# apelykh/deep-audio-mixer

Measured on AMD Instinct MI355X. Metric: stem-spectrogram-frames/sec (train), higher is better.
Workload: dtype f32; 1 GPU; C3: model_resnet (ResNet18, 8 stems) train step incl. STFT front-end, 8-stem 3 s @ 44.1 kHz stereo clips, n_fft 2048 hop 1024 -> 8x1025x130 per clip; batch_per_gpu=8, global_batch=8, parallelism=dp1, hip_graph=True, world_size=1, device_index=0, grad_buckets=1, allreduce_overlap=False

## Files before the change

deep-audio-mixer_amd/_lib.py:

```python
import ctypes
import os

import torch
import torch.utils.data

_HERE = os.path.dirname(os.path.abspath(__file__))
LIB_PATH = os.environ.get('DAM_LIB_PATH') or os.path.join(_HERE, 'libdam_hip.so')

EXPECTED_ABI = 22

_STATUS = {0: 'DAM_OK', -1: 'DAM_ERR_BAD_ARG', -2: 'DAM_ERR_UNSUPPORTED', -3: 'DAM_ERR_LAUNCH',
           -4: 'DAM_ERR_WORKSPACE'}

c_i, c_i64, c_f, c_p = ctypes.c_int, ctypes.c_int64, ctypes.c_float, ctypes.c_void_p
c_d = ctypes.c_double

SIGNATURES = {
    'dam_arch': (ctypes.c_char_p, []),
    'dam_abi_version': (c_i, []),
    'dam_host_dontfork_pinned': (c_i, [c_p, c_p]),
    'dam_step_mark_create': (c_i, [c_p]),
    'dam_step_mark_record': (c_i, [c_p, c_p]),
    'dam_step_mark_wait': (c_i, [c_p, c_p]),
    'dam_step_mark_synchronize': (c_i, [c_p]),
    'dam_step_mark_destroy': (c_i, [c_p]),
    'dam_stft_twiddle_count': (c_i64, [c_i]),
    'dam_stft_fill_twiddles_host': (c_i, [c_i, c_p]),
    'dam_stft_logmag_f32': (c_i, [c_p, c_i, c_i64, c_i64, c_i, c_i64, c_p, c_p, c_p, c_i, c_i, c_f, c_i, c_p, c_p]),
    'dam_stft_logmag_strided_f32': (c_i, [c_p, c_i, c_i64, c_i64, c_i64, c_i64, c_i64, c_i, c_i64, c_i64, c_p, c_p, c_p,
                                          c_i, c_i, c_f, c_i, c_p, c_p, c_i, c_p]),
    'dam_stft_complex_f32': (c_i, [c_p, c_i, c_i64, c_i64, c_i, c_i64, c_i64, c_i64, c_p, c_p, c_p, c_i, c_i, c_p, c_p]),
    'dam_stft_complex_strided_f32': (c_i, [c_p, c_i, c_i64, c_i64, c_i64, c_i64, c_i64, c_i64, c_i64, c_i, c_i64, c_i64,
                                           c_p, c_p, c_p, c_i, c_i, c_p, c_p]),
    'dam_istft_workspace_bytes': (c_i64, [c_i64, c_i64, c_i, c_i, c_i64]),
    'dam_istft_f32': (c_i, [c_p, c_p, c_i64, c_i64, c_i, c_i, c_i64, c_p, c_p, c_p, c_p, c_i64, c_p]),
    'dam_augment_gains_f32': (c_i, [ctypes.c_uint64, c_p, c_i64, c_i, c_i, c_f, c_f, c_p, c_p]),
    'dam_conv_packed_weight_count': (c_i64, [c_i, c_i, c_i, c_i]),
    'dam_conv_pack_weights_f32': (c_i, [c_p, c_i, c_i, c_i, c_i, c_i, c_p, c_p]),
    'dam_conv_pack_weights_multi_f32': (c_i, [c_p, c_i, c_i64, c_p]),
    'dam_conv2d_tapgrid_f32': (c_i, [c_p, c_i, c_i, c_i, c_i, c_i, c_p, c_i, c_i, c_p, c_p, c_p, c_i, c_i, c_p] +
                               [c_i] * 17 + [c_p, c_p, c_p, c_p, c_p, c_p, c_i64, c_p, c_p]),
    'dam_conv_batch_bytes': (c_i64, []),
    'dam_conv_batch_init': (c_i, [c_p]),
    'dam_conv_batch_flush': (c_i, [c_p, c_p]),
    'dam_conv2d_wgrad_workspace_floats': (c_i64, [c_i, c_i, c_i, c_i]),
    'dam_conv2d_wgrad_f32': (c_i, [c_p, c_i, c_i, c_i, c_i, c_i, c_p, c_p, c_i, c_p] + [c_i] * 9 +
                             [c_p, c_i, c_p, c_i64, c_p, c_p]),
    'dam_wgrad_queue_bytes': (c_i64, []),
    'dam_wgrad_queue_init': (c_i, [c_p]),
    'dam_wgrad_queue_pending': (c_i, [c_p]),
    'dam_wgrad_queue_flush': (c_i, [c_p, c_p]),
    'dam_wgrad_queue_set_batching': (c_i, [c_p, c_i]),
    'dam_bn_workspace_floats': (c_i64, [c_i]),
    'dam_bn_stats_f32': (c_i, [c_p, c_i64, c_i, c_p, c_p, c_p, c_p, c_p, c_f, c_f, c_p, c_p, c_p, c_p, c_p, c_p]),
    'dam_bn_finalize_f32': (c_i, [c_p, c_i, c_i, c_p, c_p, c_p, c_p, c_p, c_f, c_f, c_p, c_p, c_p, c_p, c_p]),
    'dam_conv1x1_pair_f32': (c_i, [c_p, c_p, c_i, c_p, c_p, c_i, c_i, c_i, c_i, c_i, c_i, c_p, c_i, c_i, c_i, c_i, c_i, c_p]),
    'dam_dgrad_s2_3x3_f32': (c_i, [c_p, c_p, c_p, c_p, c_i, c_i, c_i, c_i, c_i, c_p, c_i, c_i, c_p, c_p, c_p, c_p]),
    'dam_conv_s2_pair_fwd_f32': (c_i, [c_p, c_p, c_p, c_i, c_i, c_i, c_i, c_i, c_p, c_p, c_p, c_p, c_p, c_p]),
    'dam_bn_finalize_pair_f32': (c_i, [c_p, c_p, c_i, c_i, c_p, c_p, c_p]),
    'dam_strip_diag_counters': (c_i, [c_p, c_i]),
    'dam_bn_stats_partial_f32': (c_i, [c_p, c_i64, c_i, c_p, c_p, c_p]),
    'dam_bn_finalize_apply_f32': (c_i, [c_p, c_i, c_i, c_p, c_p, c_i64, c_p, c_p, c_p, c_i, c_p, c_p, c_p]),
    'dam_bn_eval_affine_f32': (c_i, [c_i, c_p, c_p, c_p, c_p, c_f, c_p, c_p, c_p, c_p, c_p]),
    'dam_bn_apply_f32': (c_i, [c_p, c_i64, c_i, c_p, c_p, c_p, c_p, c_p, c_i, c_p, c_p, c_p]),
    'dam_bn_stats_pair_f32': (c_i, [c_p, c_p, c_i64, c_i, c_p, c_p, c_p, c_p]),
    'dam_bn_pair_workspace_floats': (c_i64, [c_i]),
    'dam_bn_backward_pair_f32': (c_i, [c_p, c_p, c_p, c_i64, c_i, c_i] + [c_p] * 16),
    'dam_bn_backward_f32': (c_i, [c_p, c_p, c_p, c_i64, c_i, c_p, c_p, c_p, c_i, c_p, c_p, c_p, c_p, c_p, c_p, c_p, c_i, c_p]),
    'dam_channel_sum_f32': (c_i, [c_p, c_i64, c_i, c_i, c_p, c_p, c_p]),
    'dam_dropout_tick': (c_i, [c_p, c_i64, c_p, c_p]),
    'dam_dropout_apply_f32': (c_i, [c_p, c_i64, c_f, ctypes.c_uint64, c_p, c_p, c_p]),
    'dam_heads_fwd_f32': (c_i, [c_p, c_i, c_i, c_i, c_i, c_p, c_p, c_p, c_p, c_p, c_p, c_p]),
    'dam_heads_bwd_workspace_floats': (c_i64, [c_i, c_i, c_i, c_i]),
    'dam_heads_bwd_f32': (c_i, [c_p, c_p, c_p, c_i, c_i, c_i, c_i, c_p, c_p, c_p, c_p, c_p, c_p, c_p, c_p, c_p]),
    'dam_masksum_fwd_f32': (c_i, [c_p, c_p, c_i, c_i, c_i64, c_p, c_p]),
    'dam_masksum_workspace_floats': (c_i64, [c_i, c_i]),
    'dam_masksum_bwd_f32': (c_i, [c_p, c_p, c_i, c_i, c_i64, c_p, c_p, c_p]),
    'dam_masksum_mse_f32': (c_i, [c_p, c_p, c_p, c_i, c_i, c_i64, c_p, c_p, c_p, c_p, c_p]),
    'dam_adam_l2_step_f32': (c_i, [c_p, c_p, c_p, c_p, c_i64, c_p, c_p, c_f, c_f, c_f, c_f, c_f, c_f, c_p, c_p]),
    'dam_digest64_u32': (c_i, [c_p, c_i64, c_i64, c_i, c_i, c_p, c_p]),
    'dam_gains_smooth': (c_i, [c_p, c_i, c_i, c_i, c_i, c_p, c_p, c_p, c_p]),
    'dam_gain_ramp_apply': (c_i, [c_p, c_i, c_p, c_i64, c_i64, c_i64, c_i, c_p, c_i, c_p]),
    'dam_mixdown_workspace_elems': (c_i64, [c_i64]),
    'dam_mixdown_peak_normalize': (c_i, [c_p, c_i, c_p, c_i, c_i64, c_i64, c_i, c_i, c_p, c_i, c_p, c_p]),
    'dam_nchw_to_nhwc16_f32': (c_i, [c_p, c_i, c_i, c_i64, c_p, c_p]),
    'dam_loudness_kweight_coeffs': (c_i, [c_d, c_p]),
    'dam_loudness_workspace_bytes': (c_i64, [c_i64, c_i]),
    'dam_loudness_block_energy': (c_i, [c_p, c_i, c_i64, c_i, c_i64, c_i64, c_p, c_p, c_p, c_i, c_d, c_p, c_p, c_p]),
    'dam_loudness_batch_workspace_bytes': (c_i64, [c_i, c_i64, c_i, c_i]),
    'dam_loudness_block_energy_batch': (c_i, [c_p, c_i, c_i, c_i64, c_i, c_i64, c_i64, c_i64, c_p, c_i, c_p, c_p, c_p, c_i,
                                              c_d, c_p, c_p, c_p]),
    'dam_loudness_gate': (c_i, [c_p, c_i, c_i, c_i, c_p, c_p]),
    'dam_loudness_target_gains': (c_i, [c_p, c_p, c_i, c_p, c_p]),
    'dam_pcm_tile_frames': (c_i64, [c_i]),
    'dam_pcm_max_blocks': (c_i, []),
    'dam_pcm_encode': (c_i, [c_p, c_i, c_i, c_i64, c_p, c_i, c_i, c_i, ctypes.c_uint64, c_p, c_p, c_p]),
    'dam_true_peak_taps_host': (c_i, [c_p]),
    'dam_true_peak_tile_samples': (c_i64, []),
    'dam_true_peak_max_blocks': (c_i, []),
    'dam_true_peak_workspace_bytes': (c_i64, [c_i, c_i64, c_i]),
    'dam_true_peak_batch': (c_i, [c_p, c_i, c_i, c_i64, c_i, c_i64, c_i64, c_i64, c_p, c_i, c_p, c_p, c_p, c_p]),
    'dam_peak_limit_gains': (c_i, [c_p, c_p, c_i, c_i, c_d, c_p]),
    'dam_loudness_window_power': (c_i, [c_p, c_i, c_i, c_i, c_i, c_p, c_p, c_p]),
    'dam_loudness_curve_stats': (c_i, [c_p, c_i, c_i, c_p, c_p]),
    'dam_loudness_profile_error': (c_i, [c_p, c_p, c_i, c_i, c_i, c_p, c_p, c_p]),
}



class BnFin(ctypes.Structure):
    _fields_ = [('gamma', c_p), ('beta', c_p), ('running_mean', c_p), ('running_var', c_p), ('num_batches_tracked', c_p),
                ('momentum', c_f), ('eps', c_f), ('save_mean', c_p), ('save_invstd', c_p), ('scale', c_p), ('shift', c_p)]


class BnBwdSums(ctypes.Structure):
    _fields_ = [('x', c_p), ('mean', c_p), ('invstd', c_p), ('mask_scale', c_p), ('mask_shift', c_p), ('res_mask_bits', c_p),
                ('mask_bits', c_p)]


_lib = None


def lib():
    global _lib
    if torch.cuda._is_in_bad_fork() or torch.utils.data.get_worker_info() is not None:
        raise RuntimeError('deep_audio_mixer_amd: a GPU kernel was asked for in a DataLoader worker / forked child process '
                           '(pid %d).  The GPU belongs to the parent: workers of MultitrackAudioDataset return host PCM '
                           '(PcmItem / HostPcmBatch) and the front-end runs in the main process -- see '
                           'features.batch_features(batch)' % os.getpid())
    if _lib is None:
        if not os.path.exists(LIB_PATH):
            raise RuntimeError('libdam_hip.so is not built (%s): run `python __graft_entry__.py` or '
                               '`python deep-audio-mixer_amd/build.py`; there is no CPU fallback' % LIB_PATH)
        l = ctypes.CDLL(LIB_PATH)
        l.dam_abi_version.restype, l.dam_abi_version.argtypes = c_i, []
        have = l.dam_abi_version()
        if have != EXPECTED_ABI:
            raise RuntimeError('%s speaks ABI version %d, this package expects %d: the library is stale -- rebuild it '
                               '(`python deep-audio-mixer_amd/build.py --force`)' % (LIB_PATH, have, EXPECTED_ABI))
        for name, (res, args) in SIGNATURES.items():
            fn = getattr(l, name)
            fn.restype, fn.argtypes = res, args
        _lib = l
    return _lib


def check(status, what):
    if status != 0:
        raise RuntimeError('%s failed: %s (%d)' % (what, _STATUS.get(status, '?'), status))


def ptr(t):
    return None if t is None else t.data_ptr()


def stream():
    return torch.cuda.current_stream().cuda_stream


def require_cuda(*tensors):
    for t in tensors:
        if t is not None and not t.is_cuda:
            raise RuntimeError('deep_audio_mixer_amd kernels run on the GPU only (got a %s tensor); '
                               'there is no CPU fallback' % t.device)
```

deep-audio-mixer_amd/csrc/dam_bn.hip:

```cpp
#include <type_traits>
#include "dam_common.h"

namespace dam {
namespace {

constexpr int BN_MAX_PARTS = 1024;
static_assert(BN_MAX_PARTS == BN_BWD_RECORDS_MAX, "records a data-gradient epilogue may leave");

struct BnLaunch { int threads, q, r, parts; int64_t ppb; };

inline BnLaunch bn_plan(int64_t P, int C, int max_parts = BN_MAX_PARTS) {
    BnLaunch l;
    l.q = C / 4;
    l.r = 256 / l.q;
    if (l.r < 1) l.r = 1;
    l.threads = l.q * l.r;
    int64_t parts = cdiv(P, (int64_t)l.r * 16);
    if (parts > max_parts) {
        parts = max_parts;
        while (l.threads < 1024 && parts * l.threads < 131072 && (size_t)(l.r * 2) * C * 3 * sizeof(float) <= 48 * 1024) {
            l.r *= 2;
            l.threads *= 2;
        }
    }
    if (parts < 1) parts = 1;
    l.ppb = cdiv(P, parts);
    l.parts = (int)cdiv(P, l.ppb);
    return l;
}

struct RecAdd {
    template <int NV>
    static __device__ __forceinline__ void step(float* a, const float* b) {
#pragma unroll
        for (int k = 0; k < NV; ++k) a[k] += b[k];
    }
};
struct RecChan {
    template <int NV>
    static __device__ __forceinline__ void step(float* a, const float* b) {
        static_assert(NV == 3, "(n, mean, M2)");
        const float na = a[0], nb = b[0];
        if (nb != 0.f) {
            const float nn = na + nb, d = b[1] - a[1];
            a[1] += d * (nb / nn);
            a[2] += b[2] + d * d * (na * nb / nn);
            a[0] = nn;
        }
    }
};
template <int NV, typename Merge>
__device__ __forceinline__ void record_tail(float* sm, const float (&v)[NV][4], int C, int cq, int pr, int R,
                                            float* __restrict__ record ) {
#pragma unroll
    for (int i = 0; i < 4; ++i) {
        float* o = sm + ((size_t)pr * C + cq * 4 + i) * NV;
#pragma unroll
        for (int k = 0; k < NV; ++k) o[k] = v[k][i];
    }
    __syncthreads();
    int span = 1;
    while (span < R) span <<= 1;
    for (int stride = span >> 1; stride >= 1; stride >>= 1) {
        if (pr < stride && pr + stride < R) {
#pragma unroll
            for (int i = 0; i < 4; ++i)
                Merge::template step<NV>(sm + ((size_t)pr * C + cq * 4 + i) * NV, sm + ((size_t)(pr + stride) * C + cq * 4 + i) * NV);
        }
        __syncthreads();
    }
    if (pr == 0) {
#pragma unroll
        for (int i = 0; i < 4; ++i) {
            const int c = cq * 4 + i;
#pragma unroll
            for (int k = 0; k < NV; ++k) store_sc1(record + (size_t)c * NV + k, sm[(size_t)c * NV + k]);
        }
    }
}

__global__ void bn_stats_partial_kernel(const float* __restrict__ x, int64_t P, int C, int Q, int R, int64_t ppb,
                                        float* __restrict__ partial ,
                                        const float* __restrict__ x2, float* __restrict__ partial2) {
    extern __shared__ __attribute__((aligned(16))) float sm[];
    if (blockIdx.y) { x = x2; partial = partial2; }
    const int cq = threadIdx.x % Q, pr = threadIdx.x / Q;
    const int64_t lo = blockIdx.x * ppb, hi = (lo + ppb < P) ? lo + ppb : P;
    float k[4] = {0, 0, 0, 0}, s1[4] = {0, 0, 0, 0}, s2[4] = {0, 0, 0, 0};
    int n = 0;
    constexpr int U = 8;
    for (int64_t p = lo + pr; p < hi; p += (int64_t)R * U) {
        float4 v[U];
#pragma unroll
        for (int u = 0; u < U; ++u) {
            const int64_t q = p + (int64_t)u * R;
            v[u] = q < hi ? *reinterpret_cast<const float4*>(x + q * C + cq * 4) : make_float4(0.f, 0.f, 0.f, 0.f);
        }
        if (n == 0) { k[0] = v[0].x; k[1] = v[0].y; k[2] = v[0].z; k[3] = v[0].w; }
#pragma unroll
        for (int u = 0; u < U; ++u) {
            if (p + (int64_t)u * R < hi) {
                const float e[4] = {v[u].x, v[u].y, v[u].z, v[u].w};
#pragma unroll
                for (int i = 0; i < 4; ++i) {
                    const float d = e[i] - k[i];
                    s1[i] += d;
                    s2[i] = fmaf(d, d, s2[i]);
                }
                ++n;
            }
        }
    }
    float v[3][4];
#pragma unroll
    for (int i = 0; i < 4; ++i) {
        const float md = n ? s1[i] / n : 0.f;
        v[0][i] = (float)n;
        v[1][i] = k[i] + md;
        v[2][i] = n ? fmaxf(s2[i] - s1[i] * md, 0.f) : 0.f;
    }
    record_tail<3, RecChan>(sm, v, C, cq, pr, R, partial + (size_t)blockIdx.x * C * 3);
}

__global__ __launch_bounds__(64) void bn_stats_finalize_kernel(const float* __restrict__ partial, int parts, int C,
                                         const float* __restrict__ gamma, const float* __restrict__ beta,
                                         float* __restrict__ running_mean, float* __restrict__ running_var,
                                         long long* __restrict__ num_batches, float momentum, float eps,
                                         float* __restrict__ save_mean, float* __restrict__ save_invstd,
                                         float* __restrict__ scale, float* __restrict__ shift, const BnFinArgs second,
                                         const float* __restrict__ partial2) {
    if (blockIdx.y) {
        partial = partial2; gamma = second.gamma; beta = second.beta; running_mean = second.running_mean;
        running_var = second.running_var; num_batches = second.num_batches; momentum = second.momentum; eps = second.eps;
        save_mean = second.save_mean; save_invstd = second.save_invstd; scale = second.scale; shift = second.shift;
    }
    const int c = blockIdx.x, lane = threadIdx.x;
    if (c == 0 && lane == 0 && num_batches) *num_batches += 1;
    const float gam_c = gamma[c], bet_c = beta[c];
    const float rm_c = running_mean ? running_mean[c] : 0.f, rv_c = running_mean ? running_var[c] : 0.f;
    constexpr int U = 16;
    float rn[U], rmn[U], rq[U];
#pragma unroll
    for (int u = 0; u < U; ++u) {
        const int p = lane + 64 * u;
        const float* o = partial + ((size_t)(p < parts ? p : 0) * C + c) * 3;
        rn[u] = o[0]; rmn[u] = o[1]; rq[u] = o[2];
        if (p >= parts) rn[u] = 0.f;
    }
    double na = 0, sa = 0;
#pragma unroll
    for (int u = 0; u < U; ++u) { na += (double)rn[u]; sa += (double)rn[u] * (double)rmn[u]; }
    for (int p = lane + 64 * U; p < parts; p += 64) {
        const float* o = partial + ((size_t)p * C + c) * 3;
        na += (double)o[0]; sa += (double)o[0] * (double)o[1];
    }
#pragma unroll
    for (int off = 32; off >= 1; off >>= 1) { na += __shfl_xor(na, off); sa += __shfl_xor(sa, off); }
    const double ma = sa / na;
    double qa = 0;
#pragma unroll
    for (int u = 0; u < U; ++u) { const double d = (double)rmn[u] - ma; qa += (double)rq[u] * (rn[u] != 0.f ? 1.0 : 0.0) + (double)rn[u] * d * d; }
    for (int p = lane + 64 * U; p < parts; p += 64) {
        const float* o = partial + ((size_t)p * C + c) * 3;
        const double d = (double)o[1] - ma;
        qa += (double)o[2] + (double)o[0] * d * d;
    }
#pragma unroll
    for (int off = 32; off >= 1; off >>= 1) qa += __shfl_xor(qa, off);
    if (lane != 0) return;
    const double var = qa / na;
    const float mean = (float)ma;
    const float invstd = (float)(1.0 / sqrt(var + (double)eps));
    save_mean[c] = mean;
    save_invstd[c] = invstd;
    const float sc = gam_c * invstd;
    scale[c] = sc;
    shift[c] = bet_c - mean * sc;
    if (running_mean) {
        const double unbiased = na > 1 ? qa / (na - 1) : var;
        running_mean[c] = (1.f - momentum) * rm_c + momentum * mean;
        running_var[c] = (1.f - momentum) * rv_c + momentum * (float)unbiased;
    }
}

__global__ void bn_eval_affine_kernel(int C, const float* __restrict__ gamma, const float* __restrict__ beta,
                                      const float* __restrict__ running_mean, const float* __restrict__ running_var,
                                      float eps, float* __restrict__ save_mean, float* __restrict__ save_invstd,
                                      float* __restrict__ scale, float* __restrict__ shift) {
    const int c = blockIdx.x * blockDim.x + threadIdx.x;
    if (c >= C) return;
    const float invstd = 1.0f / sqrtf(running_var[c] + eps);
    const float sc = gamma[c] * invstd;
    save_mean[c] = running_mean[c];
    save_invstd[c] = invstd;
    scale[c] = sc;
    shift[c] = beta[c] - running_mean[c] * sc;
}

__global__ void bn_apply_kernel(const float* __restrict__ x, int64_t nquads, int Q, const float* __restrict__ scale,
                                const float* __restrict__ shift, const float* __restrict__ res,
                                const float* __restrict__ rscale, const float* __restrict__ rshift, int relu,
                                float* __restrict__ y, unsigned char* __restrict__ sign_bits) {
    for (int64_t e = blockIdx.x * (int64_t)blockDim.x + threadIdx.x; e < nquads; e += (int64_t)gridDim.x * blockDim.x) {
        const int cq = (int)(e % Q);
        const float4 v = reinterpret_cast<const float4*>(x)[e];
        const float4 sc = reinterpret_cast<const float4*>(scale)[cq], sh = reinterpret_cast<const float4*>(shift)[cq];
        float4 o = make_float4(fmaf(v.x, sc.x, sh.x), fmaf(v.y, sc.y, sh.y), fmaf(v.z, sc.z, sh.z), fmaf(v.w, sc.w, sh.w));
        if (res) {
            float4 r = reinterpret_cast<const float4*>(res)[e];
            if (rscale) {
                const float4 a = reinterpret_cast<const float4*>(rscale)[cq], b = reinterpret_cast<const float4*>(rshift)[cq];
                r = make_float4(fmaf(r.x, a.x, b.x), fmaf(r.y, a.y, b.y), fmaf(r.z, a.z, b.z), fmaf(r.w, a.w, b.w));
            }
            o.x += r.x; o.y += r.y; o.z += r.z; o.w += r.w;
        }
        if (relu) { o.x = fmaxf(o.x, 0.f); o.y = fmaxf(o.y, 0.f); o.z = fmaxf(o.z, 0.f); o.w = fmaxf(o.w, 0.f); }
        reinterpret_cast<float4*>(y)[e] = o;
        if (sign_bits) sign_bits[e] = (unsigned char)((o.x > 0.f) | ((o.y > 0.f) << 1) | ((o.z > 0.f) << 2) | ((o.w > 0.f) << 3));
    }
}

__device__ __forceinline__ float4 sign_quad(unsigned b) {
    return make_float4((float)(b & 1u), (float)((b >> 1) & 1u), (float)((b >> 2) & 1u), (float)((b >> 3) & 1u));
}

struct BnBwdSide {
    const float* x;
    const float* gamma;
    const float* mean;
    const float* invstd;
    float* dx;
    float* dgamma;
    float* dbeta;
};
template <int NB>
struct BnBwdSides { BnBwdSide s[NB]; };

template <int MASK, int NB>
__global__ void bn_bwd_partial_kernel(const float* __restrict__ dy, const float* __restrict__ y_mask, const BnBwdSides<NB> sd,
                                      int64_t P, int C, int Q, int R, int64_t ppb, const float* __restrict__ mscale,
                                      const float* __restrict__ mshift, float* __restrict__ partial ) {
    extern __shared__ __attribute__((aligned(16))) float sm[];
    const int cq = threadIdx.x % Q, pr = threadIdx.x / Q;
    const int64_t lo = blockIdx.x * ppb, hi = (lo + ppb < P) ? lo + ppb : P;
    float4 mu[NB], is[NB];
#pragma unroll
    for (int s = 0; s < NB; ++s) {
        mu[s] = reinterpret_cast<const float4*>(sd.s[s].mean)[cq];
        is[s] = reinterpret_cast<const float4*>(sd.s[s].invstd)[cq];
    }
    float4 msc = make_float4(0.f, 0.f, 0.f, 0.f), msh = msc;
    if (MASK == 2) { msc = reinterpret_cast<const float4*>(mscale)[cq]; msh = reinterpret_cast<const float4*>(mshift)[cq]; }
    float acc[1 + NB][4] = {};
    constexpr int U = NB == 1 ? 4 : 3;
    for (int64_t p = lo + pr; p < hi; p += (int64_t)R * U) {
        float4 gv[U], mv[U], xv[NB][U];
#pragma unroll
        for (int u = 0; u < U; ++u) {
            const int64_t q = p + (int64_t)u * R;
            const bool ok = q < hi;
            const float4 z = make_float4(0.f, 0.f, 0.f, 0.f);
            gv[u] = z; mv[u] = make_float4(1.f, 1.f, 1.f, 1.f);
#pragma unroll
            for (int s = 0; s < NB; ++s) xv[s][u] = z;
            if (ok) {
                gv[u] = *reinterpret_cast<const float4*>(dy + q * C + cq * 4);
#pragma unroll
                for (int s = 0; s < NB; ++s) xv[s][u] = *reinterpret_cast<const float4*>(sd.s[s].x + q * C + cq * 4);
                if (MASK == 1) mv[u] = *reinterpret_cast<const float4*>(y_mask + q * C + cq * 4);
            }
            if (MASK == 3) mv[u] = sign_quad(ok ? reinterpret_cast<const unsigned char*>(y_mask)[q * Q + cq] : 0);
        }
#pragma unroll
        for (int u = 0; u < U; ++u) {
            float4 g = gv[u];
            float4 m = mv[u];
            if (MASK == 2) {
                const float4 v = xv[0][u];
                m = make_float4(fmaf(v.x, msc.x, msh.x), fmaf(v.y, msc.y, msh.y), fmaf(v.z, msc.z, msh.z), fmaf(v.w, msc.w, msh.w));
            }
            g.x = m.x > 0.f ? g.x : 0.f; g.y = m.y > 0.f ? g.y : 0.f; g.z = m.z > 0.f ? g.z : 0.f; g.w = m.w > 0.f ? g.w : 0.f;
            acc[0][0] += g.x; acc[0][1] += g.y; acc[0][2] += g.z; acc[0][3] += g.w;
#pragma unroll
            for (int s = 0; s < NB; ++s) {
                const float4 v = xv[s][u];
                float* b = acc[1 + s];
                b[0] = fmaf(g.x, (v.x - mu[s].x) * is[s].x, b[0]); b[1] = fmaf(g.y, (v.y - mu[s].y) * is[s].y, b[1]);
                b[2] = fmaf(g.z, (v.z - mu[s].z) * is[s].z, b[2]); b[3] = fmaf(g.w, (v.w - mu[s].w) * is[s].w, b[3]);
            }
        }
    }
    record_tail<1 + NB, RecAdd>(sm, acc, C, cq, pr, R, partial + (size_t)blockIdx.x * C * (1 + NB));
}

__device__ __forceinline__ double wave_sum64_f64(double v) {
#pragma unroll
    for (int off = 32; off >= 1; off >>= 1) v += __shfl_down(v, off);
    return v;
}

template <int NV>
__device__ __forceinline__ void wave_record_sums(const float* __restrict__ partial, int parts, int C, int c, double (&s)[NV]) {
    const int lane = threadIdx.x;
    constexpr int U = 16;
    float r[U][NV];
#pragma unroll
    for (int u = 0; u < U; ++u) {
        const int p = lane + 64 * u;
        const float* o = partial + ((size_t)(p < parts ? p : 0) * C + c) * NV;
#pragma unroll
        for (int k = 0; k < NV; ++k) r[u][k] = p < parts ? o[k] : 0.f;
    }
#pragma unroll
    for (int k = 0; k < NV; ++k) s[k] = 0;
#pragma unroll
    for (int u = 0; u < U; ++u)
#pragma unroll
        for (int k = 0; k < NV; ++k) s[k] += (double)r[u][k];
    for (int p = lane + 64 * U; p < parts; p += 64)
#pragma unroll
        for (int k = 0; k < NV; ++k) s[k] += partial[((size_t)p * C + c) * NV + k];
#pragma unroll
    for (int k = 0; k < NV; ++k) s[k] = wave_sum64_f64(s[k]);
}

__global__ __launch_bounds__(64) void bn_bwd_finalize_kernel(const float* __restrict__ partial, int parts, int C, double count,
                                       const float* __restrict__ gamma, const float* __restrict__ mean,
                                       const float* __restrict__ invstd, int training, float* __restrict__ dgamma,
                                       float* __restrict__ dbeta, float* __restrict__ coef ) {
    const int c = blockIdx.x, lane = threadIdx.x;
    const float gam_c = gamma[c], inv_c = invstd[c], mean_c = mean[c];
    double s[2];
    wave_record_sums<2>(partial, parts, C, c, s);
    if (lane != 0) return;
    const double s1 = s[0], s2 = s[1];
    dbeta[c] = (float)s1;
    dgamma[c] = (float)s2;
    const double g = (double)gam_c * inv_c;
    double c2 = 0, c3 = 0;
    if (training) {
        c2 = -g * inv_c * s2 / count;
        c3 = -g * s1 / count - c2 * mean_c;
    }
    coef[c] = (float)g; coef[C + c] = (float)c2; coef[2 * C + c] = (float)c3;
}

template <int MASK>
__global__ void bn_bwd_apply_kernel(const float* __restrict__ dy, const float* __restrict__ y_mask,
                                    const float* __restrict__ x, int64_t nquads, int Q, int C,
                                    const float* __restrict__ coef, const float* __restrict__ mscale,
                                    const float* __restrict__ mshift, float* __restrict__ dx) {
    for (int64_t e = blockIdx.x * (int64_t)blockDim.x + threadIdx.x; e < nquads; e += (int64_t)gridDim.x * blockDim.x) {
        const int cq = (int)(e % Q);
        float4 g = reinterpret_cast<const float4*>(dy)[e];
        const float4 v = reinterpret_cast<const float4*>(x)[e];
        if (MASK != 0) {
            float4 m;
            if (MASK == 1) {
                m = reinterpret_cast<const float4*>(y_mask)[e];
            } else if (MASK == 3) {
                m = sign_quad(reinterpret_cast<const unsigned char*>(y_mask)[e]);
            } else {
                const float4 sc = reinterpret_cast<const float4*>(mscale)[cq], sh = reinterpret_cast<const float4*>(mshift)[cq];
                m = make_float4(fmaf(v.x, sc.x, sh.x), fmaf(v.y, sc.y, sh.y), fmaf(v.z, sc.z, sh.z), fmaf(v.w, sc.w, sh.w));
            }
            g.x = m.x > 0.f ? g.x : 0.f; g.y = m.y > 0.f ? g.y : 0.f; g.z = m.z > 0.f ? g.z : 0.f; g.w = m.w > 0.f ? g.w : 0.f;
        }
        const float4 c1 = reinterpret_cast<const float4*>(coef)[cq], c2 = reinterpret_cast<const float4*>(coef + C)[cq],
                     c3 = reinterpret_cast<const float4*>(coef + 2 * C)[cq];
        float4 o;
        o.x = fmaf(c1.x, g.x, fmaf(c2.x, v.x, c3.x)); o.y = fmaf(c1.y, g.y, fmaf(c2.y, v.y, c3.y));
        o.z = fmaf(c1.z, g.z, fmaf(c2.z, v.z, c3.z)); o.w = fmaf(c1.w, g.w, fmaf(c2.w, v.w, c3.w));
        reinterpret_cast<float4*>(dx)[e] = o;
    }
}

__global__ void channel_sum_partial_kernel(const float* __restrict__ x, int64_t P, int C, int Q, int R, int64_t ppb,
                                           float* __restrict__ partial) {
    extern __shared__ float sm[];
    const int cq = threadIdx.x % Q, pr = threadIdx.x / Q;
    const int64_t lo = blockIdx.x * ppb, hi = (lo + ppb < P) ? lo + ppb : P;
    float a[1][4] = {};
    constexpr int U = 8;
    for (int64_t p = lo + pr; p < hi; p += (int64_t)R * U) {
        float4 v[U];
#pragma unroll
        for (int u = 0; u < U; ++u) {
            const int64_t q = p + (int64_t)u * R;
            v[u] = q < hi ? *reinterpret_cast<const float4*>(x + q * C + cq * 4) : make_float4(0.f, 0.f, 0.f, 0.f);
        }
#pragma unroll
        for (int u = 0; u < U; ++u) { a[0][0] += v[u].x; a[0][1] += v[u].y; a[0][2] += v[u].z; a[0][3] += v[u].w; }
    }
    record_tail<1, RecAdd>(sm, a, C, cq, pr, R, partial + (size_t)blockIdx.x * C);
}
__global__ __launch_bounds__(64) void channel_sum_finalize_kernel(const float* __restrict__ partial, int parts, int C, int n_real,
                                            float* __restrict__ out) {
    double s[1];
    wave_record_sums<1>(partial, parts, C, blockIdx.x, s);
    if (threadIdx.x == 0) out[blockIdx.x] = (float)s[0];
}

__device__ __forceinline__ float4 zero4() { return make_float4(0.f, 0.f, 0.f, 0.f); }
constexpr int FA_THREADS = 256;
constexpr int FA_U = 4;

constexpr int FA_WGS = 512;

struct FaPlan { int cs, nslices, nranges, q, ppi; int64_t ppr; };

inline int fa_cs(int C) { return C <= 32 ? C : 16; }
inline FaPlan fa_plan(int64_t P, int C) {
    FaPlan f;
    f.cs = fa_cs(C);
    f.nslices = C / f.cs;
    f.q = f.cs / 4;
    f.ppi = FA_THREADS / f.q;
    int64_t want = P / ((int64_t)f.ppi * FA_U * 2);
    const int64_t cap = FA_WGS / f.nslices > 0 ? FA_WGS / f.nslices : 1;
    if (want > cap) want = cap;
    if (want < 1) want = 1;
    f.ppr = cdiv(P, want);
    f.nranges = (int)cdiv(P, f.ppr);
    return f;
}
constexpr int FA_TABLE_BYTES_MAX = 80 * 1024;
inline bool fa_table_ok(int C, int parts, int rec_floats) { return (int64_t)parts * fa_cs(C) * rec_floats * 4 <= FA_TABLE_BYTES_MAX; }
constexpr int FA_FWD_TABLE_KB = 24;
inline bool fa_fwd_table_ok(int C, int parts) {
    return fa_table_ok(C, parts, 3) && (int64_t)parts * fa_cs(C) * 12 <= (int64_t)FA_FWD_TABLE_KB * 1024;
}

template <int NR, int NV, typename F>
__device__ __forceinline__ void fa_slice_sums(const float* __restrict__ partial, int parts, int C, int ch, int CS, double* red,
                                              double (&acc)[NV], F term) {
    const int tid = threadIdx.x, TPC = FA_THREADS / CS, i0 = tid / CS;
    constexpr int RU = 16;
#pragma unroll
    for (int k = 0; k < NV; ++k) acc[k] = 0;
    for (int p0 = i0; p0 < parts; p0 += TPC * RU) {
        float rec[RU][NR];
#pragma unroll
        for (int u = 0; u < RU; ++u) {
            const int p = p0 + u * TPC;
            const float* o = partial + ((size_t)(p < parts ? p : i0) * C + ch) * NR;
#pragma unroll
            for (int k = 0; k < NR; ++k) rec[u][k] = o[k];
        }
#pragma unroll
        for (int u = 0; u < RU; ++u)
            if (p0 + u * TPC < parts) {
                double v[NV];
                term(rec[u], v);
#pragma unroll
                for (int k = 0; k < NV; ++k) acc[k] += v[k];
            }
    }
#pragma unroll
    for (int k = 0; k < NV; ++k) red[tid * NV + k] = acc[k];
    __syncthreads();
    if (tid < CS)
        for (int i = 1; i < TPC; ++i)
#pragma unroll
            for (int k = 0; k < NV; ++k) acc[k] += red[(tid + i * CS) * NV + k];
}

template <int S> using FaSet = std::integral_constant<int, S>;
template <typename Load, typename Emit>
__device__ __forceinline__ void fa_stream(int64_t p0, int64_t hi, int64_t step, Load load, Emit emit) {
    for (;;) {
        if (p0 + step < hi) load(FaSet<1>{}, p0 + step);
        emit(FaSet<0>{}, p0);
        p0 += step;
        if (p0 >= hi) break;
        if (p0 + step < hi) load(FaSet<0>{}, p0 + step);
        emit(FaSet<1>{}, p0);
        p0 += step;
        if (p0 >= hi) break;
    }
}

__global__ __launch_bounds__(FA_THREADS) void bn_fin_apply_kernel(const float* __restrict__ partial, int parts, int C, int CS,
                                                                   const BnFinArgs fin, const float* __restrict__ x, int64_t P,
                                                                   int64_t ppr, const float* __restrict__ res,
                                                                   const float* __restrict__ rscale, const float* __restrict__ rshift,
                                                                   int relu, float* __restrict__ y, unsigned char* __restrict__ sign_bits) {
    __shared__ double red[FA_THREADS * 3];
    __shared__ __attribute__((aligned(16))) float tab[2 * 32];
    const int tid = threadIdx.x, slice = blockIdx.y, q = CS / 4, tq = tid % q, tp = tid / q, ppi = FA_THREADS / q;
    const int Q = C / 4, cq = slice * q + tq;
    const int64_t lo = blockIdx.x * ppr, hi = (lo + ppr < P) ? lo + ppr : P;
    const int64_t step = (int64_t)ppi * FA_U;
    float4 xv[2][FA_U], rv[2][FA_U];
    auto load = [&](auto set, int64_t p0) {
        constexpr int S = decltype(set)::value;
#pragma unroll
        for (int u = 0; u < FA_U; ++u) {
            const int64_t p = p0 + (int64_t)u * ppi;
            xv[S][u] = p < hi ? reinterpret_cast<const float4*>(x)[p * Q + cq] : zero4();
            if (res) rv[S][u] = p < hi ? reinterpret_cast<const float4*>(res)[p * Q + cq] : zero4();
        }
    };
    load(FaSet<0>{}, lo + tp);
    float4 ra = make_float4(1.f, 1.f, 1.f, 1.f), rb = zero4();
    if (rscale) { ra = reinterpret_cast<const float4*>(rscale)[cq]; rb = reinterpret_cast<const float4*>(rshift)[cq]; }
    {
        const int cl = tid % CS, ch = slice * CS + cl;
        const float m0 = partial[(size_t)ch * 3 + 1];
        const float gam = fin.gamma[ch], bet = fin.beta[ch];
        const bool writer = blockIdx.x == 0 && tid < CS;
        const float rm = (writer && fin.running_mean) ? fin.running_mean[ch] : 0.f, rvv = (writer && fin.running_mean) ? fin.running_var[ch] : 0.f;
        double acc[3];
        fa_slice_sums<3, 3>(partial, parts, C, ch, CS, red, acc, [m0](const float (&r)[3], double (&v)[3]) {
            const double n = (double)r[0], d = (double)r[1] - (double)m0;
            v[0] = n; v[1] = n * d; v[2] = n != 0.0 ? (double)r[2] + n * d * d : 0.0;
        });
        if (tid < CS) {
            const double na = acc[0], ds = acc[1] / na, qa = acc[2] - acc[1] * ds;
            const double var = qa / na;
            const float mean = (float)((double)m0 + ds);
            const float invstd = (float)(1.0 / sqrt((var > 0 ? var : 0.0) + (double)fin.eps));
            const float sc = gam * invstd, sh = bet - mean * sc;
            tab[cl] = sc; tab[CS + cl] = sh;
            if (writer) {
                fin.save_mean[ch] = mean; fin.save_invstd[ch] = invstd; fin.scale[ch] = sc; fin.shift[ch] = sh;
                if (fin.running_mean) {
                    const double unbiased = na > 1 ? (qa > 0 ? qa : 0.0) / (na - 1) : var;
                    fin.running_mean[ch] = (1.f - fin.momentum) * rm + fin.momentum * mean;
                    fin.running_var[ch] = (1.f - fin.momentum) * rvv + fin.momentum * (float)unbiased;
                }
                if (ch == 0 && fin.num_batches) *fin.num_batches += 1;
            }
        }
        __syncthreads();
    }
    const float4 sc = *reinterpret_cast<const float4*>(tab + tq * 4), sh = *reinterpret_cast<const float4*>(tab + CS + tq * 4);
    fa_stream(lo + tp, hi, step, load, [&](auto set, int64_t p0) {
        constexpr int S = decltype(set)::value;
#pragma unroll
        for (int u = 0; u < FA_U; ++u) {
            const int64_t p = p0 + (int64_t)u * ppi;
            if (p < hi) {
                const float4 v = xv[S][u];
                float4 o = make_float4(fmaf(v.x, sc.x, sh.x), fmaf(v.y, sc.y, sh.y), fmaf(v.z, sc.z, sh.z), fmaf(v.w, sc.w, sh.w));
                if (res) {
                    float4 r = rv[S][u];
                    if (rscale) r = make_float4(fmaf(r.x, ra.x, rb.x), fmaf(r.y, ra.y, rb.y), fmaf(r.z, ra.z, rb.z), fmaf(r.w, ra.w, rb.w));
                    o.x += r.x; o.y += r.y; o.z += r.z; o.w += r.w;
                }
                if (relu) { o.x = fmaxf(o.x, 0.f); o.y = fmaxf(o.y, 0.f); o.z = fmaxf(o.z, 0.f); o.w = fmaxf(o.w, 0.f); }
                reinterpret_cast<float4*>(y)[p * Q + cq] = o;
                if (sign_bits)
                    sign_bits[p * Q + cq] = (unsigned char)((o.x > 0.f) | ((o.y > 0.f) << 1) | ((o.z > 0.f) << 2) | ((o.w > 0.f) << 3));
            }
        }
    });
}

template <int MASK, int NB>
__global__ __launch_bounds__(FA_THREADS) void bn_bwd_fin_apply_kernel(const float* __restrict__ partial, int parts, int C, int CS,
                                                                       double count, int training, const BnBwdSides<NB> sd,
                                                                       const float* __restrict__ dy, const float* __restrict__ y_mask,
                                                                       int64_t P, int64_t ppr, const float* __restrict__ mscale,
                                                                       const float* __restrict__ mshift) {
    constexpr int NR = 1 + NB;
    __shared__ double red[FA_THREADS * NR];
    __shared__ __attribute__((aligned(16))) float tab[3 * NB * 32];
    const int tid = threadIdx.x, slice = blockIdx.y, q = CS / 4, tq = tid % q, tp = tid / q, ppi = FA_THREADS / q;
    const int Q = C / 4, cq = slice * q + tq;
    const int64_t lo = blockIdx.x * ppr, hi = (lo + ppr < P) ? lo + ppr : P;
    constexpr int UB = NB == 1 ? 3 : 2;
    const int64_t step = (int64_t)ppi * UB;
    float4 gv[2][UB], xv[NB][2][UB], mv[2][UB];
    auto load = [&](auto set, int64_t p0) {
        constexpr int S = decltype(set)::value;
#pragma unroll
        for (int u = 0; u < UB; ++u) {
            const int64_t p = p0 + (int64_t)u * ppi;
            const bool ok = p < hi;
            gv[S][u] = ok ? reinterpret_cast<const float4*>(dy)[p * Q + cq] : zero4();
#pragma unroll
            for (int s = 0; s < NB; ++s) xv[s][S][u] = ok ? reinterpret_cast<const float4*>(sd.s[s].x)[p * Q + cq] : zero4();
            if (MASK == 1) mv[S][u] = ok ? reinterpret_cast<const float4*>(y_mask)[p * Q + cq] : zero4();
            if (MASK == 3) mv[S][u] = sign_quad(ok ? reinterpret_cast<const unsigned char*>(y_mask)[p * Q + cq] : 0);
        }
    };
    load(FaSet<0>{}, lo + tp);
    float4 msc = zero4(), msh = zero4();
    if (MASK == 2) { msc = reinterpret_cast<const float4*>(mscale)[cq]; msh = reinterpret_cast<const float4*>(mshift)[cq]; }
    {
        const int cl = tid % CS, ch = slice * CS + cl;
        float gam[NB], inv[NB], mu[NB];
#pragma unroll
        for (int s = 0; s < NB; ++s) { gam[s] = sd.s[s].gamma[ch]; inv[s] = sd.s[s].invstd[ch]; mu[s] = sd.s[s].mean[ch]; }
        double acc[NR];
        fa_slice_sums<NR, NR>(partial, parts, C, ch, CS, red, acc, [](const float (&r)[NR], double (&v)[NR]) {
#pragma unroll
            for (int k = 0; k < NR; ++k) v[k] = (double)r[k];
        });
        if (tid < CS) {
#pragma unroll
            for (int s = 0; s < NB; ++s) {
                const double s1 = acc[0], s2 = acc[1 + s];
                const double g = (double)gam[s] * inv[s];
                double c2 = 0, c3 = 0;
                if (training) { c2 = -g * inv[s] * s2 / count; c3 = -g * s1 / count - c2 * mu[s]; }
                float* t = tab + 3 * s * CS;
                t[cl] = (float)g; t[CS + cl] = (float)c2; t[2 * CS + cl] = (float)c3;
                if (blockIdx.x == 0) { sd.s[s].dbeta[ch] = (float)s1; sd.s[s].dgamma[ch] = (float)s2; }
            }
        }
        __syncthreads();
    }
    float4 k[NB][3];
#pragma unroll
    for (int i = 0; i < 3 * NB; ++i) k[i / 3][i % 3] = *reinterpret_cast<const float4*>(tab + i * CS + tq * 4);
    fa_stream(lo + tp, hi, step, load, [&](auto set, int64_t p0) {
        constexpr int S = decltype(set)::value;
#pragma unroll
        for (int u = 0; u < UB; ++u) {
            const int64_t p = p0 + (int64_t)u * ppi;
            if (p < hi) {
                float4 g = gv[S][u];
                if (MASK != 0) {
                    float4 m = mv[S][u];
                    if (MASK == 2) {
                        const float4 v = xv[0][S][u];
                        m = make_float4(fmaf(v.x, msc.x, msh.x), fmaf(v.y, msc.y, msh.y), fmaf(v.z, msc.z, msh.z), fmaf(v.w, msc.w, msh.w));
                    }
                    g.x = m.x > 0.f ? g.x : 0.f; g.y = m.y > 0.f ? g.y : 0.f; g.z = m.z > 0.f ? g.z : 0.f; g.w = m.w > 0.f ? g.w : 0.f;
                }
                float4 o[NB];
#pragma unroll
                for (int s = 0; s < NB; ++s) {
                    const float4 v = xv[s][S][u], c1 = k[s][0], c2 = k[s][1], c3 = k[s][2];
                    o[s].x = fmaf(c1.x, g.x, fmaf(c2.x, v.x, c3.x)); o[s].y = fmaf(c1.y, g.y, fmaf(c2.y, v.y, c3.y));
                    o[s].z = fmaf(c1.z, g.z, fmaf(c2.z, v.z, c3.z)); o[s].w = fmaf(c1.w, g.w, fmaf(c2.w, v.w, c3.w));
                }
#pragma unroll
                for (int s = 0; s < NB; ++s) reinterpret_cast<float4*>(sd.s[s].dx)[p * Q + cq] = o[s];
            }
        }
    });
}

inline int elt_blocks(int64_t n) {
    int64_t b = cdiv(n, 256);
    return (int)(b < 4096 ? (b < 1 ? 1 : b) : 4096);
}

constexpr int FA_PARTS_KB = 64;
inline int fa_max_parts(int C, int rec_floats) {
    int m = FA_PARTS_KB * 1024 / (fa_cs(C) * rec_floats * 4);
    if (m > BN_MAX_PARTS) m = BN_MAX_PARTS;
    return m < 64 ? 64 : m;
}

inline bool fin_args(const dam_bn_fin* f, BnFinArgs* a) {
    if (!f || !f->gamma || !f->beta || !f->save_mean || !f->save_invstd || !f->scale || !f->shift) return false;
    *a = BnFinArgs{f->gamma, f->beta, f->running_mean, f->running_var, (long long*)f->num_batches_tracked, f->momentum,
                   f->eps, f->save_mean, f->save_invstd, f->scale, f->shift};
    return true;
}

template <int... MASKS, typename F>
inline bool with_mask(int mask, F f) {
    return ((mask == MASKS ? (f(std::integral_constant<int, MASKS>{}), true) : false) || ...);
}

template <int NB, int... MASKS>
inline int bn_bwd_launch(const BnLaunch& l, bool given, bool fused, int mask, const BnBwdSides<NB>& sd, const float* dy,
                         const float* y_mask, int64_t P, int C, int training, const float* mask_scale, const float* mask_shift,
                         float* workspace, hipStream_t st) {
    if (!given) {
        const bool known = with_mask<MASKS...>(mask, [&](auto m) {
            hipLaunchKernelGGL((bn_bwd_partial_kernel<decltype(m)::value, NB>), dim3(l.parts), dim3(l.threads),
                               (size_t)l.r * C * (1 + NB) * sizeof(float), st, dy, y_mask, sd, P, C, l.q, l.r, l.ppb, mask_scale,
                               mask_shift, workspace);
        });
        if (!known) return DAM_ERR_BAD_ARG;
        DAM_CHECK_LAUNCH();
    }
    if (fused) {
        const FaPlan f = fa_plan(P, C);
        const bool known = with_mask<MASKS...>(mask, [&](auto m) {
            hipLaunchKernelGGL((bn_bwd_fin_apply_kernel<decltype(m)::value, NB>), dim3(f.nranges, f.nslices), dim3(FA_THREADS), 0, st,
                               (const float*)workspace, l.parts, C, f.cs, (double)P, training, sd, dy, y_mask, P, f.ppr, mask_scale,
                               mask_shift);
        });
        if (!known) return DAM_ERR_BAD_ARG;
        DAM_CHECK_LAUNCH();
    }
    return DAM_OK;
}

}
}

using namespace dam;

extern "C" int64_t dam_bn_workspace_floats(int C) { return (int64_t)BN_RECORDS_MAX * C * 3; }

extern "C" int dam_bn_stats_partial_f32(const float* x, int64_t n_pixels, int C, float* workspace, int* parts_host, void* stream) {
    if (!x || !workspace || !parts_host || n_pixels <= 0) return DAM_ERR_BAD_ARG;
    if (C % 16 || C > 1024) return DAM_ERR_UNSUPPORTED;
    const BnLaunch l = bn_plan(n_pixels, C, fa_max_parts(C, 3));
    hipLaunchKernelGGL(bn_stats_partial_kernel, dim3(l.parts), dim3(l.threads), (size_t)l.r * C * 3 * sizeof(float), (hipStream_t)stream,
                       x, n_pixels, C, l.q, l.r, l.ppb, workspace, (const float*)nullptr, (float*)nullptr);
    DAM_CHECK_LAUNCH();
    *parts_host = l.parts;
    return DAM_OK;
}

extern "C" int dam_bn_finalize_apply_f32(const float* partial, int parts, int C, const dam_bn_fin* fin, const float* x,
                                         int64_t n_pixels, const float* res, const float* res_scale, const float* res_shift,
                                         int relu, float* y, uint8_t* sign_bits, void* stream) {
    BnFinArgs a;
    if (!partial || parts <= 0 || !fin_args(fin, &a) || !x || !y || n_pixels <= 0) return DAM_ERR_BAD_ARG;
    if (res_scale && (!res || !res_shift)) return DAM_ERR_BAD_ARG;
    if (C % 16 || C > 1024) return DAM_ERR_UNSUPPORTED;
    hipStream_t st = (hipStream_t)stream;
    if (!fa_fwd_table_ok(C, parts)) {
        int rc = dam_bn_finalize_f32(partial, parts, C, fin->gamma, fin->beta, fin->running_mean, fin->running_var,
                                     fin->num_batches_tracked, fin->momentum, fin->eps, fin->save_mean, fin->save_invstd, fin->scale,
                                     fin->shift, stream);
        if (rc != DAM_OK) return rc;
        return dam_bn_apply_f32(x, n_pixels, C, fin->scale, fin->shift, res, res_scale, res_shift, relu, y, sign_bits, stream);
    }
    const FaPlan f = fa_plan(n_pixels, C);
    hipLaunchKernelGGL(bn_fin_apply_kernel, dim3(f.nranges, f.nslices), dim3(FA_THREADS), 0, st, partial, parts, C, f.cs, a, x,
                       n_pixels, f.ppr, res, res_scale, res_shift, relu, y, sign_bits);
    DAM_CHECK_LAUNCH();
    return DAM_OK;
}

extern "C" int dam_bn_stats_f32(const float* x, int64_t n_pixels, int C, const float* gamma, const float* beta,
                                float* running_mean, float* running_var, int64_t* num_batches_tracked,
                                float momentum, float eps, float* save_mean, float* save_invstd, float* scale,
                                float* shift, float* workspace, void* stream) {
    if (!x || !gamma || !beta || !save_mean || !save_invstd || !scale || !shift || !workspace || n_pixels <= 0)
        return DAM_ERR_BAD_ARG;
    if (C % 16 || C > 1024) return DAM_ERR_UNSUPPORTED;
    const BnLaunch l = bn_plan(n_pixels, C);
    hipStream_t st = (hipStream_t)stream;
    hipLaunchKernelGGL(bn_stats_partial_kernel, dim3(l.parts), dim3(l.threads), (size_t)l.r * C * 3 * sizeof(float), st,
                       x, n_pixels, C, l.q, l.r, l.ppb, workspace, (const float*)nullptr, (float*)nullptr);
    DAM_CHECK_LAUNCH();
    hipLaunchKernelGGL(bn_stats_finalize_kernel, dim3(C), dim3(64), 0, st, workspace, l.parts, C,
                       gamma, beta, running_mean, running_var, (long long*)num_batches_tracked, momentum, eps,
                       save_mean, save_invstd, scale, shift, BnFinArgs{}, (const float*)nullptr);
    DAM_CHECK_LAUNCH();
    return DAM_OK;
}

extern "C" int dam_bn_stats_pair_f32(const float* x_a, const float* x_b, int64_t n_pixels, int C, const dam_bn_fin* a,
                                     const dam_bn_fin* b, float* workspace, void* stream) {
    BnFinArgs fa, fb;
    if (!x_a || !x_b || !fin_args(a, &fa) || !fin_args(b, &fb) || !workspace || n_pixels <= 0) return DAM_ERR_BAD_ARG;
    if (C % 16 || C > 1024) return DAM_ERR_UNSUPPORTED;
    const BnLaunch l = bn_plan(n_pixels, C);
    hipStream_t st = (hipStream_t)stream;
    float* ws_b = workspace + (size_t)BN_RECORDS_MAX * C * 3;
    hipLaunchKernelGGL(bn_stats_partial_kernel, dim3(l.parts, 2), dim3(l.threads), (size_t)l.r * C * 3 * sizeof(float), st, x_a,
                       n_pixels, C, l.q, l.r, l.ppb, workspace, x_b, ws_b);
    DAM_CHECK_LAUNCH();
    hipLaunchKernelGGL(bn_stats_finalize_kernel, dim3(C, 2), dim3(64), 0, st, workspace, l.parts, C, fa.gamma, fa.beta,
                       fa.running_mean, fa.running_var, fa.num_batches, fa.momentum, fa.eps, fa.save_mean, fa.save_invstd, fa.scale,
                       fa.shift, fb, (const float*)ws_b);
    DAM_CHECK_LAUNCH();
    return DAM_OK;
}

extern "C" int dam_bn_finalize_f32(const float* partial, int parts, int C, const float* gamma, const float* beta,
                                   float* running_mean, float* running_var, int64_t* num_batches_tracked,
                                   float momentum, float eps, float* save_mean, float* save_invstd, float* scale,
                                   float* shift, void* stream) {
    if (!partial || parts <= 0 || C <= 0 || !gamma || !beta || !save_mean || !save_invstd || !scale || !shift)
        return DAM_ERR_BAD_ARG;
    hipLaunchKernelGGL(bn_stats_finalize_kernel, dim3(C), dim3(64), 0, (hipStream_t)stream, partial, parts, C, gamma, beta,
                       running_mean, running_var, (long long*)num_batches_tracked, momentum, eps, save_mean, save_invstd,
                       scale, shift, BnFinArgs{}, (const float*)nullptr);
    DAM_CHECK_LAUNCH();
    return DAM_OK;
}

extern "C" int dam_bn_finalize_pair_f32(const float* partial_a, const float* partial_b, int parts, int C, const dam_bn_fin* a,
                                        const dam_bn_fin* b, void* stream) {
    BnFinArgs fa, fb;
    if (!partial_a || !partial_b || parts <= 0 || C <= 0 || !fin_args(a, &fa) || !fin_args(b, &fb)) return DAM_ERR_BAD_ARG;
    hipLaunchKernelGGL(bn_stats_finalize_kernel, dim3(C, 2), dim3(64), 0, (hipStream_t)stream, partial_a, parts, C, fa.gamma, fa.beta,
                       fa.running_mean, fa.running_var, fa.num_batches, fa.momentum, fa.eps, fa.save_mean, fa.save_invstd, fa.scale,
                       fa.shift, fb, partial_b);
    DAM_CHECK_LAUNCH();
    return DAM_OK;
}

extern "C" int dam_bn_eval_affine_f32(int C, const float* gamma, const float* beta, const float* running_mean,
                                      const float* running_var, float eps, float* save_mean, float* save_invstd,
                                      float* scale, float* shift, void* stream) {
    if (!gamma || !beta || !running_mean || !running_var || !save_mean || !save_invstd || !scale || !shift || C <= 0)
        return DAM_ERR_BAD_ARG;
    hipLaunchKernelGGL(bn_eval_affine_kernel, dim3((unsigned)cdiv(C, 64)), dim3(64), 0, (hipStream_t)stream, C, gamma, beta,
                       running_mean, running_var, eps, save_mean, save_invstd, scale, shift);
    DAM_CHECK_LAUNCH();
    return DAM_OK;
}

extern "C" int dam_bn_apply_f32(const float* x, int64_t n_pixels, int C, const float* scale, const float* shift,
                                const float* res, const float* res_scale, const float* res_shift, int relu, float* y,
                                uint8_t* sign_bits, void* stream) {
    if (!x || !scale || !shift || !y || n_pixels <= 0) return DAM_ERR_BAD_ARG;
    if (C % 16) return DAM_ERR_UNSUPPORTED;
    if (res_scale && (!res || !res_shift)) return DAM_ERR_BAD_ARG;
    const int64_t nq = n_pixels * (C / 4);
    hipLaunchKernelGGL(bn_apply_kernel, dim3(elt_blocks(nq)), dim3(256), 0, (hipStream_t)stream, x, nq, C / 4, scale, shift,
                       res, res_scale, res_shift, relu, y, sign_bits);
    DAM_CHECK_LAUNCH();
    return DAM_OK;
}

extern "C" int dam_bn_backward_f32(const float* dy, const float* y_mask, const float* x, int64_t n_pixels, int C,
                                   const float* gamma, const float* save_mean, const float* save_invstd, int training,
                                   const float* mask_scale, const float* mask_shift, const uint8_t* mask_bits, float* dx,
                                   float* dgamma, float* dbeta, float* workspace, int partials_given, void* stream) {
    if (!dy || !x || !gamma || !save_mean || !save_invstd || !dx || !dgamma || !dbeta || !workspace || n_pixels <= 0)
        return DAM_ERR_BAD_ARG;
    if ((mask_scale != nullptr) != (mask_shift != nullptr) || (y_mask && mask_scale) || (mask_bits && (y_mask || mask_scale)))
        return DAM_ERR_BAD_ARG;
    if (mask_bits) y_mask = reinterpret_cast<const float*>(mask_bits);
    if (C % 16 || C > 1024) return DAM_ERR_UNSUPPORTED;
    BnLaunch l = bn_plan(n_pixels, C, fa_max_parts(C, 2));
    if (partials_given < 0 || partials_given > BN_MAX_PARTS) return DAM_ERR_BAD_ARG;
    if (partials_given) l.parts = partials_given;
    const bool fused = fa_table_ok(C, l.parts, 2);
    hipStream_t st = (hipStream_t)stream;
    const int mask = mask_bits ? 3 : (y_mask ? 1 : (mask_scale ? 2 : 0));
    const BnBwdSides<1> sd{{{x, gamma, save_mean, save_invstd, dx, dgamma, dbeta}}};
    const int rc = bn_bwd_launch<1, 0, 1, 2, 3>(l, partials_given != 0, fused, mask, sd, dy, y_mask, n_pixels, C, training,
                                                mask_scale, mask_shift, workspace, st);
    if (rc != DAM_OK || fused) return rc;
    float* coef = workspace + (size_t)BN_MAX_PARTS * C * 2;
    hipLaunchKernelGGL(bn_bwd_finalize_kernel, dim3(C), dim3(64), 0, st, workspace, l.parts, C,
                       (double)n_pixels, gamma, save_mean, save_invstd, training, dgamma, dbeta, coef);
    DAM_CHECK_LAUNCH();
    const int64_t nq = n_pixels * (C / 4);
    const bool known = with_mask<0, 1, 2, 3>(mask, [&](auto m) {
        hipLaunchKernelGGL(bn_bwd_apply_kernel<decltype(m)::value>, dim3(elt_blocks(nq)), dim3(256), 0, st, dy, y_mask, x, nq, C / 4,
                           C, (const float*)coef, mask_scale, mask_shift, dx);
    });
    if (!known) return DAM_ERR_BAD_ARG;
    DAM_CHECK_LAUNCH();
    return DAM_OK;
}

extern "C" int64_t dam_bn_pair_workspace_floats(int C) { return (int64_t)BN_MAX_PARTS * C * 3 + 6 * (int64_t)C; }

extern "C" int dam_bn_backward_pair_f32(const float* dy, const float* y_mask, const uint8_t* mask_bits, int64_t n_pixels, int C,
                                        int training,
                                        const float* x_a, const float* gamma_a, const float* mean_a, const float* invstd_a,
                                        float* dx_a, float* dgamma_a, float* dbeta_a,
                                        const float* x_b, const float* gamma_b, const float* mean_b, const float* invstd_b,
                                        float* dx_b, float* dgamma_b, float* dbeta_b, float* workspace, void* stream) {
    if ((y_mask != nullptr) == (mask_bits != nullptr)) return DAM_ERR_BAD_ARG;
    const bool bits = mask_bits != nullptr;
    if (bits) y_mask = reinterpret_cast<const float*>(mask_bits);
    if (!dy || !y_mask || !x_a || !gamma_a || !mean_a || !invstd_a || !dx_a || !dgamma_a || !dbeta_a || !x_b || !gamma_b ||
        !mean_b || !invstd_b || !dx_b || !dgamma_b || !dbeta_b || !workspace || n_pixels <= 0)
        return DAM_ERR_BAD_ARG;
    if (C % 16 || C > 1024) return DAM_ERR_UNSUPPORTED;
    const BnLaunch l = bn_plan(n_pixels, C, fa_max_parts(C, 3));
    if ((size_t)l.r * C * 3 * sizeof(float) > 64 * 1024) return DAM_ERR_UNSUPPORTED;
    const BnBwdSides<2> sd{{{x_a, gamma_a, mean_a, invstd_a, dx_a, dgamma_a, dbeta_a},
                            {x_b, gamma_b, mean_b, invstd_b, dx_b, dgamma_b, dbeta_b}}};
    return bn_bwd_launch<2, 1, 3>(l, false, true, bits ? 3 : 1, sd, dy, y_mask, n_pixels, C, training, nullptr, nullptr, workspace,
                                  (hipStream_t)stream);
}

extern "C" int dam_channel_sum_f32(const float* x, int64_t n_pixels, int C, int n_real, float* out, float* workspace,
                                   void* stream) {
    if (!x || !out || !workspace || n_pixels <= 0 || n_real <= 0 || n_real > C) return DAM_ERR_BAD_ARG;
    if (C % 16 || C > 1024) return DAM_ERR_UNSUPPORTED;
    const BnLaunch l = bn_plan(n_pixels, C);
    hipStream_t st = (hipStream_t)stream;
    hipLaunchKernelGGL(channel_sum_partial_kernel, dim3(l.parts), dim3(l.threads), (size_t)l.r * C * sizeof(float), st, x,
                       n_pixels, C, l.q, l.r, l.ppb, workspace);
    DAM_CHECK_LAUNCH();
    hipLaunchKernelGGL(channel_sum_finalize_kernel, dim3(n_real), dim3(64), 0, st, workspace, l.parts, C,
                       n_real, out);
    DAM_CHECK_LAUNCH();
    return DAM_OK;
}
```

deep-audio-mixer_amd/csrc/dam_head.hip:

```cpp
#include "dam_common.h"

namespace dam {
namespace {

constexpr int MAX_STEMS = 16;

template <int GS>
__global__ __launch_bounds__(256) void head_conv_kernel(const float* __restrict__ trunk, int P, int C, int S,
                                                        const float* __restrict__ cw, const float* __restrict__ cb,
                                                        float* __restrict__ h) {
    extern __shared__ float w_s[];
    for (int e = threadIdx.x; e < S * C; e += blockDim.x) w_s[e] = cw[e];
    __syncthreads();
    constexpr int G = 64 / GS;
    const int lane = threadIdx.x & 63, wave = threadIdx.x >> 6, b = blockIdx.y;
    const int gl = lane % GS, gi = lane / GS;
    const int Q = C / 4;
    for (int p0 = (blockIdx.x * 4 + wave) * G; p0 < P; p0 += gridDim.x * 4 * G) {
        const int p = p0 + gi;
        const bool live = p < P;
        float acc[MAX_STEMS];
#pragma unroll
        for (int s = 0; s < MAX_STEMS; ++s) acc[s] = 0.f;
        const float4* row = reinterpret_cast<const float4*>(trunk + ((size_t)b * P + (live ? p : 0)) * C);
        for (int q = gl; q < Q; q += GS) {
            const float4 v = live ? row[q] : make_float4(0.f, 0.f, 0.f, 0.f);
#pragma unroll
            for (int s = 0; s < MAX_STEMS; ++s) {
                if (s < S) {
                    const float4 w = reinterpret_cast<const float4*>(w_s + s * C)[q];
                    acc[s] = fmaf(v.x, w.x, fmaf(v.y, w.y, fmaf(v.z, w.z, fmaf(v.w, w.w, acc[s]))));
                }
            }
        }
#pragma unroll
        for (int s = 0; s < MAX_STEMS; ++s) {
            if (s < S) {
                float t = wave_sum16(acc[s]);
                if (GS >= 32) t += __shfl_xor(t, 16);
                if (GS >= 64) t += __shfl_xor(t, 32);
                if (gl == 0 && live) h[((size_t)b * S + s) * P + p] = fmaxf(t + cb[s], 0.f);
            }
        }
    }
}

__device__ __forceinline__ float block_sum(float v, float* red) {
    v = wave_sum64(v);
    const int lane = threadIdx.x & 63, wave = threadIdx.x >> 6;
    __syncthreads();
    if (lane == 0) red[wave] = v;
    __syncthreads();
    return red[0] + red[1] + red[2] + red[3];
}

__global__ __launch_bounds__(256) void head_fc_kernel(const float* __restrict__ h, int P, int S,
                                                      const float* __restrict__ fcw, const float* __restrict__ fcb,
                                                      float* __restrict__ g) {
    __shared__ float red[4];
    const int s = blockIdx.x, b = blockIdx.y;
    const float* hr = h + ((size_t)b * S + s) * P;
    const float* wr = fcw + (size_t)s * P;
    float a8[8] = {0.f, 0.f, 0.f, 0.f, 0.f, 0.f, 0.f, 0.f};
    int p = threadIdx.x;
    for (; p + 7 * 256 < P; p += 8 * 256) {
        float hv[8], wv[8];
#pragma unroll
        for (int u = 0; u < 8; ++u) { hv[u] = hr[p + u * 256]; wv[u] = wr[p + u * 256]; }
#pragma unroll
        for (int u = 0; u < 8; ++u) a8[u] = fmaf(hv[u], wv[u], a8[u]);
    }
    for (; p < P; p += 256) a8[0] = fmaf(hr[p], wr[p], a8[0]);
    float a = ((a8[0] + a8[1]) + (a8[2] + a8[3])) + ((a8[4] + a8[5]) + (a8[6] + a8[7]));
    a = block_sum(a, red);
    if (threadIdx.x == 0) g[b * S + s] = a + fcb[s];
}

template <int GS>
__global__ __launch_bounds__(256) void head_bwd_pixel_kernel(const float* __restrict__ dg, const float* __restrict__ h,
                                                             int P, int C, int S, const float* __restrict__ cw,
                                                             const float* __restrict__ fcw, float* __restrict__ e_out,
                                                             float* __restrict__ dtrunk, int B, float* __restrict__ dfcw,
                                                             float* __restrict__ dfcb) {
    extern __shared__ float w_s[];
    if (blockIdx.y == (unsigned)B) {
        for (int i = blockIdx.x * blockDim.x + threadIdx.x; i < S * P; i += gridDim.x * blockDim.x) {
            const int s = i / P, p = i - s * P;
            float a = 0.f;
            for (int bb = 0; bb < B; ++bb) a = fmaf(dg[bb * S + s], h[((size_t)bb * S + s) * P + p], a);
            dfcw[i] = a;
            if (i < S) {
                float t = 0.f;
                for (int bb = 0; bb < B; ++bb) t += dg[bb * S + i];
                dfcb[i] = t;
            }
        }
        return;
    }
    for (int e = threadIdx.x; e < S * C; e += blockDim.x) w_s[e] = cw[e];
    __syncthreads();
    constexpr int G = 64 / GS;
    const int lane = threadIdx.x & 63, wave = threadIdx.x >> 6, b = blockIdx.y;
    const int gl = lane % GS, gi = lane / GS;
    const int Q = C / 4;
    for (int p0 = (blockIdx.x * 4 + wave) * G; p0 < P; p0 += gridDim.x * 4 * G) {
        const int p = p0 + gi;
        if (p >= P) continue;
        float ev[MAX_STEMS];
#pragma unroll
        for (int s = 0; s < MAX_STEMS; ++s) {
            ev[s] = 0.f;
            if (s < S) {
                const size_t i = ((size_t)b * S + s) * P + p;
                ev[s] = h[i] > 0.f ? dg[b * S + s] * fcw[(size_t)s * P + p] : 0.f;
                if (gl == 0) e_out[i] = ev[s];
            }
        }
        float4* row = reinterpret_cast<float4*>(dtrunk + ((size_t)b * P + p) * C);
        for (int q = gl; q < Q; q += GS) {
            float4 o = make_float4(0.f, 0.f, 0.f, 0.f);
#pragma unroll
            for (int s = 0; s < MAX_STEMS; ++s) {
                if (s < S) {
                    const float4 w = reinterpret_cast<const float4*>(w_s + s * C)[q];
                    o.x = fmaf(ev[s], w.x, o.x); o.y = fmaf(ev[s], w.y, o.y);
                    o.z = fmaf(ev[s], w.z, o.z); o.w = fmaf(ev[s], w.w, o.w);
                }
            }
            row[q] = o;
        }
    }
}

__global__ void head_bwd_cw_partial_kernel(const float* __restrict__ e, const float* __restrict__ trunk, int B, int P,
                                           int C, int S, int Q, int R, int64_t ppb, float* __restrict__ partial,
                                           float* __restrict__ partial_b) {
    extern __shared__ float sm[];
    const int cq = threadIdx.x % Q, pr = threadIdx.x / Q;
    const int64_t BP = (int64_t)B * P;
    const int64_t lo = blockIdx.x * ppb, hi = (lo + ppb < BP) ? lo + ppb : BP;
    float acc[MAX_STEMS][4], esum[MAX_STEMS];
#pragma unroll
    for (int s = 0; s < MAX_STEMS; ++s) { acc[s][0] = acc[s][1] = acc[s][2] = acc[s][3] = 0.f; esum[s] = 0.f; }
    for (int64_t bp = lo + pr; bp < hi; bp += R) {
        const int b = (int)(bp / P), p = (int)(bp - (int64_t)b * P);
        const float4 v = *reinterpret_cast<const float4*>(trunk + bp * C + cq * 4);
#pragma unroll
        for (int s = 0; s < MAX_STEMS; ++s) {
            if (s < S) {
                const float ev = e[((size_t)b * S + s) * P + p];
                esum[s] += ev;
                acc[s][0] = fmaf(ev, v.x, acc[s][0]); acc[s][1] = fmaf(ev, v.y, acc[s][1]);
                acc[s][2] = fmaf(ev, v.z, acc[s][2]); acc[s][3] = fmaf(ev, v.w, acc[s][3]);
            }
        }
    }
#pragma unroll
    for (int s = 0; s < MAX_STEMS; ++s)
        if (s < S)
#pragma unroll
            for (int i = 0; i < 4; ++i) sm[((size_t)pr * S + s) * C + cq * 4 + i] = acc[s][i];
    __syncthreads();
    if (pr == 0) {
        for (int s = 0; s < S; ++s)
#pragma unroll
            for (int i = 0; i < 4; ++i) {
                float a = 0.f;
                for (int r = 0; r < R; ++r) a += sm[((size_t)r * S + s) * C + cq * 4 + i];
                partial[((size_t)blockIdx.x * S + s) * C + cq * 4 + i] = a;
            }
    }
    __syncthreads();
    if (cq == 0)
        for (int s = 0; s < S; ++s) sm[pr * S + s] = esum[s];
    __syncthreads();
    if (threadIdx.x < S) {
        float a = 0.f;
        for (int r = 0; r < R; ++r) a += sm[r * S + threadIdx.x];
        partial_b[(size_t)blockIdx.x * S + threadIdx.x] = a;
    }
}
__global__ __launch_bounds__(256) void head_bwd_cw_finalize_kernel(const float* __restrict__ partial,
                                                                   const float* __restrict__ partial_b, int parts, int C, int S,
                                                                   float* __restrict__ dcw, float* __restrict__ dcb) {
    __shared__ double sub[32][8];
    const int el = threadIdx.x & 7, ys = threadIdx.x >> 3;
    const int i = blockIdx.x * 8 + el, n = S * C;
    double a = 0;
    if (i < n) {
        for (int p = ys; p < parts; p += 32) a += (double)partial[(size_t)p * n + i];
    } else if (i < n + S) {
        for (int p = ys; p < parts; p += 32) a += (double)partial_b[(size_t)p * S + (i - n)];
    }
    sub[ys][el] = a;
    __syncthreads();
#pragma unroll
    for (int stride = 16; stride >= 1; stride >>= 1) {
        if (ys < stride) sub[ys][el] += sub[ys + stride][el];
        __syncthreads();
    }
    if (ys == 0) {
        if (i < n) dcw[i] = (float)sub[0][el];
        else if (i < n + S) dcb[i - n] = (float)sub[0][el];
    }
}

__global__ void masksum_fwd_kernel(const float* __restrict__ x, const float* __restrict__ g, int S, int64_t FT,
                                   float* __restrict__ masked) {
    const int b = blockIdx.y;
    float gv[MAX_STEMS];
#pragma unroll
    for (int s = 0; s < MAX_STEMS; ++s) gv[s] = s < S ? g[b * S + s] : 0.f;
    const float* xb = x + (size_t)b * S * FT;
    for (int64_t i = blockIdx.x * (int64_t)blockDim.x + threadIdx.x; i < FT; i += (int64_t)gridDim.x * blockDim.x) {
        float a = 0.f;
#pragma unroll
        for (int s = 0; s < MAX_STEMS; ++s)
            if (s < S) a = fmaf(gv[s], xb[(size_t)s * FT + i], a);
        masked[(size_t)b * FT + i] = a;
    }
}

template <int MODE, int SC>
__global__ __launch_bounds__(256) void masksum_bwd_partial_kernel(const float* __restrict__ x, const float* __restrict__ g,
                                                                  const float* __restrict__ d_or_gt, int S_rt, int64_t FT,
                                                                  float* __restrict__ masked_out,
                                                                  float* __restrict__ partial ) {
    constexpr int SM = SC ? SC : MAX_STEMS, U = SC ? 2 : 1;
    const int S = SC ? SC : S_rt;
    const int b = blockIdx.y;
    float gv[SM], acc[SM + 1];
#pragma unroll
    for (int s = 0; s < SM; ++s) { gv[s] = (MODE == 1 && s < S) ? g[b * S + s] : 0.f; acc[s] = 0.f; }
    acc[SM] = 0.f;
    const float* xb = x + (size_t)b * S * FT;
    const int64_t step = (int64_t)gridDim.x * blockDim.x;
    if (SC && (FT & 1) == 0) {
        const int64_t F2 = FT >> 1;
        const float2* tb = reinterpret_cast<const float2*>(d_or_gt + (size_t)b * FT);
        for (int64_t i0 = blockIdx.x * (int64_t)blockDim.x + threadIdx.x; i0 < F2; i0 += step * U) {
            float2 xv[U][SM], tv[U];
#pragma unroll
            for (int u = 0; u < U; ++u) {
                const int64_t i = i0 + u * step;
                const bool ok = i < F2;
#pragma unroll
                for (int s = 0; s < SM; ++s)
                    xv[u][s] = ok ? reinterpret_cast<const float2*>(xb + (size_t)s * FT)[i] : make_float2(0.f, 0.f);
                tv[u] = ok ? tb[i] : make_float2(0.f, 0.f);
            }
#pragma unroll
            for (int u = 0; u < U; ++u) {
                const int64_t i = i0 + u * step;
                if (i < F2) {
                    float2 d;
                    if (MODE == 1) {
                        float2 m = make_float2(0.f, 0.f);
#pragma unroll
                        for (int s = 0; s < SM; ++s) { m.x = fmaf(gv[s], xv[u][s].x, m.x); m.y = fmaf(gv[s], xv[u][s].y, m.y); }
                        if (masked_out) reinterpret_cast<float2*>(masked_out + (size_t)b * FT)[i] = m;
                        d = make_float2(m.x - tv[u].x, m.y - tv[u].y);
                        acc[SM] = fmaf(d.x, d.x, acc[SM]);
                        acc[SM] = fmaf(d.y, d.y, acc[SM]);
                    } else {
                        d = tv[u];
                    }
#pragma unroll
                    for (int s = 0; s < SM; ++s) { acc[s] = fmaf(d.x, xv[u][s].x, acc[s]); acc[s] = fmaf(d.y, xv[u][s].y, acc[s]); }
                }
            }
        }
    } else {
        for (int64_t i0 = blockIdx.x * (int64_t)blockDim.x + threadIdx.x; i0 < FT; i0 += step * U) {
            float xv[U][SM], tv[U];
#pragma unroll
            for (int u = 0; u < U; ++u) {
                const int64_t i = i0 + u * step;
                const bool ok = i < FT;
#pragma unroll
                for (int s = 0; s < SM; ++s) xv[u][s] = (ok && s < S) ? xb[(size_t)s * FT + i] : 0.f;
                tv[u] = ok ? d_or_gt[(size_t)b * FT + i] : 0.f;
            }
#pragma unroll
            for (int u = 0; u < U; ++u) {
                const int64_t i = i0 + u * step;
                if (i < FT) {
                    float d;
                    if (MODE == 1) {
                        float m = 0.f;
#pragma unroll
                        for (int s = 0; s < SM; ++s) m = fmaf(gv[s], xv[u][s], m);
                        if (masked_out) masked_out[(size_t)b * FT + i] = m;
                        d = m - tv[u];
                        acc[SM] = fmaf(d, d, acc[SM]);
                    } else {
                        d = tv[u];
                    }
#pragma unroll
                    for (int s = 0; s < SM; ++s) acc[s] = fmaf(d, xv[u][s], acc[s]);
                }
            }
        }
    }
    __shared__ float redw[4][MAX_STEMS + 1];
    const int lane = threadIdx.x & 63, wave = threadIdx.x >> 6;
#pragma unroll
    for (int k = 0; k <= SM; ++k) {
        const float t = wave_sum64(acc[k]);
        if (lane == 0) redw[wave][k == SM ? MAX_STEMS : k] = t;
    }
    __syncthreads();
    float* out = partial + ((size_t)b * gridDim.x + blockIdx.x) * (S + 1);
    if ((int)threadIdx.x <= S) {
        const int k = (int)threadIdx.x == S ? MAX_STEMS : (int)threadIdx.x;
        out[threadIdx.x] = redw[0][k] + redw[1][k] + redw[2][k] + redw[3][k];
    }
}
__global__ __launch_bounds__(64) void masksum_bwd_finalize_kernel(const float* __restrict__ partial, int B, int nblk, int S,
                                                                  double scale, double inv_count, float* __restrict__ dg,
                                                                  float* __restrict__ loss) {
    const int i = blockIdx.x, lane = threadIdx.x;
    double a = 0;
    if (i < B * S) {
        const int b = i / S, s = i - b * S;
        for (int k = lane; k < nblk; k += 64) a += partial[((size_t)b * nblk + k) * (S + 1) + s];
    } else {
        for (int k = lane; k < B * nblk; k += 64) a += partial[(size_t)k * (S + 1) + S];
    }
#pragma unroll
    for (int off = 32; off >= 1; off >>= 1) a += __shfl_down(a, off);
    if (lane != 0) return;
    if (i < B * S) dg[i] = (float)(a * scale);
    else if (loss) *loss = (float)(a * inv_count);
}

}
}

using namespace dam;

extern "C" int dam_heads_fwd_f32(const float* trunk, int B, int P, int C, int S, const float* conv_w, const float* conv_b,
                                 const float* fc_w, const float* fc_b, float* h, float* gains, void* stream) {
    if (!trunk || !conv_w || !conv_b || !fc_w || !fc_b || !h || !gains || B <= 0 || P <= 0) return DAM_ERR_BAD_ARG;
    if (C % 4 || S < 1 || S > MAX_STEMS || B > 65535) return DAM_ERR_UNSUPPORTED;
    hipStream_t st = (hipStream_t)stream;
    const int Q = C / 4, gs = Q <= 16 ? 16 : Q <= 32 ? 32 : 64, ppw = 4 * (64 / gs);
    const int gx = (int)(cdiv(P, ppw) < 1024 ? cdiv(P, ppw) : 1024);
    if (gs == 16) hipLaunchKernelGGL(head_conv_kernel<16>, dim3(gx, B), dim3(256), (size_t)S * C * sizeof(float), st, trunk, P, C, S, conv_w, conv_b, h);
    else if (gs == 32) hipLaunchKernelGGL(head_conv_kernel<32>, dim3(gx, B), dim3(256), (size_t)S * C * sizeof(float), st, trunk, P, C, S, conv_w, conv_b, h);
    else hipLaunchKernelGGL(head_conv_kernel<64>, dim3(gx, B), dim3(256), (size_t)S * C * sizeof(float), st, trunk, P, C, S, conv_w, conv_b, h);
    DAM_CHECK_LAUNCH();
    hipLaunchKernelGGL(head_fc_kernel, dim3(S, B), dim3(256), 0, st, h, P, S, fc_w, fc_b, gains);
    DAM_CHECK_LAUNCH();
    return DAM_OK;
}

extern "C" int64_t dam_heads_bwd_workspace_floats(int B, int P, int C, int S) {
    return (int64_t)B * S * P + (int64_t)1024 * S * C + (int64_t)1024 * S;
}

extern "C" int dam_heads_bwd_f32(const float* dgains, const float* h, const float* trunk, int B, int P, int C, int S,
                                 const float* conv_w, const float* fc_w, float* dtrunk, float* dconv_w, float* dconv_b,
                                 float* dfc_w, float* dfc_b, float* workspace, void* stream) {
    if (!dgains || !h || !trunk || !conv_w || !fc_w || !dtrunk || !dconv_w || !dconv_b || !dfc_w || !dfc_b || !workspace)
        return DAM_ERR_BAD_ARG;
    if (C % 16 || S < 1 || S > MAX_STEMS || B > 65534 || C > 1024) return DAM_ERR_UNSUPPORTED;
    hipStream_t st = (hipStream_t)stream;
    float* e = workspace;
    float* partial = workspace + (size_t)B * S * P;
    float* partial_b = partial + (size_t)1024 * S * C;
    const int Qp = C / 4, gs = Qp <= 16 ? 16 : Qp <= 32 ? 32 : 64, ppw = 4 * (64 / gs);
    const int gx = (int)(cdiv(P, ppw) < 1024 ? cdiv(P, ppw) : 1024);
#define DAM_HEAD_PIXEL(GS_)                                                                                                     \
    hipLaunchKernelGGL(head_bwd_pixel_kernel<GS_>, dim3(gx, B + 1), dim3(256), (size_t)S * C * sizeof(float), st, dgains, h, P, C, S, \
                       conv_w, fc_w, e, dtrunk, B, dfc_w, dfc_b)
    if (gs == 16) DAM_HEAD_PIXEL(16); else if (gs == 32) DAM_HEAD_PIXEL(32); else DAM_HEAD_PIXEL(64);
#undef DAM_HEAD_PIXEL
    DAM_CHECK_LAUNCH();
    const int Q = C / 4;
    int R = 256 / Q; if (R < 1) R = 1;
    while ((size_t)R * S * C * sizeof(float) > 60 * 1024 && R > 1) R >>= 1;
    const int64_t BP = (int64_t)B * P;
    int64_t parts = cdiv(BP, (int64_t)R * 2); if (parts > 1024) parts = 1024;
    const int64_t ppb = cdiv(BP, parts);
    parts = cdiv(BP, ppb);
    hipLaunchKernelGGL(head_bwd_cw_partial_kernel, dim3((unsigned)parts), dim3(Q * R), (size_t)R * S * C * sizeof(float), st, e,
                       trunk, B, P, C, S, Q, R, ppb, partial, partial_b);
    DAM_CHECK_LAUNCH();
    hipLaunchKernelGGL(head_bwd_cw_finalize_kernel, dim3((unsigned)cdiv((int64_t)S * C + S, 8)), dim3(256), 0, st, partial, partial_b,
                       (int)parts, C, S, dconv_w, dconv_b);
    DAM_CHECK_LAUNCH();
    return DAM_OK;
}

extern "C" int dam_masksum_fwd_f32(const float* x, const float* gains, int B, int S, int64_t FT, float* masked, void* stream) {
    if (!x || !gains || !masked || B <= 0 || FT <= 0) return DAM_ERR_BAD_ARG;
    if (S < 1 || S > MAX_STEMS || B > 65535) return DAM_ERR_UNSUPPORTED;
    const int gx = (int)(cdiv(FT, 256) < 512 ? cdiv(FT, 256) : 512);
    hipLaunchKernelGGL(masksum_fwd_kernel, dim3(gx, B), dim3(256), 0, (hipStream_t)stream, x, gains, S, FT, masked);
    DAM_CHECK_LAUNCH();
    return DAM_OK;
}

extern "C" int64_t dam_masksum_workspace_floats(int B, int S) { return (int64_t)B * 256 * (S + 1); }

extern "C" int dam_masksum_bwd_f32(const float* dmasked, const float* x, int B, int S, int64_t FT, float* dgains,
                                   float* workspace, void* stream) {
    if (!dmasked || !x || !dgains || !workspace || B <= 0 || FT <= 0) return DAM_ERR_BAD_ARG;
    if (S < 1 || S > MAX_STEMS || B > 65535) return DAM_ERR_UNSUPPORTED;
    hipStream_t st = (hipStream_t)stream;
    const int gx = (int)(cdiv(FT, 1024) < 256 ? cdiv(FT, 1024) : 256);
#define DAM_MASKSUM_GO(MODE_, G_, D_, M_)                                                                                       \
    do {                                                                                                                        \
        if (S == 8) hipLaunchKernelGGL((masksum_bwd_partial_kernel<MODE_, 8>), dim3(gx, B), dim3(256), 0, st, x, G_, D_, S, FT, M_, workspace);      \
        else if (S == 4) hipLaunchKernelGGL((masksum_bwd_partial_kernel<MODE_, 4>), dim3(gx, B), dim3(256), 0, st, x, G_, D_, S, FT, M_, workspace); \
        else if (S == 2) hipLaunchKernelGGL((masksum_bwd_partial_kernel<MODE_, 2>), dim3(gx, B), dim3(256), 0, st, x, G_, D_, S, FT, M_, workspace); \
        else hipLaunchKernelGGL((masksum_bwd_partial_kernel<MODE_, 0>), dim3(gx, B), dim3(256), 0, st, x, G_, D_, S, FT, M_, workspace);             \
    } while (0)
    DAM_MASKSUM_GO(0, (const float*)nullptr, dmasked, (float*)nullptr);
    DAM_CHECK_LAUNCH();
    hipLaunchKernelGGL(masksum_bwd_finalize_kernel, dim3(B * S), dim3(64), 0, st, workspace, B, gx, S, 1.0, 0.0,
                       dgains, (float*)nullptr);
    DAM_CHECK_LAUNCH();
    return DAM_OK;
}

extern "C" int dam_masksum_mse_f32(const float* x, const float* gains, const float* gt, int B, int S, int64_t FT,
                                   float* masked, float* loss, float* dgains, float* workspace, void* stream) {
    if (!x || !gains || !gt || !loss || !dgains || !workspace || B <= 0 || FT <= 0) return DAM_ERR_BAD_ARG;
    if (S < 1 || S > MAX_STEMS || B > 65535) return DAM_ERR_UNSUPPORTED;
    hipStream_t st = (hipStream_t)stream;
    const int gx = (int)(cdiv(FT, 1024) < 256 ? cdiv(FT, 1024) : 256);
    DAM_MASKSUM_GO(1, gains, gt, masked);
    DAM_CHECK_LAUNCH();
    const double count = (double)B * (double)FT;
    hipLaunchKernelGGL(masksum_bwd_finalize_kernel, dim3(B * S + 1), dim3(64), 0, st, workspace, B, gx, S,
                       2.0 / count, 1.0 / count, dgains, loss);
    DAM_CHECK_LAUNCH();
    return DAM_OK;
}
```

deep-audio-mixer_amd/layers.py:

```python
import torch
import torch.nn as nn

from . import ops


def _slot(p):
    return None if p is None else getattr(p, '_dam_grad', None)


class ConvSpec:

    def __init__(self, cin, cout, k, stride=1, pad=0, dil=1, in_nchw=False):
        self.cin, self.cout, self.k, self.stride, self.pad, self.dil, self.in_nchw = cin, cout, k, stride, pad, dil, in_nchw
        self.wp = self.wpt = None
        self.nhwc16 = None
        if in_nchw and k == 3 and stride == 1 and pad == 1 and dil == 1 and cin <= 16:
            self.nhwc16 = _Nhwc16Spec(self)

    def packed(self, w, transpose=False):
        cached = self.wpt if transpose else self.wp
        return cached if cached is not None else ops.pack_weights(w, transpose=transpose)

    def fwd(self, x, w, bias=None):
        return ops.conv2d_fwd(x, self.packed(w), self.cout, self.k, self.k, self.stride, self.pad, self.dil,
                              bias=bias, in_nchw=self.in_nchw)

    def fwd_conv(self, x, w, bn, training, bias=None, in_affine=None, fuse_stats=True, finalize=True):
        wp = self.packed(w)
        aff = {} if in_affine is None else dict(in_scale=in_affine[0], in_shift=in_affine[1], relu_in=True)
        if training and not self.in_nchw and fuse_stats:
            n16 = (self.cout + 15) // 16 * 16
            buf = ops.bn_partial_buffer(x.device, n16)
            c, parts, out4 = ops.conv2d_fwd(x, wp, self.cout, self.k, self.k, self.stride, self.pad, self.dil, bias=bias,
                                            bn_partial=buf, bn=_bn_args(bn, training), finalize=finalize, **aff)
            if not finalize:
                return c, ((buf, parts) if parts > 0 else None)
            return c, ((out4[0], out4[1], out4[2], out4[3]) if parts > 0 else None)
        return ops.conv2d_fwd(x, wp, self.cout, self.k, self.k, self.stride, self.pad, self.dil, bias=bias,
                              in_nchw=self.in_nchw, **aff), None

    def fwd_bn(self, x, w, bn, training, bias=None, in_affine=None):
        c, stats = self.fwd_conv(x, w, bn, training, bias=bias, in_affine=in_affine)
        return (c,) + tuple(stats if stats is not None else _bn_fwd_stats(c, bn, training))

    def fwd_bn_apply(self, x, w, bn, training, in_affine=None, res=None, res_affine=None, sign_bits=False, bias=None):
        rs, rh = res_affine if res_affine is not None else (None, None)
        if training:
            c, rec = self.fwd_conv(x, w, bn, training, bias=bias, in_affine=in_affine, finalize=False)
            rec = rec if rec is not None else ops.bn_stats_partial(c)
            (m, i, sc, sh), out = ops.bn_finalize_apply(rec[0], rec[1], _bn_args(bn, training), c, relu=True, res=res,
                                                        res_scale=rs, res_shift=rh, sign_bits=sign_bits)
            return c, m, i, sc, sh, out
        c, m, i, sc, sh = self.fwd_bn(x, w, bn, training, bias=bias, in_affine=in_affine)
        return c, m, i, sc, sh, ops.bn_apply(c, sc, sh, relu=True, res=res, res_scale=rs, res_shift=rh, sign_bits=sign_bits)

    def wgrad(self, x, dy, in_affine=None, out=None):
        aff = {} if in_affine is None else dict(in_scale=in_affine[0], in_shift=in_affine[1], relu_in=True)
        return ops.conv2d_wgrad(x, dy, self.cout, self.k, self.k, self.stride, self.pad, self.dil,
                                in_nchw=self.in_nchw, out=out, defer=out is not None, **aff)

    def dgrad(self, dy, w, hw, **kw):
        return ops.conv2d_dgrad(dy, self.packed(w, transpose=True), self.cin, hw[0], hw[1], self.k, self.k,
                                self.stride, self.pad, self.dil, **kw)


class _Nhwc16Spec(ConvSpec):

    def __init__(self, parent):
        self.cin, self.cout, self.k, self.stride, self.pad, self.dil, self.in_nchw = 16, parent.cout, 3, 1, 1, 1, False
        self.parent, self.nhwc16, self.wpt = parent, None, None

    @property
    def wp(self):
        return self.parent.wp

    def packed(self, w, transpose=False):
        return self.parent.packed(w, transpose)

    def wgrad(self, x, dy, in_affine=None, out=None):
        return ops.conv2d_wgrad(x, dy, self.cout, 3, 3, 1, 1, 1, out=out, c_real=self.parent.cin, defer=out is not None)


class WeightPacker:

    def __init__(self, pairs):
        self.pairs = list(pairs)
        self._key = None

    def _build(self):
        rows, dev = [], self.pairs[0][1].device
        L = ops._lib.lib()
        for spec, w, need_t in self.pairs:
            o, i, kh, kw = w.shape
            for transpose in ((False, True) if need_t else (False,)):
                n_out, k_in = (i, o) if transpose else (o, i)
                n = L.dam_conv_packed_weight_count(n_out, k_in, kh, kw)
                buf = torch.empty(n, dtype=torch.float32, device=dev)
                if transpose:
                    spec.wpt = buf
                else:
                    spec.wp = buf
                rows.append([w.data_ptr(), buf.data_ptr(), o, i, kh, kw, int(transpose), n])
        self.desc = torch.tensor(rows, dtype=torch.int64).to(dev)
        self.n, self.max_total = len(rows), max(r[7] for r in rows)

    def pack_all(self):
        key = tuple(w.data_ptr() for _, w, _ in self.pairs)
        if key != self._key:
            self._build()
            self._key = key
        ops.pack_weights_multi(self.desc, self.n, self.max_total)


def _bn_args(bn, training):
    mom = bn.momentum if bn.momentum is not None else 0.1
    track = training and bn.track_running_stats
    return (bn.weight, bn.bias, bn.running_mean if track else None, bn.running_var if track else None,
            bn.num_batches_tracked if track else None, mom, bn.eps)


def _bn_fwd_stats(c, bn, training):
    if training or bn.running_mean is None:
        return ops.bn_stats(c, *_bn_args(bn, training))
    return ops.bn_eval_affine(bn.weight, bn.bias, bn.running_mean, bn.running_var, bn.eps)


def _hw(x, in_nchw):
    return (x.shape[2], x.shape[3]) if in_nchw else (x.shape[1], x.shape[2])


class FoldedConvBn:

    def __init__(self, spec, conv, bn):
        self.spec, self.conv, self.bn = spec, conv, bn
        self._key = self.wp = self.bias = None

    def foldable(self):
        return self.bn.running_mean is not None and self.bn.running_var is not None

    def _tensors(self):
        bn, conv = self.bn, self.conv
        return [t for t in (conv.weight, conv.bias, bn.weight, bn.bias, bn.running_mean, bn.running_var) if t is not None]

    def get(self):
        key = (ops.PARAM_EPOCH,) + tuple((t.data_ptr(), t._version) for t in self._tensors())
        if key != self._key:
            bn, conv = self.bn, self.conv
            with torch.no_grad():
                scale = bn.weight * torch.rsqrt(bn.running_var + bn.eps)
                shift = bn.bias - bn.running_mean * scale
                if conv.bias is not None:
                    shift = shift + conv.bias * scale
                n16 = (self.spec.cout + 15) // 16 * 16
                bias = torch.zeros(n16, dtype=torch.float32, device=scale.device)
                bias[:self.spec.cout] = shift
                self.wp = ops.pack_weights(conv.weight * scale.view(-1, 1, 1, 1))
                self.bias = bias
            self._key = key
        return self.wp, self.bias

    def fwd(self, x, res=None, relu=True):
        wp, bias = self.get()
        sp = self.spec
        if sp.nhwc16 is not None:
            sp, x = sp.nhwc16, ops.nchw_to_nhwc16(x)
        return ops.conv2d_fwd(x, wp, sp.cout, sp.k, sp.k, sp.stride, sp.pad, sp.dil, bias=bias, in_nchw=sp.in_nchw,
                              res=res, relu_out=relu)


def inference_mode(module):
    return not module.training and not torch.is_grad_enabled()


UNIT_SEED = '_dam_unit_seed'


class _UpstreamBn:
    __slots__ = ('c', 'mean', 'invstd', 'scale', 'shift', 'bits', 'partials', 'dx_ptr', 'dx_version')

    def __init__(self, c, mean, invstd, scale, shift, bits=None):
        self.c, self.mean, self.invstd, self.scale, self.shift, self.bits = c, mean, invstd, scale, shift, bits
        self.partials, self.dx_ptr, self.dx_version = None, None, None

    def request(self):
        return (self.c, self.mean, self.invstd, self.scale, self.shift) + ((self.bits,) if self.bits is not None else ())

    def offer(self, sums, dx):
        self.partials, self.dx_ptr, self.dx_version = sums, dx.data_ptr(), dx._version

    def take(self, grad):
        ok = self.partials is not None and self.dx_ptr == grad.data_ptr() and self.dx_version == grad._version
        sums = self.partials if ok else None
        self.partials = None
        if sums is not None:
            _UpstreamBn.hits += 1
        return sums

    hits = 0


class ConvBnReluFn(torch.autograd.Function):

    @staticmethod
    def forward(ctx, x, w, bias, gamma, beta, spec, bn, training):
        if spec.nhwc16 is not None and not ctx.needs_input_grad[0]:
            spec, x = spec.nhwc16, ops.nchw_to_nhwc16(x)
        c, mean, invstd, scale, shift, a = spec.fwd_bn_apply(x, w.detach(), bn, training,
                                                             bias=None if bias is None else bias.detach())
        ctx.save_for_backward(x, w, c, gamma, mean, invstd, scale, shift)
        ctx.up = a._dam_upstream = _UpstreamBn(c, mean, invstd, scale, shift) if ops.DGRAD_BN_SUMS else None
        ctx.spec, ctx.training, ctx.has_bias = spec, training, bias is not None
        ctx.slots = (_slot(w), _slot(bias), _slot(gamma), _slot(beta))
        return a

    @staticmethod
    def backward(ctx, da):
        x, w, c, gamma, mean, invstd, scale, shift = ctx.saved_tensors
        spec = ctx.spec
        sw, sb, sg, sbt = ctx.slots
        da = da.contiguous()
        sums = ctx.up.take(da) if ctx.up is not None else None
        dc, dgamma, dbeta = ops.bn_backward(da, None, c, gamma, mean, invstd, ctx.training,
                                            mask_affine=(scale, shift), dgamma=sg, dbeta=sbt, partials=sums)
        dw = spec.wgrad(x, dc, out=None if sw is None else sw.view(w.shape))
        dbias = ops.channel_sum(dc, spec.cout, out=sb) if ctx.has_bias else None
        dx = spec.dgrad(dc, w, _hw(x, spec.in_nchw)) if ctx.needs_input_grad[0] else None
        return (dx, None if sw is not None else dw, None if sb is not None else dbias, None if sg is not None else dgamma,
                None if sbt is not None else dbeta, None, None, None)


class DropoutFn(torch.autograd.Function):

    @staticmethod
    def forward(ctx, x, p):
        ops.dropout_check(x.numel(), p)
        snap = ops.dropout_tick(x.device, x.numel())
        ctx.p, ctx.seed = p, torch.initial_seed()
        ctx.save_for_backward(snap)
        return ops.dropout_apply(x, p, ctx.seed, snap)

    @staticmethod
    def backward(ctx, dy):
        (snap,) = ctx.saved_tensors
        return ops.dropout_apply(dy, ctx.p, ctx.seed, snap), None


class BasicBlockFn(torch.autograd.Function):

    @staticmethod
    def forward(ctx, x, w1, g1, b1, w2, g2, b2, wsc, gsc, bsc, blk, training):
        if wsc is not None:
            bn_sc = blk.shortcut[1]
            one = None
            if (training and blk.spec1.k == 3 and blk.spec1.stride == 2 and blk.spec1.pad == 1
                    and blk.spec1.dil == 1 and blk.spec_sc.k == 1 and blk.spec_sc.stride == 2 and blk.spec_sc.pad == 0
                    and not blk.spec1.in_nchw):
                one = ops.conv_s2_pair_fwd(x, blk.spec1.packed(w1.detach()), blk.spec_sc.packed(wsc.detach()), blk.spec1.cout)
            if one is not None:
                c1, cs, (p1, p2, parts) = one
                st1, sts = ops.bn_finalize_pair(p1, p2, parts, _bn_args(blk.bn1, True), _bn_args(bn_sc, True))
            else:
                c1, st1 = blk.spec1.fwd_conv(x, w1.detach(), blk.bn1, training, fuse_stats=False)
                cs, sts = blk.spec_sc.fwd_conv(x, wsc.detach(), bn_sc, training, fuse_stats=False)
            if st1 is None and sts is None and training and c1.shape == cs.shape:
                st1, sts = ops.bn_stats_pair(c1, _bn_args(blk.bn1, True), cs, _bn_args(bn_sc, True))
            m1, i1, sc1, sh1 = st1 if st1 is not None else _bn_fwd_stats(c1, blk.bn1, training)
            ms, is_, scs, shs = sts if sts is not None else _bn_fwd_stats(cs, bn_sc, training)
            c2, m2, i2, sc2, sh2, (out, bits) = blk.spec2.fwd_bn_apply(c1, w2.detach(), blk.bn2, training, in_affine=(sc1, sh1),
                                                                       res=cs, res_affine=(scs, shs), sign_bits=True)
            ctx.save_for_backward(x, w1, g1, w2, g2, c1, c2, out, m1, i1, m2, i2, sc1, sh1, bits, wsc, gsc, cs, ms, is_)
        else:
            c1, m1, i1, sc1, sh1 = blk.spec1.fwd_bn(x, w1.detach(), blk.bn1, training)
            c2, m2, i2, sc2, sh2, (out, bits) = blk.spec2.fwd_bn_apply(c1, w2.detach(), blk.bn2, training, in_affine=(sc1, sh1),
                                                                       res=x, sign_bits=True)
            ctx.save_for_backward(x, w1, g1, w2, g2, c1, c2, out, m1, i1, m2, i2, sc1, sh1, bits)
        ctx.up_self = None
        if wsc is None and ops.DGRAD_BN_SUMS:
            ctx.up_self = out._dam_upstream = _UpstreamBn(c2, m2, i2, None, None, bits)
        ctx.blk, ctx.training, ctx.has_sc = blk, training, wsc is not None
        ctx.upstream = getattr(x, '_dam_upstream', None)
        if wsc is not None and (ctx.upstream is None or ctx.upstream.bits is None or ctx.upstream.scale is not None):
            ctx.upstream = None
        ctx.slots = tuple(_slot(p) for p in (w1, g1, b1, w2, g2, b2, wsc, gsc, bsc))
        return out

    @staticmethod
    def backward(ctx, dout):
        blk, tr = ctx.blk, ctx.training
        if ctx.has_sc:
            x, w1, g1, w2, g2, c1, c2, out, m1, i1, m2, i2, sc1, sh1, bits, wsc, gsc, cs, ms, is_ = ctx.saved_tensors
        else:
            x, w1, g1, w2, g2, c1, c2, out, m1, i1, m2, i2, sc1, sh1, bits = ctx.saved_tensors
        dout = dout.contiguous()
        hw = (x.shape[1], x.shape[2])
        s_w1, s_g1, s_b1, s_w2, s_g2, s_b2, s_ws, s_gs, s_bs = ctx.slots
        keep = lambda grad, slot: None if slot is not None else grad
        wview = lambda slot, w: None if slot is None else slot.view(w.shape)
        if ctx.has_sc:
            (dc2, dg2, db2), (dcs, dgs, dbs) = ops.bn_backward_pair(dout, None, (c2, g2, m2, i2, s_g2, s_b2),
                                                                    (cs, gsc, ms, is_, s_gs, s_bs), tr, mask_bits=bits)
        else:
            sums2 = ctx.up_self.take(dout) if ctx.up_self is not None else None
            dc2, dg2, db2 = ops.bn_backward(dout, None, c2, g2, m2, i2, tr, dgamma=s_g2, dbeta=s_b2, mask_bits=bits, partials=sums2)
        dw2 = blk.spec2.wgrad(c1, dc2, in_affine=(sc1, sh1), out=wview(s_w2, w2))
        sums = None
        if ops.DGRAD_BN_SUMS:
            da1, sums = blk.spec2.dgrad(dc2, w2, (c1.shape[1], c1.shape[2]), bn_bwd=(c1, m1, i1, sc1, sh1))
        else:
            da1 = blk.spec2.dgrad(dc2, w2, (c1.shape[1], c1.shape[2]))
        dc1, dg1, db1 = ops.bn_backward(da1, None, c1, g1, m1, i1, tr, mask_affine=(sc1, sh1),
                                        dgamma=s_g1, dbeta=s_b1, partials=sums)
        dw1 = blk.spec1.wgrad(x, dc1, out=wview(s_w1, w1))
        first = (keep(dw1, s_w1), keep(dg1, s_g1), keep(db1, s_b1), keep(dw2, s_w2), keep(dg2, s_g2), keep(db2, s_b2))
        if ctx.has_sc:
            dws = blk.spec_sc.wgrad(x, dcs, out=wview(s_ws, wsc))
            if (blk.spec1.k == 3 and blk.spec1.stride == 2 and blk.spec1.pad == 1 and blk.spec1.dil == 1
                    and blk.spec_sc.k == 1 and blk.spec_sc.stride == 2 and blk.spec_sc.pad == 0):
                up = ctx.upstream
                pair = (dcs, blk.spec_sc.packed(wsc, transpose=True))
                if up is not None and ops.DGRAD_BN_SUMS and ops.DGRAD_S2 and up.c.shape == x.shape:
                    dx, sums = blk.spec1.dgrad(dc1, w1, hw, pair_1x1=pair, bn_bwd=up.request())
                    if sums is not None:
                        up.offer(sums, dx)
                else:
                    dx = blk.spec1.dgrad(dc1, w1, hw, pair_1x1=pair)
            else:
                dx = blk.spec1.dgrad(dc1, w1, hw)
                blk.spec_sc.dgrad(dcs, wsc, hw, accumulate_into=dx)
            return (dx,) + first + (keep(dws, s_ws), keep(dgs, s_gs), keep(dbs, s_bs), None, None)
        up = ctx.upstream
        if up is not None and ops.DGRAD_BN_SUMS and up.c.shape == x.shape:
            dx, sums = blk.spec1.dgrad(dc1, w1, hw, res=dout, res_mask=out, res_mask_bits=bits, bn_bwd=up.request())
            up.offer(sums, dx)
        else:
            dx = blk.spec1.dgrad(dc1, w1, hw, res=dout, res_mask=out)
        return (dx,) + first + (None, None, None, None, None)


class HeadsFn(torch.autograd.Function):

    @staticmethod
    def forward(ctx, trunk, x, cw, cb, fw, fb):
        h, g = ops.heads_fwd(trunk, cw.detach(), cb.detach(), fw.detach(), fb.detach())
        masked = ops.masksum_fwd(x, g)
        ctx.save_for_backward(trunk, x, h, cw, fw)
        ctx.set_materialize_grads(False)
        ctx.slots = (_slot(cw), _slot(cb), _slot(fw), _slot(fb))
        return masked, g

    @staticmethod
    def backward(ctx, dmasked, dg_out):
        trunk, x, h, cw, fw = ctx.saved_tensors
        dg = None
        if dmasked is not None:
            dg = ops.masksum_bwd(dmasked.contiguous(), x)
        if dg_out is not None:
            dg = dg_out.contiguous() if dg is None else dg + dg_out
        if dg is None:
            return None, None, None, None, None, None
        dtrunk, dcw, dcb, dfw, dfb = ops.heads_bwd(dg, h, trunk, cw, fw, outs=ctx.slots)
        sl = ctx.slots
        return (dtrunk, None, None if sl[0] is not None else dcw, None if sl[1] is not None else dcb,
                None if sl[2] is not None else dfw, None if sl[3] is not None else dfb)


class HeadsMseFn(torch.autograd.Function):

    @staticmethod
    def forward(ctx, trunk, x, gt, cw, cb, fw, fb):
        h, g = ops.heads_fwd(trunk, cw.detach(), cb.detach(), fw.detach(), fb.detach())
        masked, loss, dg = ops.masksum_mse(x, g, gt.contiguous())
        ctx.save_for_backward(trunk, h, cw, fw, dg)
        ctx.mark_non_differentiable(masked, g)
        ctx.set_materialize_grads(False)
        ctx.slots = (_slot(cw), _slot(cb), _slot(fw), _slot(fb))
        return loss.reshape(()), masked, g

    @staticmethod
    def backward(ctx, dloss, _dm, _dg):
        trunk, h, cw, fw, dg = ctx.saved_tensors
        if dloss is None:
            dloss = torch.zeros((), dtype=torch.float32, device=dg.device)
        seed = dg if getattr(dloss, UNIT_SEED, False) else dg * dloss
        dtrunk, dcw, dcb, dfw, dfb = ops.heads_bwd(seed, h, trunk, cw, fw, outs=ctx.slots)
        sl = ctx.slots
        return (dtrunk, None, None, None if sl[0] is not None else dcw, None if sl[1] is not None else dcb,
                None if sl[2] is not None else dfw, None if sl[3] is not None else dfb)


class BasicBlock(nn.Module):
    expansion = 1

    def __init__(self, in_channels, out_channels, stride=1):
        super().__init__()
        self.conv1 = nn.Conv2d(in_channels, out_channels, kernel_size=3, stride=stride, padding=1, bias=False)
        self.bn1 = nn.BatchNorm2d(out_channels)
        self.conv2 = nn.Conv2d(out_channels, out_channels, kernel_size=3, stride=1, padding=1, bias=False)
        self.bn2 = nn.BatchNorm2d(out_channels)
        self.shortcut = nn.Sequential()
        if stride != 1 or in_channels != self.expansion * out_channels:
            self.shortcut = nn.Sequential(
                nn.Conv2d(in_channels, self.expansion * out_channels, kernel_size=1, stride=stride, bias=False),
                nn.BatchNorm2d(self.expansion * out_channels))
        self.spec1 = ConvSpec(in_channels, out_channels, 3, stride, 1)
        self.spec2 = ConvSpec(out_channels, out_channels, 3, 1, 1)
        self.spec_sc = ConvSpec(in_channels, out_channels, 1, stride, 0) if len(self.shortcut) else None

    def _folded(self):
        f = getattr(self, '_fold', None)
        if f is None:
            f = self._fold = (FoldedConvBn(self.spec1, self.conv1, self.bn1), FoldedConvBn(self.spec2, self.conv2, self.bn2),
                              FoldedConvBn(self.spec_sc, self.shortcut[0], self.shortcut[1]) if self.spec_sc is not None else None)
        return f

    def forward(self, x):
        if inference_mode(self):
            f1, f2, fs = self._folded()
            if f1.foldable() and f2.foldable() and (fs is None or fs.foldable()):
                a1 = f1.fwd(x)
                return f2.fwd(a1, res=x if fs is None else fs.fwd(x, relu=False))
        if self.spec_sc is not None:
            sc, sbn = self.shortcut[0], self.shortcut[1]
            return BasicBlockFn.apply(x, self.conv1.weight, self.bn1.weight, self.bn1.bias, self.conv2.weight,
                                      self.bn2.weight, self.bn2.bias, sc.weight, sbn.weight, sbn.bias, self, self.training)
        return BasicBlockFn.apply(x, self.conv1.weight, self.bn1.weight, self.bn1.bias, self.conv2.weight,
                                  self.bn2.weight, self.bn2.bias, None, None, None, self, self.training)


class ConvBlock2d(nn.Module):

    def __init__(self, in_channels, out_channels, kernel_size, stride=1, dilation=1, dropout_p=-1.0, in_nchw=False):
        super().__init__()
        self.add_padding = None
        self.conv = nn.Conv2d(in_channels=in_channels, out_channels=out_channels, kernel_size=kernel_size,
                              stride=stride, padding=0, dilation=dilation)
        self.batch_norm = nn.BatchNorm2d(num_features=out_channels, momentum=0.90, eps=0.001)
        self.activation = nn.ReLU()
        self.dropout = nn.Dropout(dropout_p) if dropout_p != -1 else None
        self.spec = ConvSpec(in_channels, out_channels, kernel_size, stride, 0, dilation, in_nchw=in_nchw)

    def forward(self, x):
        if inference_mode(self):
            f = getattr(self, '_fold', None)
            if f is None:
                f = self._fold = FoldedConvBn(self.spec, self.conv, self.batch_norm)
            if f.foldable():
                return f.fwd(x)
        out = ConvBnReluFn.apply(x, self.conv.weight, self.conv.bias, self.batch_norm.weight, self.batch_norm.bias,
                                 self.spec, self.batch_norm, self.training)
        if self.training and self.dropout:
            out = DropoutFn.apply(out, self.dropout.p) if self.dropout.p > 0 else out
        return out


class GainHeads(nn.Module):

    def __init__(self, channels, n_stems, flattened_dim):
        super().__init__()
        self.n_stems, self.channels, self.flattened_dim = n_stems, channels, flattened_dim
        cw, cb, fw, fb = [], [], [], []
        for _ in range(n_stems):
            conv, fc = nn.Conv2d(channels, 1, kernel_size=(1, 1)), nn.Linear(flattened_dim, 1)
            cw.append(conv.weight.detach().view(1, channels)), cb.append(conv.bias.detach())
            fw.append(fc.weight.detach()), fb.append(fc.bias.detach())
        self.conv_w, self.conv_b = nn.Parameter(torch.cat(cw)), nn.Parameter(torch.cat(cb))
        self.fc_w, self.fc_b = nn.Parameter(torch.cat(fw)), nn.Parameter(torch.cat(fb))

    def reference_items(self):
        for i in range(self.n_stems):
            yield 'conv_head%d.weight' % (i + 1), self.conv_w[i].view(1, self.channels, 1, 1)
            yield 'conv_head%d.bias' % (i + 1), self.conv_b[i:i + 1]
            yield 'fc_head%d.weight' % (i + 1), self.fc_w[i:i + 1]
            yield 'fc_head%d.bias' % (i + 1), self.fc_b[i:i + 1]

    def forward(self, trunk, x):
        return HeadsFn.apply(trunk, x, self.conv_w, self.conv_b, self.fc_w, self.fc_b)

    def forward_mse(self, trunk, x, gt):
        return HeadsMseFn.apply(trunk, x, gt, self.conv_w, self.conv_b, self.fc_w, self.fc_b)


class MixingNet(nn.Module):

    def _init_heads(self, channels, n_stems, flattened_dim):
        self._heads = GainHeads(channels, n_stems, flattened_dim)
        self.n_stems = n_stems
        self._register_state_dict_hook(MixingNet._sd_hook)
        self._register_load_state_dict_pre_hook(self._load_hook)

    @staticmethod
    def _sd_hook(module, state_dict, prefix, local_metadata):
        for k in ('conv_w', 'conv_b', 'fc_w', 'fc_b'):
            state_dict.pop(prefix + '_heads.' + k, None)
        for name, view in module._heads.reference_items():
            state_dict[prefix + name] = view.detach()
        return state_dict

    def _load_hook(self, state_dict, prefix, local_metadata, strict, missing_keys, unexpected_keys, error_msgs):
        h = self._heads
        parts = {}
        for i in range(h.n_stems):
            for kind in ('conv_head%d.weight', 'conv_head%d.bias', 'fc_head%d.weight', 'fc_head%d.bias'):
                key = prefix + kind % (i + 1)
                if key in state_dict:
                    parts.setdefault(kind, []).append(state_dict.pop(key))
        if not parts:
            return
        if any(len(v) != h.n_stems for v in parts.values()) or len(parts) != 4:
            error_msgs.append('incomplete per-stem head parameters in state_dict')
            return
        dev = h.conv_w.device
        state_dict[prefix + '_heads.conv_w'] = torch.cat([t.reshape(1, h.channels) for t in parts['conv_head%d.weight']]).to(dev)
        state_dict[prefix + '_heads.conv_b'] = torch.cat([t.reshape(1) for t in parts['conv_head%d.bias']]).to(dev)
        state_dict[prefix + '_heads.fc_w'] = torch.cat([t.reshape(1, -1) for t in parts['fc_head%d.weight']]).to(dev)
        state_dict[prefix + '_heads.fc_b'] = torch.cat([t.reshape(1) for t in parts['fc_head%d.bias']]).to(dev)

    def trunk(self, x, tap=None):
        raise NotImplementedError

    def ddp_late_parameters(self):
        raise NotImplementedError

    @staticmethod
    def _check_input(x):
        if x.dim() != 4:
            raise ValueError('expected x of shape [B, S, F, T]')
        if not x.is_cuda:
            raise RuntimeError('deep_audio_mixer_amd models run on the GPU only (got a %s tensor); there is no CPU '
                               'fallback' % x.device)
        if x.dtype != torch.float32:
            raise RuntimeError('expected scalar type Float but found %s' % str(x.dtype).replace('torch.', '').capitalize())
        return x.contiguous()

    @staticmethod
    def _refuse_input_grad(x):
        if x.requires_grad and torch.is_grad_enabled():
            raise RuntimeError('input gradients are not supported: x requires grad (detach it, or run under torch.no_grad())')

    def conv_pairs(self):
        return []

    def _pack_weights(self):
        if self.training:
            ops.params_changed()
        if getattr(self, '_packer', None) is None:
            pairs = self.conv_pairs()
            self._packer = WeightPacker(pairs) if pairs else False
        if self._packer:
            self._packer.pack_all()

    def forward(self, x):
        x = self._check_input(x)
        self._refuse_input_grad(x)
        self._pack_weights()
        masked, g = self._heads(self.trunk(x), x)
        return masked, tuple(g[:, s:s + 1] for s in range(self.n_stems))

    def predict_gains(self, x):
        x = self._check_input(x)
        self._pack_weights()
        with torch.no_grad():
            h = self._heads
            return ops.heads_fwd(self.trunk(x), h.conv_w, h.conv_b, h.fc_w, h.fc_b)[1]

    def forward_mse(self, x, gt, tap=None):
        x = self._check_input(x)
        self._refuse_input_grad(x)
        self._pack_weights()
        loss, masked, g = self._heads.forward_mse(self.trunk(x) if tap is None else self.trunk(x, tap), x, gt)
        return loss, masked, tuple(g[:, s:s + 1] for s in range(self.n_stems))
```

deep-audio-mixer_amd/models/model_resnet.py:

```python
import torch.nn as nn
import torch.nn.functional as F

from ..layers import BasicBlock, ConvBnReluFn, ConvSpec, FoldedConvBn, MixingNet, inference_mode
from ..ops import conv_out_size

__all__ = ['BasicBlock', 'ResNet', 'ResNet18']


def _trunk_hw(f, t, strides):
    for s in strides:
        if s != 1:
            f, t = conv_out_size(f, 3, s, 1), conv_out_size(t, 3, s, 1)
    return f, t


class ResNet(MixingNet):
    def __init__(self, block, num_blocks, *, n_stems=4, input_shape=(1025, 216)):
        super().__init__()
        self.in_planes = 16
        self.conv1 = nn.Conv2d(n_stems, 16, kernel_size=3, stride=1, padding=1, bias=False)
        self.bn1 = nn.BatchNorm2d(16)
        self._stem = ConvSpec(n_stems, 16, 3, 1, 1, in_nchw=True)
        widths, strides = (16, 32, 64, 96, 128, 256), (1, 2, 2, 2, 2, 2)
        for i, (w, s, n) in enumerate(zip(widths, strides, num_blocks), start=1):
            setattr(self, 'layer%d' % i, self._make_layer(block, w, n, stride=s))
        fh, ft = _trunk_hw(input_shape[0], input_shape[1], strides)
        flattened_dim = fh * ft
        self._init_heads(256 * block.expansion, n_stems, flattened_dim)

    def _make_layer(self, block, planes, num_blocks, stride):
        layers = []
        for s in [stride] + [1] * (num_blocks - 1):
            layers.append(block(self.in_planes, planes, s))
            self.in_planes = planes * block.expansion
        return nn.Sequential(*layers)

    def conv_pairs(self):
        pairs = [(self._stem, self.conv1.weight, False)]
        for i in range(1, 7):
            for blk in getattr(self, 'layer%d' % i):
                pairs += [(blk.spec1, blk.conv1.weight, True), (blk.spec2, blk.conv2.weight, True)]
                if blk.spec_sc is not None:
                    pairs.append((blk.spec_sc, blk.shortcut[0].weight, True))
        return pairs

    DDP_BOUNDARY = 4

    def trunk(self, x, tap=None):
        stem = getattr(self, '_stem_fold', None)
        if stem is None:
            stem = self._stem_fold = FoldedConvBn(self._stem, self.conv1, self.bn1)
        if inference_mode(self) and stem.foldable():
            out = stem.fwd(x)
        else:
            out = ConvBnReluFn.apply(x, self.conv1.weight, None, self.bn1.weight, self.bn1.bias, self._stem, self.bn1,
                                     self.training)
        for i in range(1, 7):
            out = getattr(self, 'layer%d' % i)(out)
            if tap is not None and i == self.DDP_BOUNDARY:
                tap.append(out)
        return out

    def ddp_late_parameters(self):
        late = []
        for i in range(self.DDP_BOUNDARY + 1, 7):
            late += list(getattr(self, 'layer%d' % i).parameters())
        return late + list(self._heads.parameters())


def ResNet18(**kwargs):
    return ResNet(BasicBlock, [2, 2, 2, 2, 2, 2], **kwargs)
```

deep-audio-mixer_amd/ops.py:

```python
import ctypes
import os

import torch

from . import _lib


def _f32c(t, name):
    if t is None:
        return None
    if t.dtype != torch.float32 or not t.is_contiguous():
        raise ValueError('%s must be a contiguous float32 tensor' % name)
    return t


def conv_out_size(n, k, stride=1, pad=0, dil=1):
    return (n + 2 * pad - dil * (k - 1) - 1) // stride + 1


def pack_weights(w, transpose=False, out=None):
    _lib.require_cuda(w)
    w = _f32c(w.detach(), 'weight')
    o, i, kh, kw = w.shape
    n_out, k_in = (i, o) if transpose else (o, i)
    n = _lib.lib().dam_conv_packed_weight_count(n_out, k_in, kh, kw)
    if out is None:
        out = torch.empty(n, dtype=torch.float32, device=w.device)
    _lib.check(_lib.lib().dam_conv_pack_weights_f32(_lib.ptr(w), o, i, kh, kw, 1 if transpose else 0,
                                                    _lib.ptr(out), _lib.stream()), 'dam_conv_pack_weights_f32')
    return out


def pack_weights_multi(desc, n_tensors, max_total):
    _lib.check(_lib.lib().dam_conv_pack_weights_multi_f32(_lib.ptr(desc), n_tensors, max_total, _lib.stream()),
               'dam_conv_pack_weights_multi_f32')


DGRAD_S2 = not os.environ.get('DAM_NO_DGRAD_S2')
dgrad_s2_launches = 0
DGRAD_BN_SUMS = not os.environ.get('DAM_NO_DGRAD_SUMS')


def _bn_fin_struct(bn, out4):
    gamma, beta, rm, rv, nbt, mom, eps = bn
    return _lib.BnFin(_lib.ptr(gamma), _lib.ptr(beta), _lib.ptr(rm), _lib.ptr(rv), _lib.ptr(nbt), float(mom), float(eps),
                      _lib.ptr(out4[0]), _lib.ptr(out4[1]), _lib.ptr(out4[2]), _lib.ptr(out4[3]))


def _tapgrid(x, B, H, W, C, in_nchw, wp, k_chunks, n_out, bias, in_scale, in_shift, relu_in, y, OHt, OWt, Ho, Wo,
             out_stride, oo_h, oo_w, in_stride, nA, nB, off_h, step_h, off_w, step_w, wt_base, wt_sa, wt_sb,
             res=None, res_mask=None, bn_partial=None, relu_out=False, batch=None, bn_bwd=None):
    parts = ctypes.c_int(0)
    ws = _workspace(y.device, min(8 * y.numel(), 8 * 400 * 64 * 64))
    st = _lib.lib().dam_conv2d_tapgrid_f32(
        _lib.ptr(x), B, H, W, C, 1 if in_nchw else 0, _lib.ptr(wp), k_chunks, n_out, _lib.ptr(bias),
        _lib.ptr(in_scale), _lib.ptr(in_shift), 1 if relu_in else 0, 1 if relu_out else 0, _lib.ptr(y), OHt, OWt, Ho, Wo,
        out_stride,
        oo_h, oo_w, in_stride, nA, nB, off_h, step_h, off_w, step_w, wt_base, wt_sa, wt_sb, _lib.ptr(res),
        _lib.ptr(res_mask), _lib.ptr(bn_partial), ctypes.byref(parts) if bn_partial is not None else None,
        ctypes.byref(bn_bwd) if bn_bwd is not None else None,
        _lib.ptr(ws), ws.numel(),
        ctypes.addressof(batch) if batch is not None else None, _lib.stream())
    _lib.check(st, 'dam_conv2d_tapgrid_f32')
    return parts.value


def conv2d_fwd(x, wp, n_out, kh, kw, stride=1, pad=0, dil=1, bias=None, in_scale=None, in_shift=None,
               relu_in=False, in_nchw=False, bn_partial=None, bn=None, res=None, relu_out=False, finalize=True):
    _lib.require_cuda(x, wp)
    _f32c(x, 'x'), _f32c(bias, 'bias'), _f32c(in_scale, 'in_scale'), _f32c(in_shift, 'in_shift'), _f32c(res, 'res')
    if in_nchw:
        B, C, H, W = x.shape
        k_chunks = 1
    else:
        B, H, W, C = x.shape
        k_chunks = C // 16
    n16 = (n_out + 15) // 16 * 16
    Ho, Wo = conv_out_size(H, kh, stride, pad, dil), conv_out_size(W, kw, stride, pad, dil)
    if Ho <= 0 or Wo <= 0:
        raise ValueError('convolution output would be empty')
    y = torch.empty((B, Ho, Wo, n16), dtype=torch.float32, device=x.device)
    parts = _tapgrid(x, B, H, W, C, in_nchw, wp, k_chunks, n16, bias, in_scale, in_shift, relu_in, y, Ho, Wo, Ho, Wo,
                     1, 0, 0, stride, kh, kw, -pad, dil, -pad, dil, 0, kw, 1, res=res, bn_partial=bn_partial,
                     relu_out=relu_out)
    if bn is not None and bn_partial is not None:
        out4 = bn_finalize(bn_partial, parts, *bn) if parts > 0 and finalize else None
        return y, parts, out4
    if bn_partial is not None:
        return y, parts
    return y


def _dgrad_axis(parity, pad, dil, k, stride):
    valid = [t for t in range(k) if (parity + pad - t * dil) % stride == 0]
    if not valid:
        return None
    k0 = valid[0]
    kstep = valid[1] - valid[0] if len(valid) > 1 else 1
    return len(valid), k0, kstep, (parity + pad - k0 * dil) // stride, -(kstep * dil) // stride


def conv2d_dgrad(dy, wpt, n_in, H, W, kh, kw, stride=1, pad=0, dil=1, res=None, res_mask=None, accumulate_into=None,
                 bn_bwd=None, res_mask_bits=None, pair_1x1=None, _s2_sums=None):
    _lib.require_cuda(dy, wpt)
    if bn_bwd is not None and stride == 2:
        if accumulate_into is not None or res is not None or len(bn_bwd) < 6 or bn_bwd[5] is None or bn_bwd[3] is not None:
            raise ValueError('bn_bwd at stride 2: mask as sign bytes, no residual / accumulation')
        xb, mean, invstd, up_bits = bn_bwd[0], bn_bwd[1], bn_bwd[2], bn_bwd[5]
        _lib.require_cuda(xb)
        n16 = (n_in + 15) // 16 * 16
        if tuple(xb.shape) != (dy.shape[0], H, W, n16):
            raise ValueError('bn_bwd: x has the shape of the data gradient')
        rec = torch.empty(_lib.lib().dam_bn_workspace_floats(n16), dtype=torch.float32, device=dy.device)
        epi = _lib.BnBwdSums(_lib.ptr(xb), _lib.ptr(mean), _lib.ptr(invstd), None, None, None, _lib.ptr(up_bits))
        got = conv2d_dgrad(dy, wpt, n_in, H, W, kh, kw, stride, pad, dil, pair_1x1=pair_1x1, _s2_sums=(epi, rec))
        return got if isinstance(got, tuple) else (got, None)
    if bn_bwd is not None:
        if stride != 1 or accumulate_into is not None:
            raise ValueError('bn_bwd: stride-1 data gradients only')
        if res is not None and (res_mask is None or res_mask_bits is None):
            raise ValueError('bn_bwd with a residual: res_mask and res_mask_bits')
        _f32c(dy, 'dy'), _f32c(res, 'res'), _f32c(res_mask, 'res_mask')
        xb, mean, invstd, msc, msh = bn_bwd[:5]
        up_bits = bn_bwd[5] if len(bn_bwd) > 5 else None
        if (up_bits is None) == (msc is None) or (up_bits is not None and res is None):
            raise ValueError('bn_bwd: the mask as (scale, shift) or -- with a residual -- as sign bytes')
        _lib.require_cuda(xb)
        B, Ho, Wo, Co = dy.shape
        n16 = (n_in + 15) // 16 * 16
        if tuple(xb.shape) != (B, H, W, n16):
            raise ValueError('bn_bwd: x has the shape of the data gradient')
        dx = torch.empty((B, H, W, n16), dtype=torch.float32, device=dy.device)
        rec = torch.empty(_lib.lib().dam_bn_workspace_floats(n16), dtype=torch.float32, device=dy.device)
        epi = _lib.BnBwdSums(_lib.ptr(xb), _lib.ptr(mean), _lib.ptr(invstd), _lib.ptr(msc), _lib.ptr(msh), _lib.ptr(res_mask_bits),
                             _lib.ptr(up_bits))
        parts = _tapgrid(dy, B, Ho, Wo, Co, False, wpt, Co // 16, n16, None, None, None, False, dx, H, W, H, W, 1, 0, 0, 1,
                         kh, kw, pad, -dil, pad, -dil, 0, kw, 1, res, res_mask, bn_partial=rec, bn_bwd=epi)
        return dx, ((rec, parts) if parts > 0 else None)
    _f32c(dy, 'dy'), _f32c(res, 'res'), _f32c(res_mask, 'res_mask')
    B, Ho, Wo, Co = dy.shape
    n16 = (n_in + 15) // 16 * 16
    if accumulate_into is not None:
        dx, res, res_mask = accumulate_into, accumulate_into, None
    else:
        dx = torch.empty((B, H, W, n16), dtype=torch.float32, device=dy.device)
    if stride == 1:
        _tapgrid(dy, B, Ho, Wo, Co, False, wpt, Co // 16, n16, None, None, None, False, dx, H, W, H, W, 1, 0, 0, 1,
                 kh, kw, pad, -dil, pad, -dil, 0, kw, 1, res, res_mask)
        return dx
    if pair_1x1 is not None:
        dy2, wpt2 = pair_1x1
        _lib.require_cuda(dy2, wpt2)
        _f32c(dy2, 'pair dy')
        if accumulate_into is not None or res is not None or tuple(dy2.shape) != tuple(dy.shape):
            raise ValueError('pair_1x1: a second gradient of the same shape, no residual / accumulation')
        a0 = _dgrad_axis(0, pad, dil, kh, stride), _dgrad_axis(0, pad, dil, kw, stride)
        if a0[0] is None or a0[1] is None or a0[0][0] != 1 or a0[1][0] != 1 or a0[0][3] != 0 or a0[1][3] != 0:
            raise ValueError('pair_1x1: class (0, 0) of this operator is not a single tap at offset 0')
    if (DGRAD_S2 and stride == 2 and kh == 3 and kw == 3 and pad == 1 and dil == 1 and accumulate_into is None and res is None
            and Ho == (H + 1) // 2 and Wo == (W + 1) // 2):
        parts = ctypes.c_int(0)
        st = _lib.lib().dam_dgrad_s2_3x3_f32(_lib.ptr(dy), _lib.ptr(wpt), _lib.ptr(pair_1x1[0]) if pair_1x1 else None,
                                             _lib.ptr(pair_1x1[1]) if pair_1x1 else None, B, Ho, Wo, Co, n16, _lib.ptr(dx), H, W,
                                             ctypes.byref(_s2_sums[0]) if _s2_sums else None,
                                             _lib.ptr(_s2_sums[1]) if _s2_sums else None, ctypes.byref(parts) if _s2_sums else None,
                                             _lib.stream())
        if st == 0:
            global dgrad_s2_launches
            dgrad_s2_launches += 1
            if _s2_sums:
                return dx, ((_s2_sums[1], parts.value) if parts.value > 0 else None)
            return dx
        if st != -2:
            _lib.check(st, 'dam_dgrad_s2_3x3_f32')
    classes = [(_dgrad_axis(ph, pad, dil, kh, stride), _dgrad_axis(pw, pad, dil, kw, stride))
               for ph in range(stride) for pw in range(stride)]
    if any(a is None or b is None for a, b in classes) and accumulate_into is None:
        if res is not None:
            raise ValueError('a fused residual needs every output parity class to receive taps')
        dx.zero_()
    batch = _conv_batch(dy.device)
    try:
        for ph in range(stride):
            for pw in range(stride):
                ah, aw = _dgrad_axis(ph, pad, dil, kh, stride), _dgrad_axis(pw, pad, dil, kw, stride)
                nh, nw = (H - ph + stride - 1) // stride, (W - pw + stride - 1) // stride
                if nh <= 0 or nw <= 0 or ah is None or aw is None:
                    continue
                if pair_1x1 is not None and ph == 0 and pw == 0:
                    if nh != Ho or nw != Wo:
                        raise ValueError('pair_1x1: class (0, 0) does not cover the gradient\'s pixels')
                    _lib.check(_lib.lib().dam_conv1x1_pair_f32(_lib.ptr(dy), _lib.ptr(wpt), ah[1] * kw + aw[1], _lib.ptr(pair_1x1[0]),
                                                               _lib.ptr(pair_1x1[1]), 0, B, Ho, Wo, Co, n16, _lib.ptr(dx), H, W, stride,
                                                               0, 0, _lib.stream()), 'dam_conv1x1_pair_f32')
                    continue
                _tapgrid(dy, B, Ho, Wo, Co, False, wpt, Co // 16, n16, None, None, None, False, dx, H, W, nh, nw,
                         stride, ph, pw, 1, ah[0], aw[0], ah[3], ah[4], aw[3], aw[4], ah[1] * kw + aw[1],
                         ah[2] * kw, aw[2], res, res_mask, batch=batch)
        _lib.check(_lib.lib().dam_conv_batch_flush(ctypes.addressof(batch), _lib.stream()), 'dam_conv_batch_flush')
    except Exception:
        _lib.lib().dam_conv_batch_init(ctypes.addressof(batch))
        raise
    return dx


_conv_batches = {}


def _conv_batch(device):
    key = (device.type, device.index)
    b = _conv_batches.get(key)
    if b is None:
        L = _lib.lib()
        b = _conv_batches[key] = ctypes.create_string_buffer(int(L.dam_conv_batch_bytes()))
        _lib.check(L.dam_conv_batch_init(ctypes.addressof(b)), 'dam_conv_batch_init')
    return b


_workspaces = {}
_retired = []


def _grow(table, key, device, floats):
    ws = table.get(key)
    if ws is None or ws.numel() < floats:
        if ws is not None:
            _retired.append(ws)
        ws = torch.empty(int(floats), dtype=torch.float32, device=device)
        table[key] = ws
    return ws


def _workspace(device, floats):
    return _grow(_workspaces, (device.type, device.index), device, floats)


PARAM_EPOCH = 0


def params_changed():
    global PARAM_EPOCH
    PARAM_EPOCH += 1


WGRAD_BATCH = True
_wgrad_queues = {}


def _wgrad_queue(device):
    key = (device.type, device.index)
    q = _wgrad_queues.get(key)
    if q is None:
        L = _lib.lib()
        buf = ctypes.create_string_buffer(int(L.dam_wgrad_queue_bytes()))
        _lib.check(L.dam_wgrad_queue_init(ctypes.addressof(buf)), 'dam_wgrad_queue_init')
        _lib.check(L.dam_wgrad_queue_set_batching(ctypes.addressof(buf), int(WGRAD_BATCH)), 'dam_wgrad_queue_set_batching')
        q = _wgrad_queues[key] = [buf, 0, []]
    return q


def wgrad_abandon(device=None):
    for key, q in _wgrad_queues.items():
        if q[1] and (device is None or key == (device.type, device.index)):
            _lib.check(_lib.lib().dam_wgrad_queue_init(ctypes.addressof(q[0])), 'dam_wgrad_queue_init')
            del q[2][:]
            q[1] = 0


def wgrad_flush(device=None):
    for key, q in _wgrad_queues.items():
        if q[1] and (device is None or key == (device.type, device.index)):
            _lib.check(_lib.lib().dam_wgrad_queue_flush(ctypes.addressof(q[0]), _lib.stream()), 'dam_wgrad_queue_flush')
            q[1] = 0
            del q[2][:]


def conv2d_wgrad(x, dy, n_out, kh, kw, stride=1, pad=0, dil=1, in_scale=None, in_shift=None, relu_in=False,
                 in_nchw=False, out=None, c_real=None, defer=False):
    _lib.require_cuda(x, dy)
    _f32c(x, 'x'), _f32c(dy, 'dy')
    if in_nchw:
        B, C, H, W = x.shape
    else:
        B, H, W, C = x.shape
    _, Ho, Wo, n_chan = dy.shape
    L = _lib.lib()
    floats = L.dam_conv2d_wgrad_workspace_floats(n_out, C, kh, kw)
    cr = C if c_real is None else int(c_real)
    if out is None:
        if defer:
            raise ValueError('a deferred weight gradient needs the buffer it will be written to')
        out = torch.empty((n_out, cr, kh, kw), dtype=torch.float32, device=x.device)
    elif out.numel() != n_out * cr * kh * kw or not out.is_contiguous() or out.dtype != torch.float32:
        raise ValueError('bad out tensor for the weight gradient')
    if defer:
        q = _wgrad_queue(x.device)
        ws = _grow(_workspaces, (x.device.type, x.device.index, 'wgrad slabs', q[1]), x.device, floats)
        q[1] += 1
        q[2].append((x, dy, in_scale, in_shift))
        queue = ctypes.addressof(q[0])
    else:
        ws, queue = _workspace(x.device, floats), None
    _lib.check(L.dam_conv2d_wgrad_f32(_lib.ptr(x), B, H, W, C, 1 if in_nchw else 0, _lib.ptr(in_scale),
                                      _lib.ptr(in_shift), 1 if relu_in else 0, _lib.ptr(dy), Ho, Wo, n_chan, n_out,
                                      kh, kw, stride, pad, dil, _lib.ptr(out), cr, _lib.ptr(ws), ws.numel(), queue,
                                      _lib.stream()), 'dam_conv2d_wgrad_f32')
    return out


def nchw_to_nhwc16(x):
    _lib.require_cuda(x)
    _f32c(x, 'x')
    B, C, H, W = x.shape
    y = torch.empty((B, H, W, 16), dtype=torch.float32, device=x.device)
    _lib.check(_lib.lib().dam_nchw_to_nhwc16_f32(_lib.ptr(x), B, C, H * W, _lib.ptr(y), _lib.stream()), 'dam_nchw_to_nhwc16_f32')
    return y


def _bn_ws(device, C):
    return _workspace(device, _lib.lib().dam_bn_workspace_floats(C))


_bn_partials = {}


def bn_stats(x, gamma, beta, running_mean, running_var, num_batches_tracked, momentum, eps):
    _lib.require_cuda(x)
    C = x.shape[-1]
    P = x.numel() // C
    out = torch.empty((4, C), dtype=torch.float32, device=x.device)
    ws = _bn_ws(x.device, C)
    _lib.check(_lib.lib().dam_bn_stats_f32(_lib.ptr(x), P, C, _lib.ptr(gamma), _lib.ptr(beta), _lib.ptr(running_mean),
                                           _lib.ptr(running_var), _lib.ptr(num_batches_tracked), float(momentum), float(eps),
                                           _lib.ptr(out[0]), _lib.ptr(out[1]), _lib.ptr(out[2]), _lib.ptr(out[3]),
                                           _lib.ptr(ws), _lib.stream()), 'dam_bn_stats_f32')
    return out[0], out[1], out[2], out[3]


def bn_stats_partial(x):
    _lib.require_cuda(x)
    C = x.shape[-1]
    ws = bn_partial_buffer(x.device, C)
    parts = ctypes.c_int(0)
    _lib.check(_lib.lib().dam_bn_stats_partial_f32(_lib.ptr(x), x.numel() // C, C, _lib.ptr(ws), ctypes.byref(parts), _lib.stream()),
               'dam_bn_stats_partial_f32')
    return ws, parts.value


def bn_finalize_apply(partial, parts, bn, x, relu=True, res=None, res_scale=None, res_shift=None, sign_bits=False):
    _lib.require_cuda(partial, x)
    C = x.shape[-1]
    out4 = torch.empty((4, C), dtype=torch.float32, device=x.device)
    fin = _bn_fin_struct(bn, out4)
    y = torch.empty_like(x)
    bits = torch.empty(x.shape[:-1] + (C // 4,), dtype=torch.uint8, device=x.device) if sign_bits else None
    _lib.check(_lib.lib().dam_bn_finalize_apply_f32(_lib.ptr(partial), int(parts), C, ctypes.byref(fin), _lib.ptr(x), x.numel() // C,
                                                    _lib.ptr(res), _lib.ptr(res_scale), _lib.ptr(res_shift), 1 if relu else 0,
                                                    _lib.ptr(y), _lib.ptr(bits), _lib.stream()), 'dam_bn_finalize_apply_f32')
    return (out4[0], out4[1], out4[2], out4[3]), ((y, bits) if sign_bits else y)


def bn_partial_buffer(device, C):
    return _grow(_bn_partials, (device.type, device.index, C), device, _lib.lib().dam_bn_workspace_floats(C))


def bn_stats_pair(xa, bn_a, xb, bn_b):
    _lib.require_cuda(xa, xb)
    if xa.shape != xb.shape:
        raise ValueError('the two tensors of a pair have the same shape')
    C = xa.shape[-1]
    L = _lib.lib()
    outs = [torch.empty((4, C), dtype=torch.float32, device=xa.device) for _ in range(2)]
    fa, fb = _bn_fin_struct(bn_a, outs[0]), _bn_fin_struct(bn_b, outs[1])
    ws = _workspace(xa.device, 2 * L.dam_bn_workspace_floats(C))
    _lib.check(L.dam_bn_stats_pair_f32(_lib.ptr(xa), _lib.ptr(xb), xa.numel() // C, C, ctypes.byref(fa), ctypes.byref(fb),
                                       _lib.ptr(ws), _lib.stream()), 'dam_bn_stats_pair_f32')
    return tuple(outs[0]), tuple(outs[1])


def conv_s2_pair_fwd(x, wp, wp_sc, n_out, stats=True):
    _lib.require_cuda(x, wp, wp_sc)
    _f32c(x, 'x')
    B, H, W, C = x.shape
    n16 = (n_out + 15) // 16 * 16
    Hd, Wd = (H + 1) // 2, (W + 1) // 2
    c1 = torch.empty((B, Hd, Wd, n16), dtype=torch.float32, device=x.device)
    cs = torch.empty_like(c1)
    p1 = p2 = None
    parts = ctypes.c_int(0)
    if stats:
        n = _lib.lib().dam_bn_workspace_floats(n16)
        p1 = torch.empty(n, dtype=torch.float32, device=x.device)
        p2 = torch.empty(n, dtype=torch.float32, device=x.device)
    st = _lib.lib().dam_conv_s2_pair_fwd_f32(_lib.ptr(x), _lib.ptr(wp), _lib.ptr(wp_sc), B, H, W, C, n16, _lib.ptr(c1), _lib.ptr(cs),
                                             _lib.ptr(p1), _lib.ptr(p2), ctypes.byref(parts), _lib.stream())
    if st == -2:
        return None
    _lib.check(st, 'dam_conv_s2_pair_fwd_f32')
    return c1, cs, ((p1, p2, parts.value) if stats else None)


def bn_finalize_pair(partial_a, partial_b, parts, bn_a, bn_b):
    C = bn_a[0].numel()
    outs = [torch.empty((4, C), dtype=torch.float32, device=partial_a.device) for _ in range(2)]
    fa, fb = _bn_fin_struct(bn_a, outs[0]), _bn_fin_struct(bn_b, outs[1])
    _lib.check(_lib.lib().dam_bn_finalize_pair_f32(_lib.ptr(partial_a), _lib.ptr(partial_b), parts, C, ctypes.byref(fa),
                                                   ctypes.byref(fb), _lib.stream()), 'dam_bn_finalize_pair_f32')
    return tuple(outs[0]), tuple(outs[1])


def bn_finalize(partial, parts, gamma, beta, running_mean, running_var, num_batches_tracked, momentum, eps):
    C = gamma.numel()
    out = torch.empty((4, C), dtype=torch.float32, device=gamma.device)
    _lib.check(_lib.lib().dam_bn_finalize_f32(_lib.ptr(partial), parts, C, _lib.ptr(gamma), _lib.ptr(beta),
                                              _lib.ptr(running_mean), _lib.ptr(running_var), _lib.ptr(num_batches_tracked),
                                              float(momentum), float(eps), _lib.ptr(out[0]), _lib.ptr(out[1]), _lib.ptr(out[2]),
                                              _lib.ptr(out[3]), _lib.stream()), 'dam_bn_finalize_f32')
    return out[0], out[1], out[2], out[3]


def bn_eval_affine(gamma, beta, running_mean, running_var, eps):
    _lib.require_cuda(gamma)
    C = gamma.numel()
    out = torch.empty((4, C), dtype=torch.float32, device=gamma.device)
    _lib.check(_lib.lib().dam_bn_eval_affine_f32(C, _lib.ptr(gamma), _lib.ptr(beta), _lib.ptr(running_mean),
                                                 _lib.ptr(running_var), float(eps), _lib.ptr(out[0]), _lib.ptr(out[1]),
                                                 _lib.ptr(out[2]), _lib.ptr(out[3]), _lib.stream()), 'dam_bn_eval_affine_f32')
    return out[0], out[1], out[2], out[3]


def bn_apply(x, scale, shift, relu=True, res=None, res_scale=None, res_shift=None, sign_bits=False):
    _lib.require_cuda(x)
    C = x.shape[-1]
    y = torch.empty_like(x)
    bits = torch.empty(x.shape[:-1] + (C // 4,), dtype=torch.uint8, device=x.device) if sign_bits else None
    _lib.check(_lib.lib().dam_bn_apply_f32(_lib.ptr(x), x.numel() // C, C, _lib.ptr(scale), _lib.ptr(shift), _lib.ptr(res),
                                           _lib.ptr(res_scale), _lib.ptr(res_shift), 1 if relu else 0, _lib.ptr(y),
                                           _lib.ptr(bits), _lib.stream()), 'dam_bn_apply_f32')
    return (y, bits) if sign_bits else y


def bn_backward_pair(dy, y_mask, a, b, training=True, mask_bits=None):
    _lib.require_cuda(dy, a[0], b[0])
    if (y_mask is None) == (mask_bits is None):
        raise ValueError('exactly one of y_mask / mask_bits')
    C = a[0].shape[-1]
    if b[0].shape != a[0].shape or dy.shape != a[0].shape:
        raise ValueError('the two BatchNorms of a pair see the same shape')
    outs = []
    for x, gamma, mean, invstd, dgamma, dbeta in (a, b):
        dx = torch.empty_like(x)
        dgamma = torch.empty(C, dtype=torch.float32, device=x.device) if dgamma is None else dgamma
        dbeta = torch.empty(C, dtype=torch.float32, device=x.device) if dbeta is None else dbeta
        outs.append((dx, dgamma, dbeta))
    L = _lib.lib()
    ws = _workspace(dy.device, L.dam_bn_pair_workspace_floats(C))
    args = []
    for (x, gamma, mean, invstd, _, _), (dx, dgamma, dbeta) in zip((a, b), outs):
        args += [_lib.ptr(x), _lib.ptr(gamma), _lib.ptr(mean), _lib.ptr(invstd), _lib.ptr(dx), _lib.ptr(dgamma), _lib.ptr(dbeta)]
    _lib.check(L.dam_bn_backward_pair_f32(_lib.ptr(dy), _lib.ptr(y_mask), _lib.ptr(mask_bits), dy.numel() // C, C,
                                          1 if training else 0, *args,
                                          _lib.ptr(ws), _lib.stream()), 'dam_bn_backward_pair_f32')
    return outs[0], outs[1]


def bn_backward(dy, y_mask, x, gamma, save_mean, save_invstd, training=True, mask_affine=None, dgamma=None, dbeta=None,
                mask_bits=None, partials=None):
    _lib.require_cuda(dy, x)
    C = x.shape[-1]
    dx = torch.empty_like(x)
    if dgamma is None:
        dgamma = torch.empty(C, dtype=torch.float32, device=x.device)
    if dbeta is None:
        dbeta = torch.empty(C, dtype=torch.float32, device=x.device)
    ws, given = (_bn_ws(x.device, C), 0) if partials is None else partials
    _lib.check(_lib.lib().dam_bn_backward_f32(_lib.ptr(dy), _lib.ptr(y_mask), _lib.ptr(x), x.numel() // C, C, _lib.ptr(gamma),
                                              _lib.ptr(save_mean), _lib.ptr(save_invstd), 1 if training else 0,
                                              _lib.ptr(mask_affine[0]) if mask_affine else None,
                                              _lib.ptr(mask_affine[1]) if mask_affine else None, _lib.ptr(mask_bits), _lib.ptr(dx),
                                              _lib.ptr(dgamma), _lib.ptr(dbeta), _lib.ptr(ws), given, _lib.stream()),
               'dam_bn_backward_f32')
    return dx, dgamma, dbeta


def channel_sum(x, n_real, out=None):
    _lib.require_cuda(x)
    C = x.shape[-1]
    if out is None:
        out = torch.empty(n_real, dtype=torch.float32, device=x.device)
    ws = _bn_ws(x.device, C)
    _lib.check(_lib.lib().dam_channel_sum_f32(_lib.ptr(x), x.numel() // C, C, n_real, _lib.ptr(out), _lib.ptr(ws),
                                              _lib.stream()), 'dam_channel_sum_f32')
    return out


def heads_fwd(trunk, conv_w, conv_b, fc_w, fc_b):
    _lib.require_cuda(trunk)
    B, C = trunk.shape[0], trunk.shape[-1]
    P = trunk.numel() // (B * C)
    S = conv_w.shape[0]
    if fc_w.shape != (S, P):
        raise ValueError('fc_head expects %d inputs but the trunk gives %d (flattened_dim mismatch)' % (fc_w.shape[1], P))
    h = torch.empty((B, S, P), dtype=torch.float32, device=trunk.device)
    g = torch.empty((B, S), dtype=torch.float32, device=trunk.device)
    _lib.check(_lib.lib().dam_heads_fwd_f32(_lib.ptr(trunk), B, P, C, S, _lib.ptr(conv_w), _lib.ptr(conv_b), _lib.ptr(fc_w),
                                            _lib.ptr(fc_b), _lib.ptr(h), _lib.ptr(g), _lib.stream()), 'dam_heads_fwd_f32')
    return h, g


def heads_bwd(dgains, h, trunk, conv_w, fc_w, outs=None):
    B, S, P = h.shape
    C = trunk.shape[-1]
    dev = trunk.device
    dtrunk = torch.empty_like(trunk)
    o = outs or (None, None, None, None)
    dcw = o[0] if o[0] is not None else torch.empty((S, C), dtype=torch.float32, device=dev)
    dcb = o[1] if o[1] is not None else torch.empty(S, dtype=torch.float32, device=dev)
    dfw = o[2] if o[2] is not None else torch.empty((S, P), dtype=torch.float32, device=dev)
    dfb = o[3] if o[3] is not None else torch.empty(S, dtype=torch.float32, device=dev)
    L = _lib.lib()
    ws = _workspace(dev, L.dam_heads_bwd_workspace_floats(B, P, C, S))
    _lib.check(L.dam_heads_bwd_f32(_lib.ptr(dgains), _lib.ptr(h), _lib.ptr(trunk), B, P, C, S, _lib.ptr(conv_w), _lib.ptr(fc_w),
                                   _lib.ptr(dtrunk), _lib.ptr(dcw), _lib.ptr(dcb), _lib.ptr(dfw), _lib.ptr(dfb), _lib.ptr(ws),
                                   _lib.stream()), 'dam_heads_bwd_f32')
    return dtrunk, dcw, dcb, dfw, dfb


def masksum_fwd(x, gains):
    _lib.require_cuda(x, gains)
    B, S, F, T = x.shape
    masked = torch.empty((B, F, T), dtype=torch.float32, device=x.device)
    _lib.check(_lib.lib().dam_masksum_fwd_f32(_lib.ptr(x), _lib.ptr(gains), B, S, F * T, _lib.ptr(masked), _lib.stream()),
               'dam_masksum_fwd_f32')
    return masked


def masksum_bwd(dmasked, x):
    B, S, F, T = x.shape
    dg = torch.empty((B, S), dtype=torch.float32, device=x.device)
    L = _lib.lib()
    ws = _workspace(x.device, L.dam_masksum_workspace_floats(B, S))
    _lib.check(L.dam_masksum_bwd_f32(_lib.ptr(dmasked), _lib.ptr(x), B, S, F * T, _lib.ptr(dg), _lib.ptr(ws), _lib.stream()),
               'dam_masksum_bwd_f32')
    return dg


def masksum_mse(x, gains, gt, want_masked=True):
    _lib.require_cuda(x, gains, gt)
    B, S, F, T = x.shape
    dev = x.device
    masked = torch.empty((B, F, T), dtype=torch.float32, device=dev) if want_masked else None
    loss = torch.empty(1, dtype=torch.float32, device=dev)
    dg = torch.empty((B, S), dtype=torch.float32, device=dev)
    L = _lib.lib()
    ws = _workspace(dev, L.dam_masksum_workspace_floats(B, S))
    _lib.check(L.dam_masksum_mse_f32(_lib.ptr(x), _lib.ptr(gains), _lib.ptr(gt), B, S, F * T, _lib.ptr(masked), _lib.ptr(loss),
                                     _lib.ptr(dg), _lib.ptr(ws), _lib.stream()), 'dam_masksum_mse_f32')
    return masked, loss, dg


def adam_l2_step(params, grads, exp_avg, exp_avg_sq, step, derived, lr, beta1, beta2, eps, weight_decay, grad_scale=1.0,
                 hyper=None):
    _lib.require_cuda(params, grads, hyper)
    _lib.check(_lib.lib().dam_adam_l2_step_f32(_lib.ptr(params), _lib.ptr(grads), _lib.ptr(exp_avg), _lib.ptr(exp_avg_sq),
                                               params.numel(), _lib.ptr(step), _lib.ptr(derived), float(lr), float(beta1),
                                               float(beta2), float(eps), float(weight_decay), float(grad_scale),
                                               _lib.ptr(hyper), _lib.stream()), 'dam_adam_l2_step_f32')


def digest64(t, out=None, index_base=0, accumulate=False, max_blocks=0):
    _lib.require_cuda(t, out)
    if t.element_size() != 4 or not t.is_contiguous():
        raise ValueError('digest64: a contiguous tensor of 4-byte elements expected (got %s, contiguous=%s)'
                         % (t.dtype, t.is_contiguous()))
    if out is None:
        out = torch.empty(1, dtype=torch.int64, device=t.device)
    elif out.dtype != torch.int64 or out.numel() != 1 or not out.is_contiguous():
        raise ValueError('digest64: out must be a contiguous int64 tensor of one element')
    _lib.check(_lib.lib().dam_digest64_u32(_lib.ptr(t) if t.numel() else None, t.numel(), int(index_base), int(max_blocks),
                                           int(bool(accumulate)), _lib.ptr(out), _lib.stream()), 'dam_digest64_u32')
    return out


def _audio_kind(t, what):
    if t.dtype not in (torch.float32, torch.float64):
        raise TypeError('%s must be float32 or float64' % what)
    return 1 if t.dtype == torch.float64 else 0


def gain_ramp_arg(gains, N, n):
    if gains is None:
        return None, 0
    if gains.dtype != torch.float64:
        raise TypeError('gains must be float64')
    gains = gains.reshape(N, -1).contiguous()
    if not 1 <= gains.shape[1] <= n:
        raise ValueError('between one gain and one gain per sample expected')
    return gains, gains.shape[1]


def gains_smooth(raw_db, window, polyorder=2, out=None, want_f32=False):
    _lib.require_cuda(raw_db, out)
    raw_db = _f32c(raw_db, 'raw_db')
    n, S = raw_db.shape
    if window % 2 == 0 or window <= polyorder or window > n:
        raise ValueError('savgol_filter needs an odd window with polyorder < window <= len(x): window=%d polyorder=%d '
                         'len=%d' % (window, polyorder, n))
    if out is None:
        out = torch.empty((2, S, n), dtype=torch.float64, device=raw_db.device)
    elif tuple(out.shape) != (2, S, n) or out.dtype != torch.float64 or not out.is_contiguous():
        raise ValueError('bad out tensor')
    s32 = torch.empty((S, n), dtype=torch.float32, device=raw_db.device) if want_f32 else None
    _lib.check(_lib.lib().dam_gains_smooth(_lib.ptr(raw_db), n, S, window, polyorder, _lib.ptr(out[0]), _lib.ptr(out[1]),
                                           _lib.ptr(s32), _lib.stream()), 'dam_gains_smooth')
    return (out[0], out[1], s32) if want_f32 else (out[0], out[1])


def gain_ramp_apply(audio, gains, out=None, out_dtype=None):
    _lib.require_cuda(audio, gains, out)
    ak = _audio_kind(audio, 'audio')
    if gains.dtype != torch.float64:
        raise TypeError('gains must be float64')
    audio, gains = audio.contiguous(), gains.contiguous()
    if audio.dim() == 2:
        rpg, rows, n = audio.shape[0], audio.shape[0], audio.shape[1]
        n_gains = gains.numel()
    else:
        G, rpg, n = audio.shape
        rows, n_gains = G * rpg, gains.shape[-1]
        if gains.numel() != G * n_gains:
            raise ValueError('one gain sequence per leading index expected')
    if out is None:
        out = torch.empty(audio.shape, dtype=out_dtype or torch.float64, device=audio.device)
    elif out.shape != audio.shape or not out.is_contiguous():
        raise ValueError('bad out tensor')
    _lib.check(_lib.lib().dam_gain_ramp_apply(_lib.ptr(audio), ak, _lib.ptr(gains), rows, rpg, n, n_gains, _lib.ptr(out),
                                              _audio_kind(out, 'out'), _lib.stream()), 'dam_gain_ramp_apply')
    return out


def mixdown_peak_normalize(audio, gains, normalize=True, out=None, out_dtype=None, workspace=None):
    _lib.require_cuda(audio, gains, out)
    ak = _audio_kind(audio, 'audio')
    if gains.dtype != torch.float64:
        raise TypeError('gains must be float64')
    audio, gains = audio.contiguous(), gains.contiguous()
    S, rows, n = audio.shape
    if out is None:
        out = torch.empty((rows, n), dtype=out_dtype or torch.float64, device=audio.device)
    L = _lib.lib()
    if workspace is None:
        workspace = torch.empty(L.dam_mixdown_workspace_elems(rows), dtype=out.dtype, device=audio.device)
    _lib.check(L.dam_mixdown_peak_normalize(_lib.ptr(audio), ak, _lib.ptr(gains), S, rows, n, gains.shape[1],
                                            1 if normalize else 0, _lib.ptr(out), _audio_kind(out, 'out'),
                                            _lib.ptr(workspace), _lib.stream()), 'dam_mixdown_peak_normalize')
    return out


PCM_FORMATS = {'PCM_16': (0, 2), 'PCM_24': (1, 3), 'PCM_32': (2, 4), 'FLOAT': (3, 4)}
PCM_MAX_CHANNELS = 8


def pcm_grid_frames(dtype):
    L = _lib.lib()
    return L.dam_pcm_tile_frames(1 if dtype in (torch.float64, 'float64') else 0) * L.dam_pcm_max_blocks()


def pcm_encode(x, subtype, scale=None, dither_seed=None, out=None, clip_count=None):
    _lib.require_cuda(x, scale, out, clip_count)
    if subtype not in PCM_FORMATS:
        raise ValueError('pcm_encode: subtype must be one of %s, got %r' % (sorted(PCM_FORMATS), subtype))
    fmt, width = PCM_FORMATS[subtype]
    xk = _audio_kind(x, 'x')
    if x.dim() == 1:
        x = x.unsqueeze(0)
    if x.dim() != 2 or not x.is_contiguous():
        raise ValueError('pcm_encode: a contiguous [channels, n] tensor expected (got shape %s, contiguous=%s)'
                         % (tuple(x.shape), x.is_contiguous()))
    ch, n = x.shape
    if not 1 <= ch <= PCM_MAX_CHANNELS or n < 1:
        raise ValueError('pcm_encode: 1..%d channels and at least one frame expected, got [%d, %d]' % (PCM_MAX_CHANNELS, ch, n))
    n_scale = 0
    if scale is not None:
        if scale.dtype != torch.float64 or not scale.is_contiguous() or scale.numel() not in (1, ch):
            raise ValueError('pcm_encode: scale must be a contiguous float64 tensor of 1 or %d elements' % ch)
        n_scale = scale.numel()
    if out is None:
        out = torch.empty(n * ch * width, dtype=torch.uint8, device=x.device)
    elif out.dtype != torch.uint8 or out.numel() != n * ch * width or not out.is_contiguous():
        raise ValueError('pcm_encode: out must be a contiguous uint8 tensor of %d elements' % (n * ch * width))
    if clip_count is not None and (clip_count.dtype != torch.int64 or clip_count.numel() != ch or not clip_count.is_contiguous()):
        raise ValueError('pcm_encode: clip_count must be a contiguous int64 tensor of %d elements' % ch)
    seed = 0 if dither_seed is None else int(dither_seed) & 0xFFFFFFFFFFFFFFFF
    _lib.check(_lib.lib().dam_pcm_encode(_lib.ptr(x), xk, ch, n, _lib.ptr(scale), n_scale, fmt,
                                         0 if dither_seed is None else 1, seed, _lib.ptr(out), _lib.ptr(clip_count),
                                         _lib.stream()), 'dam_pcm_encode')
    return out


def true_peak_geometry():
    L = _lib.lib()
    return L.dam_true_peak_tile_samples(), L.dam_true_peak_max_blocks()


def true_peak_batch(data, gains=None, out=None, sample_peak_out=None):
    _lib.require_cuda(data, gains, out, sample_peak_out)
    xk = _audio_kind(data, 'data')
    if data.dim() != 3:
        raise ValueError('true_peak_batch: [tracks, samples, channels] expected, got shape %s' % (tuple(data.shape),))
    N, n, ch = data.shape
    if N < 1 or n < 1 or ch < 1 or N * ch > 65535:
        raise ValueError('true_peak_batch: at least one track, sample and channel and at most 65535 rows expected, got %s'
                         % (tuple(data.shape),))
    gains, n_gains = gain_ramp_arg(gains, N, n)
    dev = data.device
    if out is None:
        out = torch.empty((N, ch), dtype=torch.float64, device=dev)
    for o in (out, sample_peak_out):
        if o is not None and (tuple(o.shape) != (N, ch) or o.dtype != torch.float64 or not o.is_contiguous()):
            raise ValueError('true_peak_batch: outputs must be contiguous float64 [%d, %d] tensors' % (N, ch))
    L = _lib.lib()
    ws = torch.empty(L.dam_true_peak_workspace_bytes(N, n, ch) // 8, dtype=torch.float64, device=dev)
    with torch.cuda.device(dev):
        _lib.check(L.dam_true_peak_batch(_lib.ptr(data), xk, N, n, ch, data.stride(0), data.stride(1), data.stride(2),
                                         _lib.ptr(gains), n_gains, _lib.ptr(sample_peak_out), _lib.ptr(out), _lib.ptr(ws),
                                         _lib.stream()), 'dam_true_peak_batch')
    return out


def peak_limit_gains(gains, peaks, ceiling_db):
    _lib.require_cuda(gains, peaks)
    if gains.dtype != torch.float64 or peaks.dtype != torch.float64 or not gains.is_contiguous():
        raise TypeError('peak_limit_gains: a contiguous float64 gains tensor and float64 peaks expected')
    G = gains.numel()
    if G < 1 or peaks.numel() < G or peaks.numel() % G:
        raise ValueError('peak_limit_gains: %d peaks do not divide among %d gains' % (peaks.numel(), G))
    peaks = peaks.contiguous()
    with torch.cuda.device(gains.device):
        _lib.check(_lib.lib().dam_peak_limit_gains(_lib.ptr(gains), _lib.ptr(peaks), G, peaks.numel() // G,
                                                   float(10.0 ** (float(ceiling_db) / 20.0)), _lib.stream()),
                   'dam_peak_limit_gains')
    return gains


_dropout_counters = {}


def _dropout_counter(device):
    device = torch.device(device)
    key = (device.type, torch.cuda.current_device() if device.index is None else device.index)
    if key not in _dropout_counters:
        _dropout_counters[key] = torch.zeros(1, dtype=torch.int64, device=device)
    return _dropout_counters[key]


def dropout_counter(device):
    return int(_dropout_counter(device).item())


def set_dropout_counter(device, value):
    _dropout_counter(device).fill_(int(value))


def dropout_check(n, p):
    if n <= 0 or n % 4:
        raise ValueError('dropout: the element count must be a positive multiple of 4, got %d' % n)
    if not 0.0 <= p < 1.0:
        raise ValueError('dropout: p must lie in [0, 1), got %r' % (p,))


def dropout_tick(device, n):
    counter = _dropout_counter(device)
    snap = torch.empty(1, dtype=torch.int64, device=device)
    _lib.check(_lib.lib().dam_dropout_tick(_lib.ptr(counter), n, _lib.ptr(snap), _lib.stream()), 'dam_dropout_tick')
    return snap


def dropout_apply(x, p, seed, snapshot):
    _lib.require_cuda(x, snapshot)
    x = x.contiguous()
    y = torch.empty_like(x)
    _lib.check(_lib.lib().dam_dropout_apply_f32(_lib.ptr(x), x.numel(), float(p), int(seed) & 0xFFFFFFFFFFFFFFFF, _lib.ptr(snapshot),
                                                _lib.ptr(y), _lib.stream()), 'dam_dropout_apply_f32')
    return y
```

include/dam_hip.h:

```cpp
#ifndef DAM_HIP_H
#define DAM_HIP_H

#include <stdint.h>

#ifdef __cplusplus
extern "C" {
#endif

typedef enum dam_status {
    DAM_OK = 0,
    DAM_ERR_BAD_ARG = -1,
    DAM_ERR_UNSUPPORTED = -2,
    DAM_ERR_LAUNCH = -3,
    DAM_ERR_WORKSPACE = -4
} dam_status;

typedef enum dam_pcm_dtype { DAM_PCM_F32 = 0, DAM_PCM_F64 = 1, DAM_PCM_S16 = 2, DAM_PCM_S32 = 3 } dam_pcm_dtype;
#define DAM_PCM_INDIRECT 0x100
#define DAM_PCM_ROTATE 0x200
struct dam_bn_bwd_sums;

#define DAM_ABI_VERSION 22
const char* dam_arch(void);
int dam_abi_version(void);

int dam_host_dontfork_pinned(int64_t* n_mappings_host, int64_t* n_bytes_host);

int dam_step_mark_create(void** mark_host);
int dam_step_mark_record(void* mark, void* stream);
int dam_step_mark_wait(void* mark, void* stream);
int dam_step_mark_synchronize(void* mark);
int dam_step_mark_destroy(void* mark);


int64_t dam_stft_twiddle_count(int n_fft);
int dam_stft_fill_twiddles_host(int n_fft, float* table_host );

int dam_stft_logmag_f32(const void* pcm, int pcm_dtype, int64_t n_tracks, int64_t n_samples, int channels,
                        int64_t pcm_track_stride, const float* window, const float* twiddles,
                        const float* gain, int n_fft, int hop, float amin, int normalize,
                        float* out, void* stream);

int dam_stft_logmag_strided_f32(const void* pcm, int pcm_dtype, int64_t n_outer, int64_t outer_stride, int64_t n_inner,
                                int64_t inner_stride, int64_t n_samples, int channels, int64_t sample_stride,
                                int64_t channel_stride, const float* window, const float* twiddles, const float* gain,
                                int n_fft, int hop, float amin, int normalize, float* out, float* out_tail, int n_tail,
                                void* stream);

int dam_stft_complex_f32(const void* pcm, int pcm_dtype, int64_t n_tracks, int64_t n_samples, int channels,
                         int64_t pcm_track_stride, int64_t n_sum, int64_t sum_stride, const float* window,
                         const float* twiddles, const float* gain, int n_fft, int hop, float* out, void* stream);
int dam_stft_complex_strided_f32(const void* pcm, int pcm_dtype, int64_t n_outer, int64_t outer_stride, int64_t n_inner,
                                 int64_t inner_stride, int64_t n_sum, int64_t sum_stride, int64_t n_samples, int channels,
                                 int64_t sample_stride, int64_t channel_stride, const float* window, const float* twiddles,
                                 const float* gain, int n_fft, int hop, float* out, void* stream);
int64_t dam_istft_workspace_bytes(int64_t n_tracks, int64_t n_frames, int n_fft, int hop, int64_t length);
int dam_istft_f32(const float* spec, const float* mag_db, int64_t n_tracks, int64_t n_frames, int n_fft, int hop,
                  int64_t length, const float* window, const float* twiddles, float* out, void* workspace,
                  int64_t workspace_bytes, void* stream);

int dam_augment_gains_f32(uint64_t seed, const int64_t* items, int64_t first_item, int n_items, int n_tracks,
                          float lo, float hi, float* gains, void* stream);


int64_t dam_conv_packed_weight_count(int n_out, int k_in, int kh, int kw);

int dam_conv_pack_weights_f32(const float* w_oihw, int O, int I, int KH, int KW, int transpose,
                              float* packed, void* stream);

int dam_conv_pack_weights_multi_f32(const int64_t* desc_dev, int n_tensors, int64_t max_total, void* stream);

int dam_conv2d_tapgrid_f32(const float* x, int B, int H, int W, int C, int in_nchw, const float* w_packed,
                           int k_chunks, int n_out, const float* bias, const float* in_scale,
                           const float* in_shift, int relu_in, int relu_out, float* y, int OHt, int OWt, int Ho, int Wo,
                           int out_stride, int out_off_h, int out_off_w, int in_stride, int nA, int nB,
                           int off_h, int step_h, int off_w, int step_w, int wt_base, int wt_sa, int wt_sb,
                           const float* res, const float* res_mask, float* bn_partial, int* bn_parts_host,
                           const struct dam_bn_bwd_sums* bn_bwd, float* workspace, int64_t workspace_floats,
                           void* batch, void* stream);

int dam_conv1x1_pair_f32(const float* x1, const float* w1_packed, int tap1, const float* x2, const float* w2_packed, int tap2,
                         int B, int H, int W, int C, int n_out, float* y, int OHt, int OWt, int out_stride, int out_off_h,
                         int out_off_w, void* stream);

int dam_dgrad_s2_3x3_f32(const float* dy, const float* w_packed_t, const float* dy_pair, const float* w_pair_packed_t, int B,
                         int Hd, int Wd, int Co, int Ci, float* dx, int H, int W, const struct dam_bn_bwd_sums* bn_bwd,
                         float* bn_partial, int* bn_parts_host, void* stream);

int dam_conv_s2_pair_fwd_f32(const float* x, const float* w_packed, const float* wsc_packed, int B, int H, int W, int Ci, int Co,
                             float* y, float* ysc, float* partial, float* partial_sc, int* parts_host, void* stream);

int64_t dam_conv_batch_bytes(void);
int dam_conv_batch_init(void* batch);
int dam_conv_batch_flush(void* batch, void* stream);

int64_t dam_conv2d_wgrad_workspace_floats(int n_out, int c_in, int kh, int kw);
int dam_conv2d_wgrad_f32(const float* x, int B, int H, int W, int C, int in_nchw, const float* in_scale,
                         const float* in_shift, int relu_in, const float* dy, int Ho, int Wo, int n_chan,
                         int n_out, int kh, int kw, int stride, int pad, int dil, float* dw, int c_real,
                         float* workspace, int64_t workspace_floats, void* reduce_queue, void* stream);

int64_t dam_wgrad_queue_bytes(void);
int dam_wgrad_queue_init(void* queue);
int dam_wgrad_queue_pending(const void* queue);
int dam_wgrad_queue_flush(void* queue, void* stream);
int dam_wgrad_queue_set_batching(void* queue, int on);

int dam_strip_diag_counters(uint32_t* out2_host, int reset);

int64_t dam_bn_workspace_floats(int C);

typedef struct dam_bn_fin {
    const float* gamma; const float* beta;
    float* running_mean; float* running_var; int64_t* num_batches_tracked;
    float momentum, eps;
    float* save_mean; float* save_invstd; float* scale; float* shift;
} dam_bn_fin;

typedef struct dam_bn_bwd_sums {
    const float* x; const float* mean; const float* invstd; const float* mask_scale; const float* mask_shift;
    const uint8_t* res_mask_bits;
    const uint8_t* mask_bits;
} dam_bn_bwd_sums;

int dam_bn_stats_f32(const float* x, int64_t n_pixels, int C, const float* gamma, const float* beta,
                     float* running_mean, float* running_var, int64_t* num_batches_tracked,
                     float momentum, float eps, float* save_mean, float* save_invstd, float* scale,
                     float* shift, float* workspace, void* stream);

int dam_bn_stats_pair_f32(const float* x_a, const float* x_b, int64_t n_pixels, int C, const struct dam_bn_fin* a,
                          const struct dam_bn_fin* b, float* workspace, void* stream);

int dam_bn_finalize_f32(const float* partial, int parts, int C, const float* gamma, const float* beta,
                        float* running_mean, float* running_var, int64_t* num_batches_tracked,
                        float momentum, float eps, float* save_mean, float* save_invstd, float* scale,
                        float* shift, void* stream);

int dam_bn_finalize_pair_f32(const float* partial_a, const float* partial_b, int parts, int C, const struct dam_bn_fin* a,
                             const struct dam_bn_fin* b, void* stream);

int dam_bn_stats_partial_f32(const float* x, int64_t n_pixels, int C, float* workspace, int* parts_host, void* stream);

int dam_bn_finalize_apply_f32(const float* partial, int parts, int C, const struct dam_bn_fin* fin, const float* x,
                              int64_t n_pixels, const float* res, const float* res_scale, const float* res_shift, int relu,
                              float* y, uint8_t* sign_bits, void* stream);

int dam_bn_eval_affine_f32(int C, const float* gamma, const float* beta, const float* running_mean,
                           const float* running_var, float eps, float* save_mean, float* save_invstd,
                           float* scale, float* shift, void* stream);

int dam_bn_apply_f32(const float* x, int64_t n_pixels, int C, const float* scale, const float* shift,
                     const float* res, const float* res_scale, const float* res_shift, int relu, float* y,
                     uint8_t* sign_bits, void* stream);

int dam_bn_backward_f32(const float* dy, const float* y_mask, const float* x, int64_t n_pixels, int C,
                        const float* gamma, const float* save_mean, const float* save_invstd, int training,
                        const float* mask_scale, const float* mask_shift, const uint8_t* mask_bits, float* dx,
                        float* dgamma, float* dbeta, float* workspace, int partials_given, void* stream);

int64_t dam_bn_pair_workspace_floats(int C);
int dam_bn_backward_pair_f32(const float* dy, const float* y_mask, const uint8_t* mask_bits, int64_t n_pixels, int C,
                             int training,
                             const float* x_a, const float* gamma_a, const float* mean_a, const float* invstd_a,
                             float* dx_a, float* dgamma_a, float* dbeta_a,
                             const float* x_b, const float* gamma_b, const float* mean_b, const float* invstd_b,
                             float* dx_b, float* dgamma_b, float* dbeta_b, float* workspace, void* stream);

int dam_channel_sum_f32(const float* x, int64_t n_pixels, int C, int n_real, float* out, float* workspace,
                        void* stream);

int dam_dropout_tick(int64_t* counter, int64_t n, int64_t* snapshot, void* stream);
int dam_dropout_apply_f32(const float* x, int64_t n, float p, uint64_t seed, const int64_t* snapshot, float* y,
                          void* stream);

int dam_heads_fwd_f32(const float* trunk, int B, int P, int C, int S, const float* conv_w, const float* conv_b,
                      const float* fc_w, const float* fc_b, float* h, float* gains, void* stream);
int64_t dam_heads_bwd_workspace_floats(int B, int P, int C, int S);
int dam_heads_bwd_f32(const float* dgains, const float* h, const float* trunk, int B, int P, int C, int S,
                      const float* conv_w, const float* fc_w, float* dtrunk, float* dconv_w, float* dconv_b,
                      float* dfc_w, float* dfc_b, float* workspace, void* stream);
int dam_masksum_fwd_f32(const float* x, const float* gains, int B, int S, int64_t FT, float* masked, void* stream);
int64_t dam_masksum_workspace_floats(int B, int S);
int dam_masksum_bwd_f32(const float* dmasked, const float* x, int B, int S, int64_t FT, float* dgains,
                        float* workspace, void* stream);
int dam_masksum_mse_f32(const float* x, const float* gains, const float* gt, int B, int S, int64_t FT,
                        float* masked, float* loss, float* dgains, float* workspace, void* stream);

int dam_adam_l2_step_f32(float* params, const float* grads, float* exp_avg, float* exp_avg_sq, int64_t n,
                         int64_t* step, float* derived2, float lr, float beta1, float beta2, float eps,
                         float weight_decay, float grad_scale, const float* hyper_dev, void* stream);

int dam_digest64_u32(const uint32_t* x, int64_t n, int64_t index_base, int max_blocks, int accumulate, uint64_t* out,
                     void* stream);


int dam_gains_smooth(const float* raw_db, int n_chunks, int n_stems, int window, int polyorder, double* amp,
                     double* smooth, float* smooth_f32, void* stream);

int dam_gain_ramp_apply(const void* audio, int audio_is_f64, const double* gains, int64_t rows, int64_t rows_per_gain,
                        int64_t n_samples, int n_gains, void* out, int out_is_f64, void* stream);

int64_t dam_mixdown_workspace_elems(int64_t rows);
int dam_mixdown_peak_normalize(const void* audio, int audio_is_f64, const double* gains, int n_stems, int64_t rows,
                               int64_t n_samples, int n_gains, int normalize, void* mix, int mix_is_f64,
                               void* workspace, void* stream);

int dam_loudness_kweight_coeffs(double rate, double* coef12);
int64_t dam_loudness_workspace_bytes(int64_t n_samples, int channels);
int dam_loudness_block_energy(const void* x, int x_is_f64, int64_t n_samples, int channels, int64_t sample_stride,
                              int64_t channel_stride, const double* coef12_host, const int64_t* blk_lo,
                              const int64_t* blk_hi, int n_blocks, double block_len, double* z, void* workspace,
                              void* stream);
int64_t dam_loudness_batch_workspace_bytes(int n_tracks, int64_t n_samples, int channels, int n_blocks);
int dam_loudness_block_energy_batch(const void* x, int x_is_f64, int n_tracks, int64_t n_samples, int channels,
                                    int64_t track_stride, int64_t sample_stride, int64_t channel_stride,
                                    const double* gains, int n_gains, const double* coef12_host, const int64_t* blk_lo,
                                    const int64_t* blk_hi, int n_blocks, double block_len, double* z, void* workspace,
                                    void* stream);
int dam_loudness_gate(const double* z, int n_tracks, int channels, int n_blocks, double* lufs, void* stream);
int dam_loudness_target_gains(const double* lufs, const double* target, int n, double* gains, void* stream);

typedef enum dam_wav_format { DAM_WAV_S16 = 0, DAM_WAV_S24 = 1, DAM_WAV_S32 = 2, DAM_WAV_F32 = 3 } dam_wav_format;
#define DAM_PCM_MAX_CHANNELS 8
#define DAM_PCM_MAX_BLOCKS 2048
int64_t dam_pcm_tile_frames(int x_is_f64);
int dam_pcm_max_blocks(void);
int dam_pcm_encode(const void* x, int x_is_f64, int channels, int64_t n_samples, const double* scale, int n_scale,
                   int format, int dither, uint64_t seed, void* out, int64_t* clip_count, void* stream);

int dam_true_peak_taps_host(double* h49);
int64_t dam_true_peak_tile_samples(void);
int dam_true_peak_max_blocks(void);
int64_t dam_true_peak_workspace_bytes(int n_tracks, int64_t n_samples, int channels);
int dam_true_peak_batch(const void* x, int x_is_f64, int n_tracks, int64_t n_samples, int channels, int64_t track_stride,
                        int64_t sample_stride, int64_t channel_stride, const double* gains, int n_gains,
                        double* sample_peak, double* true_peak, void* workspace, void* stream);
int dam_peak_limit_gains(double* gains, const double* peaks, int n_gains, int peaks_per_gain, double ceiling_lin,
                         void* stream);

#define DAM_LOUDNESS_ABS_GATE_POWER 0x1.f791ec6e1d5b7p-24
int dam_loudness_window_power(const double* e, int n_tracks, int channels, int n_hops, int w, double* power, double* lufs,
                              void* stream);
int dam_loudness_curve_stats(const double* power, int n_tracks, int n_windows, double* out, void* stream);
int dam_loudness_profile_error(const double* ref_lufs, const double* cand_lufs, int n_variants, int n_stems,
                               int n_windows, double* err, double* active, void* stream);

int dam_nchw_to_nhwc16_f32(const float* x, int B, int C, int64_t HW, float* y, void* stream);

#ifdef __cplusplus
}
#endif
#endif
```

Measured before the change: 2.033 million stem-spectrogram-frames/s.

## Fuse head conv+fc kernels and defer stem BN-ReLU into first residual block

Adds fused forward and backward kernels for the per-stem heads. The forward computes the 1x1 conv, ReLU and FC reduction in one launch, and the backward merges the dtrunk, dconv and dfc computations into one kernel plus a finalize pass, selected below a P threshold. It also adds a residual-ReLU flag to the BN apply kernels, so the stem's BN+ReLU output can be handed lazily as an affine to the first residual block and never materialised. This removes kernel launches and one full activation read/write pass, at the cost of more complex control flow and new fallback paths.

```diff
diff --git a/deep-audio-mixer_amd/_lib.py b/deep-audio-mixer_amd/_lib.py
--- a/deep-audio-mixer_amd/_lib.py
+++ b/deep-audio-mixer_amd/_lib.py
@@ -7,7 +7,7 @@
 _HERE = os.path.dirname(os.path.abspath(__file__))
 LIB_PATH = os.environ.get('DAM_LIB_PATH') or os.path.join(_HERE, 'libdam_hip.so')
 
-EXPECTED_ABI = 22
+EXPECTED_ABI = 23
 
 _STATUS = {0: 'DAM_OK', -1: 'DAM_ERR_BAD_ARG', -2: 'DAM_ERR_UNSUPPORTED', -3: 'DAM_ERR_LAUNCH',
            -4: 'DAM_ERR_WORKSPACE'}
@@ -71,6 +71,8 @@
     'dam_dropout_tick': (c_i, [c_p, c_i64, c_p, c_p]),
     'dam_dropout_apply_f32': (c_i, [c_p, c_i64, c_f, ctypes.c_uint64, c_p, c_p, c_p]),
     'dam_heads_fwd_f32': (c_i, [c_p, c_i, c_i, c_i, c_i, c_p, c_p, c_p, c_p, c_p, c_p, c_p]),
+    'dam_heads_fwd_fused_f32': (c_i, [c_p, c_i, c_i, c_i, c_i, c_p, c_p, c_p, c_p, c_p, c_p, c_p]),
+    'dam_heads_bwd_fused_f32': (c_i, [c_p, c_p, c_p, c_i, c_i, c_i, c_i, c_p, c_p, c_p, c_p, c_p, c_p, c_p, c_p, c_p]),
     'dam_heads_bwd_workspace_floats': (c_i64, [c_i, c_i, c_i, c_i]),
     'dam_heads_bwd_f32': (c_i, [c_p, c_p, c_p, c_i, c_i, c_i, c_i, c_p, c_p, c_p, c_p, c_p, c_p, c_p, c_p, c_p]),
     'dam_masksum_fwd_f32': (c_i, [c_p, c_p, c_i, c_i, c_i64, c_p, c_p]),
diff --git a/deep-audio-mixer_amd/csrc/dam_bn.hip b/deep-audio-mixer_amd/csrc/dam_bn.hip
--- a/deep-audio-mixer_amd/csrc/dam_bn.hip
+++ b/deep-audio-mixer_amd/csrc/dam_bn.hip
@@ -197,6 +197,9 @@
     shift[c] = beta[c] - running_mean[c] * sc;
 }
 
+constexpr int BN_RELU_OUT = 1, BN_RELU_RES = 2;
+__device__ __forceinline__ float4 relu4(float4 v) { return make_float4(fmaxf(v.x, 0.f), fmaxf(v.y, 0.f), fmaxf(v.z, 0.f), fmaxf(v.w, 0.f)); }
+
 __global__ void bn_apply_kernel(const float* __restrict__ x, int64_t nquads, int Q, const float* __restrict__ scale,
                                 const float* __restrict__ shift, const float* __restrict__ res,
                                 const float* __restrict__ rscale, const float* __restrict__ rshift, int relu,
@@ -211,10 +214,11 @@
             if (rscale) {
                 const float4 a = reinterpret_cast<const float4*>(rscale)[cq], b = reinterpret_cast<const float4*>(rshift)[cq];
                 r = make_float4(fmaf(r.x, a.x, b.x), fmaf(r.y, a.y, b.y), fmaf(r.z, a.z, b.z), fmaf(r.w, a.w, b.w));
+                if (relu & BN_RELU_RES) r = relu4(r);
             }
             o.x += r.x; o.y += r.y; o.z += r.z; o.w += r.w;
         }
-        if (relu) { o.x = fmaxf(o.x, 0.f); o.y = fmaxf(o.y, 0.f); o.z = fmaxf(o.z, 0.f); o.w = fmaxf(o.w, 0.f); }
+        if (relu & BN_RELU_OUT) { o.x = fmaxf(o.x, 0.f); o.y = fmaxf(o.y, 0.f); o.z = fmaxf(o.z, 0.f); o.w = fmaxf(o.w, 0.f); }
         reinterpret_cast<float4*>(y)[e] = o;
         if (sign_bits) sign_bits[e] = (unsigned char)((o.x > 0.f) | ((o.y > 0.f) << 1) | ((o.z > 0.f) << 2) | ((o.w > 0.f) << 3));
     }
@@ -546,9 +550,10 @@
                 if (res) {
                     float4 r = rv[S][u];
                     if (rscale) r = make_float4(fmaf(r.x, ra.x, rb.x), fmaf(r.y, ra.y, rb.y), fmaf(r.z, ra.z, rb.z), fmaf(r.w, ra.w, rb.w));
+                    if (relu & BN_RELU_RES) r = relu4(r);
                     o.x += r.x; o.y += r.y; o.z += r.z; o.w += r.w;
                 }
-                if (relu) { o.x = fmaxf(o.x, 0.f); o.y = fmaxf(o.y, 0.f); o.z = fmaxf(o.z, 0.f); o.w = fmaxf(o.w, 0.f); }
+                if (relu & BN_RELU_OUT) { o.x = fmaxf(o.x, 0.f); o.y = fmaxf(o.y, 0.f); o.z = fmaxf(o.z, 0.f); o.w = fmaxf(o.w, 0.f); }
                 reinterpret_cast<float4*>(y)[p * Q + cq] = o;
                 if (sign_bits)
                     sign_bits[p * Q + cq] = (unsigned char)((o.x > 0.f) | ((o.y > 0.f) << 1) | ((o.z > 0.f) << 2) | ((o.w > 0.f) << 3));
@@ -718,6 +723,7 @@
     BnFinArgs a;
     if (!partial || parts <= 0 || !fin_args(fin, &a) || !x || !y || n_pixels <= 0) return DAM_ERR_BAD_ARG;
     if (res_scale && (!res || !res_shift)) return DAM_ERR_BAD_ARG;
+    if ((relu & ~(BN_RELU_OUT | BN_RELU_RES)) || ((relu & BN_RELU_RES) && !res_scale)) return DAM_ERR_BAD_ARG;
     if (C % 16 || C > 1024) return DAM_ERR_UNSUPPORTED;
     hipStream_t st = (hipStream_t)stream;
     if (!fa_fwd_table_ok(C, parts)) {
@@ -812,6 +818,7 @@
     if (!x || !scale || !shift || !y || n_pixels <= 0) return DAM_ERR_BAD_ARG;
     if (C % 16) return DAM_ERR_UNSUPPORTED;
     if (res_scale && (!res || !res_shift)) return DAM_ERR_BAD_ARG;
+    if ((relu & ~(BN_RELU_OUT | BN_RELU_RES)) || ((relu & BN_RELU_RES) && !res_scale)) return DAM_ERR_BAD_ARG;
     const int64_t nq = n_pixels * (C / 4);
     hipLaunchKernelGGL(bn_apply_kernel, dim3(elt_blocks(nq)), dim3(256), 0, (hipStream_t)stream, x, nq, C / 4, scale, shift,
                        res, res_scale, res_shift, relu, y, sign_bits);
diff --git a/deep-audio-mixer_amd/csrc/dam_head.hip b/deep-audio-mixer_amd/csrc/dam_head.hip
--- a/deep-audio-mixer_amd/csrc/dam_head.hip
+++ b/deep-audio-mixer_amd/csrc/dam_head.hip
@@ -42,6 +42,57 @@
                 if (gl == 0 && live) h[((size_t)b * S + s) * P + p] = fmaxf(t + cb[s], 0.f);
             }
         }
+    }
+}
+
+template <int GS>
+__global__ __launch_bounds__(1024) void head_fwd_fused_kernel(const float* __restrict__ trunk, int P, int C,
+                                                              const float* __restrict__ cw, const float* __restrict__ cb,
+                                                              const float* __restrict__ fcw, const float* __restrict__ fcb,
+                                                              float* __restrict__ h, float* __restrict__ g) {
+    __shared__ float red[16];
+    constexpr int G = 64 / GS, U = 4, SLOTS = 16 * G;
+    const int s = blockIdx.x, S = gridDim.x, b = blockIdx.y;
+    const int lane = threadIdx.x & 63, wave = threadIdx.x >> 6, gl = lane % GS, gi = lane / GS;
+    const int Q = C / 4;
+    const bool mine = gl < Q;
+    const float4 w = mine ? reinterpret_cast<const float4*>(cw + (size_t)s * C)[gl] : make_float4(0.f, 0.f, 0.f, 0.f);
+    const float cbs = cb[s];
+    const float* fr = fcw + (size_t)s * P;
+    float* hr = h + ((size_t)b * S + s) * P;
+    const float4* tb = reinterpret_cast<const float4*>(trunk + (size_t)b * P * C);
+    float fa = 0.f;
+    for (int base = wave * G; base < P; base += SLOTS * U) {
+        float4 v[U];
+        float fw[U];
+#pragma unroll
+        for (int u = 0; u < U; ++u) {
+            const int p = base + gi + u * SLOTS;
+            const bool live = p < P;
+            v[u] = (live && mine) ? tb[(size_t)p * Q + gl] : make_float4(0.f, 0.f, 0.f, 0.f);
+            fw[u] = live ? fr[p] : 0.f;
+        }
+#pragma unroll
+        for (int u = 0; u < U; ++u) {
+            const int p = base + gi + u * SLOTS;
+            float t = fmaf(v[u].x, w.x, fmaf(v[u].y, w.y, fmaf(v[u].z, w.z, v[u].w * w.w)));
+            t = wave_sum16(t);
+            if (GS >= 32) t += __shfl_xor(t, 16);
+            if (GS >= 64) t += __shfl_xor(t, 32);
+            if (gl == 0 && p < P) {
+                const float hv = fmaxf(t + cbs, 0.f);
+                hr[p] = hv;
+                fa = fmaf(fw[u], hv, fa);
+            }
+        }
+    }
+    fa = wave_sum64(gl == 0 ? fa : 0.f);
+    if (lane == 0) red[wave] = fa;
+    __syncthreads();
+    if (threadIdx.x == 0) {
+        float a = 0.f;
+        for (int i = 0; i < 16; ++i) a += red[i];
+        g[b * S + s] = a + fcb[s];
     }
 }
 
@@ -180,6 +231,102 @@
         partial_b[(size_t)blockIdx.x * S + threadIdx.x] = a;
     }
 }
+template <int GS>
+__global__ __launch_bounds__(256) void head_bwd_fused_kernel(const float* __restrict__ dg, const float* __restrict__ h,
+                                                             const float* __restrict__ trunk, int B, int P, int C, int S,
+                                                             const float* __restrict__ cw, const float* __restrict__ fcw,
+                                                             float* __restrict__ dtrunk, int64_t ppb, float* __restrict__ partial,
+                                                             float* __restrict__ partial_b, float* __restrict__ dfcw,
+                                                             float* __restrict__ dfcb) {
+    extern __shared__ __attribute__((aligned(16))) float sm[];
+    __shared__ float es[4][MAX_STEMS];
+    if (blockIdx.y == 1) {
+        for (int i = blockIdx.x * blockDim.x + threadIdx.x; i < S * P; i += gridDim.x * blockDim.x) {
+            const int s = i / P, p = i - s * P;
+            float a = 0.f;
+            for (int bb = 0; bb < B; ++bb) a = fmaf(dg[bb * S + s], h[((size_t)bb * S + s) * P + p], a);
+            dfcw[i] = a;
+            if (i < S) {
+                float t = 0.f;
+                for (int bb = 0; bb < B; ++bb) t += dg[bb * S + i];
+                dfcb[i] = t;
+            }
+        }
+        return;
+    }
+    const int SC = S * C;
+    for (int e = threadIdx.x; e < SC; e += blockDim.x) sm[e] = cw[e];
+    __syncthreads();
+    constexpr int G = 64 / GS, U = 2, R = 4 * G;
+    const int lane = threadIdx.x & 63, wave = threadIdx.x >> 6, gl = lane % GS, gi = lane / GS;
+    const int Q = C / 4;
+    const bool mine = gl < Q;
+    const int64_t BP = (int64_t)B * P;
+    const int64_t lo = blockIdx.x * ppb, hi = (lo + ppb < BP) ? lo + ppb : BP;
+    float acc[MAX_STEMS][4], esum[MAX_STEMS];
+#pragma unroll
+    for (int s = 0; s < MAX_STEMS; ++s) { acc[s][0] = acc[s][1] = acc[s][2] = acc[s][3] = 0.f; esum[s] = 0.f; }
+    for (int64_t base = lo + wave * G + gi; base < hi; base += R * U) {
+        float4 tv[U];
+        float ev[U][MAX_STEMS];
+#pragma unroll
+        for (int u = 0; u < U; ++u) {
+            const int64_t bp = base + u * R;
+            const bool ok = bp < hi;
+            const int b = ok ? (int)(bp / P) : 0, p = ok ? (int)(bp - (int64_t)b * P) : 0;
+            tv[u] = (ok && mine) ? reinterpret_cast<const float4*>(trunk)[bp * Q + gl] : make_float4(0.f, 0.f, 0.f, 0.f);
+#pragma unroll
+            for (int s = 0; s < MAX_STEMS; ++s) {
+                ev[u][s] = 0.f;
+                if (s < S) {
+                    const float hv = h[((size_t)b * S + s) * P + p], fv = fcw[(size_t)s * P + p], dv = dg[b * S + s];
+                    ev[u][s] = (ok && hv > 0.f) ? dv * fv : 0.f;
+                }
+            }
+        }
+#pragma unroll
+        for (int u = 0; u < U; ++u) {
+            const int64_t bp = base + u * R;
+            float4 o = make_float4(0.f, 0.f, 0.f, 0.f);
+#pragma unroll
+            for (int s = 0; s < MAX_STEMS; ++s) {
+                if (s < S) {
+                    const float e = ev[u][s];
+                    const float4 w = mine ? reinterpret_cast<const float4*>(sm + s * C)[gl] : make_float4(0.f, 0.f, 0.f, 0.f);
+                    o.x = fmaf(e, w.x, o.x); o.y = fmaf(e, w.y, o.y); o.z = fmaf(e, w.z, o.z); o.w = fmaf(e, w.w, o.w);
+                    acc[s][0] = fmaf(e, tv[u].x, acc[s][0]); acc[s][1] = fmaf(e, tv[u].y, acc[s][1]);
+                    acc[s][2] = fmaf(e, tv[u].z, acc[s][2]); acc[s][3] = fmaf(e, tv[u].w, acc[s][3]);
+                    esum[s] += e;
+                }
+            }
+            if (bp < hi && mine) reinterpret_cast<float4*>(dtrunk)[bp * Q + gl] = o;
+        }
+    }
+    __syncthreads();
+#pragma unroll
+    for (int s = 0; s < MAX_STEMS; ++s) {
+        if (s < S) {
+            if (GS <= 16) {
+#pragma unroll
+                for (int i = 0; i < 4; ++i) acc[s][i] += __shfl_xor(acc[s][i], 16);
+                esum[s] += __shfl_xor(esum[s], 16);
+            }
+            if (GS <= 32) {
+#pragma unroll
+                for (int i = 0; i < 4; ++i) acc[s][i] += __shfl_xor(acc[s][i], 32);
+                esum[s] += __shfl_xor(esum[s], 32);
+            }
+            if (gi == 0 && mine)
+                reinterpret_cast<float4*>(sm + ((size_t)wave * S + s) * C)[gl] = make_float4(acc[s][0], acc[s][1], acc[s][2], acc[s][3]);
+            if (lane == 0) es[wave][s] = esum[s];
+        }
+    }
+    __syncthreads();
+    for (int i = threadIdx.x; i < SC; i += blockDim.x)
+        partial[(size_t)blockIdx.x * SC + i] = ((sm[i] + sm[SC + i]) + sm[2 * SC + i]) + sm[3 * SC + i];
+    if ((int)threadIdx.x < S)
+        partial_b[(size_t)blockIdx.x * S + threadIdx.x] = ((es[0][threadIdx.x] + es[1][threadIdx.x]) + es[2][threadIdx.x]) + es[3][threadIdx.x];
+}
 __global__ __launch_bounds__(256) void head_bwd_cw_finalize_kernel(const float* __restrict__ partial,
                                                                    const float* __restrict__ partial_b, int parts, int C, int S,
                                                                    float* __restrict__ dcw, float* __restrict__ dcb) {
@@ -351,6 +498,20 @@
     else hipLaunchKernelGGL(head_conv_kernel<64>, dim3(gx, B), dim3(256), (size_t)S * C * sizeof(float), st, trunk, P, C, S, conv_w, conv_b, h);
     DAM_CHECK_LAUNCH();
     hipLaunchKernelGGL(head_fc_kernel, dim3(S, B), dim3(256), 0, st, h, P, S, fc_w, fc_b, gains);
+    DAM_CHECK_LAUNCH();
+    return DAM_OK;
+}
+
+extern "C" int dam_heads_fwd_fused_f32(const float* trunk, int B, int P, int C, int S, const float* conv_w, const float* conv_b,
+                                       const float* fc_w, const float* fc_b, float* h, float* gains, void* stream) {
+    if (!trunk || !conv_w || !conv_b || !fc_w || !fc_b || !h || !gains || B <= 0 || P <= 0) return DAM_ERR_BAD_ARG;
+    if (C % 4 || C < 4 || C > 256 || S < 1 || S > MAX_STEMS || B > 65535) return DAM_ERR_UNSUPPORTED;
+    hipStream_t st = (hipStream_t)stream;
+    const int Q = C / 4, gs = Q <= 16 ? 16 : Q <= 32 ? 32 : 64;
+#define DAM_HEAD_FWD_FUSED(GS_) \
+    hipLaunchKernelGGL(head_fwd_fused_kernel<GS_>, dim3(S, B), dim3(1024), 0, st, trunk, P, C, conv_w, conv_b, fc_w, fc_b, h, gains)
+    if (gs == 16) DAM_HEAD_FWD_FUSED(16); else if (gs == 32) DAM_HEAD_FWD_FUSED(32); else DAM_HEAD_FWD_FUSED(64);
+#undef DAM_HEAD_FWD_FUSED
     DAM_CHECK_LAUNCH();
     return DAM_OK;
 }
@@ -393,6 +554,32 @@
     return DAM_OK;
 }
 
+extern "C" int dam_heads_bwd_fused_f32(const float* dgains, const float* h, const float* trunk, int B, int P, int C, int S,
+                                       const float* conv_w, const float* fc_w, float* dtrunk, float* dconv_w, float* dconv_b,
+                                       float* dfc_w, float* dfc_b, float* workspace, void* stream) {
+    if (!dgains || !h || !trunk || !conv_w || !fc_w || !dtrunk || !dconv_w || !dconv_b || !dfc_w || !dfc_b || !workspace || B <= 0 || P <= 0)
+        return DAM_ERR_BAD_ARG;
+    if (C % 16 || S < 1 || S > MAX_STEMS || B > 65534 || C > 256 || (size_t)4 * S * C * sizeof(float) > 60 * 1024) return DAM_ERR_UNSUPPORTED;
+    hipStream_t st = (hipStream_t)stream;
+    float* partial = workspace + (size_t)B * S * P;
+    float* partial_b = partial + (size_t)1024 * S * C;
+    const int Q = C / 4, gs = Q <= 16 ? 16 : Q <= 32 ? 32 : 64, R = 4 * (64 / gs);
+    const int64_t BP = (int64_t)B * P;
+    int64_t parts = cdiv(BP, (int64_t)R * 2); if (parts > 1024) parts = 1024;
+    const int64_t ppb = cdiv(BP, parts);
+    parts = cdiv(BP, ppb);
+#define DAM_HEAD_BWD_FUSED(GS_)                                                                                                 \
+    hipLaunchKernelGGL(head_bwd_fused_kernel<GS_>, dim3((unsigned)parts, 2), dim3(256), (size_t)4 * S * C * sizeof(float), st, dgains, h, \
+                       trunk, B, P, C, S, conv_w, fc_w, dtrunk, ppb, partial, partial_b, dfc_w, dfc_b)
+    if (gs == 16) DAM_HEAD_BWD_FUSED(16); else if (gs == 32) DAM_HEAD_BWD_FUSED(32); else DAM_HEAD_BWD_FUSED(64);
+#undef DAM_HEAD_BWD_FUSED
+    DAM_CHECK_LAUNCH();
+    hipLaunchKernelGGL(head_bwd_cw_finalize_kernel, dim3((unsigned)cdiv((int64_t)S * C + S, 8)), dim3(256), 0, st, partial, partial_b,
+                       (int)parts, C, S, dconv_w, dconv_b);
+    DAM_CHECK_LAUNCH();
+    return DAM_OK;
+}
+
 extern "C" int dam_masksum_fwd_f32(const float* x, const float* gains, int B, int S, int64_t FT, float* masked, void* stream) {
     if (!x || !gains || !masked || B <= 0 || FT <= 0) return DAM_ERR_BAD_ARG;
     if (S < 1 || S > MAX_STEMS || B > 65535) return DAM_ERR_UNSUPPORTED;
diff --git a/deep-audio-mixer_amd/layers.py b/deep-audio-mixer_amd/layers.py
--- a/deep-audio-mixer_amd/layers.py
+++ b/deep-audio-mixer_amd/layers.py
@@ -43,16 +43,18 @@
         c, stats = self.fwd_conv(x, w, bn, training, bias=bias, in_affine=in_affine)
         return (c,) + tuple(stats if stats is not None else _bn_fwd_stats(c, bn, training))
 
-    def fwd_bn_apply(self, x, w, bn, training, in_affine=None, res=None, res_affine=None, sign_bits=False, bias=None):
+    def fwd_bn_apply(self, x, w, bn, training, in_affine=None, res=None, res_affine=None, sign_bits=False, bias=None,
+                     res_relu=False):
         rs, rh = res_affine if res_affine is not None else (None, None)
         if training:
             c, rec = self.fwd_conv(x, w, bn, training, bias=bias, in_affine=in_affine, finalize=False)
             rec = rec if rec is not None else ops.bn_stats_partial(c)
             (m, i, sc, sh), out = ops.bn_finalize_apply(rec[0], rec[1], _bn_args(bn, training), c, relu=True, res=res,
-                                                        res_scale=rs, res_shift=rh, sign_bits=sign_bits)
+                                                        res_scale=rs, res_shift=rh, sign_bits=sign_bits, res_relu=res_relu)
             return c, m, i, sc, sh, out
         c, m, i, sc, sh = self.fwd_bn(x, w, bn, training, bias=bias, in_affine=in_affine)
-        return c, m, i, sc, sh, ops.bn_apply(c, sc, sh, relu=True, res=res, res_scale=rs, res_shift=rh, sign_bits=sign_bits)
+        return c, m, i, sc, sh, ops.bn_apply(c, sc, sh, relu=True, res=res, res_scale=rs, res_shift=rh, sign_bits=sign_bits,
+                                              res_relu=res_relu)
 
     def wgrad(self, x, dy, in_affine=None, out=None):
         aff = {} if in_affine is None else dict(in_scale=in_affine[0], in_shift=in_affine[1], relu_in=True)
@@ -182,8 +184,9 @@
         self.c, self.mean, self.invstd, self.scale, self.shift, self.bits = c, mean, invstd, scale, shift, bits
         self.partials, self.dx_ptr, self.dx_version = None, None, None
 
-    def request(self):
-        return (self.c, self.mean, self.invstd, self.scale, self.shift) + ((self.bits,) if self.bits is not None else ())
+    def request(self, c=None):
+        return ((self.c if self.c is not None else c, self.mean, self.invstd, self.scale, self.shift)
+                + ((self.bits,) if self.bits is not None else ()))
 
     def offer(self, sums, dx):
         self.partials, self.dx_ptr, self.dx_version = sums, dx.data_ptr(), dx._version
@@ -202,13 +205,17 @@
 class ConvBnReluFn(torch.autograd.Function):
 
     @staticmethod
-    def forward(ctx, x, w, bias, gamma, beta, spec, bn, training):
+    def forward(ctx, x, w, bias, gamma, beta, spec, bn, training, lazy=False):
         if spec.nhwc16 is not None and not ctx.needs_input_grad[0]:
             spec, x = spec.nhwc16, ops.nchw_to_nhwc16(x)
-        c, mean, invstd, scale, shift, a = spec.fwd_bn_apply(x, w.detach(), bn, training,
-                                                             bias=None if bias is None else bias.detach())
+        b = None if bias is None else bias.detach()
+        if lazy:
+            c, mean, invstd, scale, shift = spec.fwd_bn(x, w.detach(), bn, training, bias=b)
+            a, c._dam_affine = c, (scale, shift)
+        else:
+            c, mean, invstd, scale, shift, a = spec.fwd_bn_apply(x, w.detach(), bn, training, bias=b)
         ctx.save_for_backward(x, w, c, gamma, mean, invstd, scale, shift)
-        ctx.up = a._dam_upstream = _UpstreamBn(c, mean, invstd, scale, shift) if ops.DGRAD_BN_SUMS else None
+        ctx.up = a._dam_upstream = _UpstreamBn(None if lazy else c, mean, invstd, scale, shift) if ops.DGRAD_BN_SUMS else None
         ctx.spec, ctx.training, ctx.has_bias = spec, training, bias is not None
         ctx.slots = (_slot(w), _slot(bias), _slot(gamma), _slot(beta))
         return a
@@ -226,7 +233,7 @@
         dbias = ops.channel_sum(dc, spec.cout, out=sb) if ctx.has_bias else None
         dx = spec.dgrad(dc, w, _hw(x, spec.in_nchw)) if ctx.needs_input_grad[0] else None
         return (dx, None if sw is not None else dw, None if sb is not None else dbias, None if sg is not None else dgamma,
-                None if sbt is not None else dbeta, None, None, None)
+                None if sbt is not None else dbeta, None, None, None, None)
 
 
 class DropoutFn(torch.autograd.Function):
@@ -248,7 +255,10 @@
 class BasicBlockFn(torch.autograd.Function):
 
     @staticmethod
-    def forward(ctx, x, w1, g1, b1, w2, g2, b2, wsc, gsc, bsc, blk, training):
+    def forward(ctx, x, w1, g1, b1, w2, g2, b2, wsc, gsc, bsc, blk, training, x_affine=None):
+        if x_affine is not None and wsc is not None:
+            raise ValueError('x_affine: identity blocks only')
+        ctx.x_affine = x_affine
         if wsc is not None:
             bn_sc = blk.shortcut[1]
             one = None
@@ -270,9 +280,10 @@
                                                                        res=cs, res_affine=(scs, shs), sign_bits=True)
             ctx.save_for_backward(x, w1, g1, w2, g2, c1, c2, out, m1, i1, m2, i2, sc1, sh1, bits, wsc, gsc, cs, ms, is_)
         else:
-            c1, m1, i1, sc1, sh1 = blk.spec1.fwd_bn(x, w1.detach(), blk.bn1, training)
+            c1, m1, i1, sc1, sh1 = blk.spec1.fwd_bn(x, w1.detach(), blk.bn1, training, in_affine=x_affine)
             c2, m2, i2, sc2, sh2, (out, bits) = blk.spec2.fwd_bn_apply(c1, w2.detach(), blk.bn2, training, in_affine=(sc1, sh1),
-                                                                       res=x, sign_bits=True)
+                                                                       res=x, res_affine=x_affine, sign_bits=True,
+                                                                       res_relu=x_affine is not None)
             ctx.save_for_backward(x, w1, g1, w2, g2, c1, c2, out, m1, i1, m2, i2, sc1, sh1, bits)
         ctx.up_self = None
         if wsc is None and ops.DGRAD_BN_SUMS:
@@ -310,7 +321,7 @@
             da1 = blk.spec2.dgrad(dc2, w2, (c1.shape[1], c1.shape[2]))
         dc1, dg1, db1 = ops.bn_backward(da1, None, c1, g1, m1, i1, tr, mask_affine=(sc1, sh1),
                                         dgamma=s_g1, dbeta=s_b1, partials=sums)
-        dw1 = blk.spec1.wgrad(x, dc1, out=wview(s_w1, w1))
+        dw1 = blk.spec1.wgrad(x, dc1, in_affine=ctx.x_affine, out=wview(s_w1, w1))
         first = (keep(dw1, s_w1), keep(dg1, s_g1), keep(db1, s_b1), keep(dw2, s_w2), keep(dg2, s_g2), keep(db2, s_b2))
         if ctx.has_sc:
             dws = blk.spec_sc.wgrad(x, dcs, out=wview(s_ws, wsc))
@@ -327,14 +338,14 @@
             else:
                 dx = blk.spec1.dgrad(dc1, w1, hw)
                 blk.spec_sc.dgrad(dcs, wsc, hw, accumulate_into=dx)
-            return (dx,) + first + (keep(dws, s_ws), keep(dgs, s_gs), keep(dbs, s_bs), None, None)
+            return (dx,) + first + (keep(dws, s_ws), keep(dgs, s_gs), keep(dbs, s_bs), None, None, None)
         up = ctx.upstream
-        if up is not None and ops.DGRAD_BN_SUMS and up.c.shape == x.shape:
-            dx, sums = blk.spec1.dgrad(dc1, w1, hw, res=dout, res_mask=out, res_mask_bits=bits, bn_bwd=up.request())
+        if up is not None and ops.DGRAD_BN_SUMS and (up.c is None or up.c.shape == x.shape):
+            dx, sums = blk.spec1.dgrad(dc1, w1, hw, res=dout, res_mask=out, res_mask_bits=bits, bn_bwd=up.request(x))
             up.offer(sums, dx)
         else:
             dx = blk.spec1.dgrad(dc1, w1, hw, res=dout, res_mask=out)
-        return (dx,) + first + (None, None, None, None, None)
+        return (dx,) + first + (None, None, None, None, None, None)
 
 
 class HeadsFn(torch.autograd.Function):
@@ -413,7 +424,12 @@
                               FoldedConvBn(self.spec_sc, self.shortcut[0], self.shortcut[1]) if self.spec_sc is not None else None)
         return f
 
-    def forward(self, x):
+    def forward(self, x, x_affine=None):
+        if x_affine is not None:
+            if self.spec_sc is not None:
+                raise ValueError('x_affine: identity blocks only')
+            return BasicBlockFn.apply(x, self.conv1.weight, self.bn1.weight, self.bn1.bias, self.conv2.weight,
+                                      self.bn2.weight, self.bn2.bias, None, None, None, self, self.training, x_affine)
         if inference_mode(self):
             f1, f2, fs = self._folded()
             if f1.foldable() and f2.foldable() and (fs is None or fs.foldable()):
diff --git a/deep-audio-mixer_amd/models/model_resnet.py b/deep-audio-mixer_amd/models/model_resnet.py
--- a/deep-audio-mixer_amd/models/model_resnet.py
+++ b/deep-audio-mixer_amd/models/model_resnet.py
@@ -1,3 +1,4 @@
+import torch
 import torch.nn as nn
 import torch.nn.functional as F
 
@@ -50,13 +51,22 @@
         stem = getattr(self, '_stem_fold', None)
         if stem is None:
             stem = self._stem_fold = FoldedConvBn(self._stem, self.conv1, self.bn1)
+        lazy = False
         if inference_mode(self) and stem.foldable():
             out = stem.fwd(x)
         else:
+            first = self.layer1[0]
+            lazy = (self.training and self._stem.nhwc16 is not None and not (torch.is_grad_enabled() and x.requires_grad)
+                    and isinstance(first, BasicBlock) and first.spec_sc is None)
             out = ConvBnReluFn.apply(x, self.conv1.weight, None, self.bn1.weight, self.bn1.bias, self._stem, self.bn1,
-                                     self.training)
+                                     self.training, lazy)
+            if lazy:
+                out = first(out, x_affine=out._dam_affine)
+                for blk in list(self.layer1)[1:]:
+                    out = blk(out)
         for i in range(1, 7):
-            out = getattr(self, 'layer%d' % i)(out)
+            if i > 1 or not lazy:
+                out = getattr(self, 'layer%d' % i)(out)
             if tap is not None and i == self.DDP_BOUNDARY:
                 tap.append(out)
         return out
diff --git a/deep-audio-mixer_amd/ops.py b/deep-audio-mixer_amd/ops.py
--- a/deep-audio-mixer_amd/ops.py
+++ b/deep-audio-mixer_amd/ops.py
@@ -347,7 +347,8 @@
     return ws, parts.value
 
 
-def bn_finalize_apply(partial, parts, bn, x, relu=True, res=None, res_scale=None, res_shift=None, sign_bits=False):
+def bn_finalize_apply(partial, parts, bn, x, relu=True, res=None, res_scale=None, res_shift=None, sign_bits=False,
+                      res_relu=False):
     _lib.require_cuda(partial, x)
     C = x.shape[-1]
     out4 = torch.empty((4, C), dtype=torch.float32, device=x.device)
@@ -355,7 +356,8 @@
     y = torch.empty_like(x)
     bits = torch.empty(x.shape[:-1] + (C // 4,), dtype=torch.uint8, device=x.device) if sign_bits else None
     _lib.check(_lib.lib().dam_bn_finalize_apply_f32(_lib.ptr(partial), int(parts), C, ctypes.byref(fin), _lib.ptr(x), x.numel() // C,
-                                                    _lib.ptr(res), _lib.ptr(res_scale), _lib.ptr(res_shift), 1 if relu else 0,
+                                                    _lib.ptr(res), _lib.ptr(res_scale), _lib.ptr(res_shift),
+                                                    (1 if relu else 0) | (2 if res_relu else 0),
                                                     _lib.ptr(y), _lib.ptr(bits), _lib.stream()), 'dam_bn_finalize_apply_f32')
     return (out4[0], out4[1], out4[2], out4[3]), ((y, bits) if sign_bits else y)
 
@@ -429,14 +431,14 @@
     return out[0], out[1], out[2], out[3]
 
 
-def bn_apply(x, scale, shift, relu=True, res=None, res_scale=None, res_shift=None, sign_bits=False):
+def bn_apply(x, scale, shift, relu=True, res=None, res_scale=None, res_shift=None, sign_bits=False, res_relu=False):
     _lib.require_cuda(x)
     C = x.shape[-1]
     y = torch.empty_like(x)
     bits = torch.empty(x.shape[:-1] + (C // 4,), dtype=torch.uint8, device=x.device) if sign_bits else None
     _lib.check(_lib.lib().dam_bn_apply_f32(_lib.ptr(x), x.numel() // C, C, _lib.ptr(scale), _lib.ptr(shift), _lib.ptr(res),
-                                           _lib.ptr(res_scale), _lib.ptr(res_shift), 1 if relu else 0, _lib.ptr(y),
-                                           _lib.ptr(bits), _lib.stream()), 'dam_bn_apply_f32')
+                                           _lib.ptr(res_scale), _lib.ptr(res_shift), (1 if relu else 0) | (2 if res_relu else 0),
+                                           _lib.ptr(y), _lib.ptr(bits), _lib.stream()), 'dam_bn_apply_f32')
     return (y, bits) if sign_bits else y
 
 
@@ -494,7 +496,12 @@
     return out
 
 
-def heads_fwd(trunk, conv_w, conv_b, fc_w, fc_b):
+HEADS_FUSED_FWD_P_MAX = 256
+HEADS_FUSED_BWD_P_MAX = 4096
+heads_fused_launches = [0, 0]
+
+
+def heads_fwd(trunk, conv_w, conv_b, fc_w, fc_b, fused=None):
     _lib.require_cuda(trunk)
     B, C = trunk.shape[0], trunk.shape[-1]
     P = trunk.numel() // (B * C)
@@ -503,12 +510,19 @@
         raise ValueError('fc_head expects %d inputs but the trunk gives %d (flattened_dim mismatch)' % (fc_w.shape[1], P))
     h = torch.empty((B, S, P), dtype=torch.float32, device=trunk.device)
     g = torch.empty((B, S), dtype=torch.float32, device=trunk.device)
-    _lib.check(_lib.lib().dam_heads_fwd_f32(_lib.ptr(trunk), B, P, C, S, _lib.ptr(conv_w), _lib.ptr(conv_b), _lib.ptr(fc_w),
-                                            _lib.ptr(fc_b), _lib.ptr(h), _lib.ptr(g), _lib.stream()), 'dam_heads_fwd_f32')
+    args = (_lib.ptr(trunk), B, P, C, S, _lib.ptr(conv_w), _lib.ptr(conv_b), _lib.ptr(fc_w), _lib.ptr(fc_b), _lib.ptr(h), _lib.ptr(g),
+            _lib.stream())
+    if fused or (fused is None and P <= HEADS_FUSED_FWD_P_MAX):
+        st = _lib.lib().dam_heads_fwd_fused_f32(*args)
+        if st != -2:
+            _lib.check(st, 'dam_heads_fwd_fused_f32')
+            heads_fused_launches[0] += 1
+            return h, g
+    _lib.check(_lib.lib().dam_heads_fwd_f32(*args), 'dam_heads_fwd_f32')
     return h, g
 
 
-def heads_bwd(dgains, h, trunk, conv_w, fc_w, outs=None):
+def heads_bwd(dgains, h, trunk, conv_w, fc_w, outs=None, fused=None):
     B, S, P = h.shape
     C = trunk.shape[-1]
     dev = trunk.device
@@ -520,9 +534,15 @@
     dfb = o[3] if o[3] is not None else torch.empty(S, dtype=torch.float32, device=dev)
     L = _lib.lib()
     ws = _workspace(dev, L.dam_heads_bwd_workspace_floats(B, P, C, S))
-    _lib.check(L.dam_heads_bwd_f32(_lib.ptr(dgains), _lib.ptr(h), _lib.ptr(trunk), B, P, C, S, _lib.ptr(conv_w), _lib.ptr(fc_w),
-                                   _lib.ptr(dtrunk), _lib.ptr(dcw), _lib.ptr(dcb), _lib.ptr(dfw), _lib.ptr(dfb), _lib.ptr(ws),
-                                   _lib.stream()), 'dam_heads_bwd_f32')
+    args = (_lib.ptr(dgains), _lib.ptr(h), _lib.ptr(trunk), B, P, C, S, _lib.ptr(conv_w), _lib.ptr(fc_w), _lib.ptr(dtrunk),
+            _lib.ptr(dcw), _lib.ptr(dcb), _lib.ptr(dfw), _lib.ptr(dfb), _lib.ptr(ws), _lib.stream())
+    if fused or (fused is None and P <= HEADS_FUSED_BWD_P_MAX):
+        st = L.dam_heads_bwd_fused_f32(*args)
+        if st != -2:
+            _lib.check(st, 'dam_heads_bwd_fused_f32')
+            heads_fused_launches[1] += 1
+            return dtrunk, dcw, dcb, dfw, dfb
+    _lib.check(L.dam_heads_bwd_f32(*args), 'dam_heads_bwd_f32')
     return dtrunk, dcw, dcb, dfw, dfb
 
 
diff --git a/include/dam_hip.h b/include/dam_hip.h
--- a/include/dam_hip.h
+++ b/include/dam_hip.h
@@ -20,7 +20,7 @@
 #define DAM_PCM_ROTATE 0x200
 struct dam_bn_bwd_sums;
 
-#define DAM_ABI_VERSION 22
+#define DAM_ABI_VERSION 23
 const char* dam_arch(void);
 int dam_abi_version(void);
 
@@ -179,6 +179,11 @@
 int dam_heads_bwd_f32(const float* dgains, const float* h, const float* trunk, int B, int P, int C, int S,
                       const float* conv_w, const float* fc_w, float* dtrunk, float* dconv_w, float* dconv_b,
                       float* dfc_w, float* dfc_b, float* workspace, void* stream);
+int dam_heads_fwd_fused_f32(const float* trunk, int B, int P, int C, int S, const float* conv_w, const float* conv_b,
+                            const float* fc_w, const float* fc_b, float* h, float* gains, void* stream);
+int dam_heads_bwd_fused_f32(const float* dgains, const float* h, const float* trunk, int B, int P, int C, int S,
+                            const float* conv_w, const float* fc_w, float* dtrunk, float* dconv_w, float* dconv_b,
+                            float* dfc_w, float* dfc_b, float* workspace, void* stream);
 int dam_masksum_fwd_f32(const float* x, const float* gains, int B, int S, int64_t FT, float* masked, void* stream);
 int64_t dam_masksum_workspace_floats(int B, int S);
 int dam_masksum_bwd_f32(const float* dmasked, const float* x, int B, int S, int64_t FT, float* dgains,
```

Measured after the change: 2.052 million stem-spectrogram-frames/s, median of 6. No clear change (+0.9%).
